# prstrive/SCGaussian

Hardware: AMD Instinct MI355X
Metric: train_iters_per_sec (higher is better)
Workload: dtype f32; 1 GPU; S2: 200000 Gaussians, 1008x756, SH degree 3, fwd+bwd per view (BASELINE configs[1] shape: LLFF-fern 3-view training, 200 k Gaussians @ 1008x756); gaussians=200000, width=1008, height=756, sh_degree=3, visible=174771, views=3, parallelism=single, ranks_seen=1, launched_by=single process, grad_bucket_bytes=0, grad_bucket_bytes_per_view=0

## Files before the change

scgaussian_amd/csrc/api.hip:

```cpp
#include <stdarg.h>
#include <stdio.h>
#include <string.h>

#include "scg_common.h"
#include "scg_debug.h"

#include <atomic>
#include <chrono>
#include <thread>

namespace scg {

static thread_local char g_err[512] = "";

int fail(int code, const char* fmt, ...) {
    va_list ap;
    va_start(ap, fmt);
    vsnprintf(g_err, sizeof(g_err), fmt, ap);
    va_end(ap);
    return code;
}

int check_hip(hipError_t e, const char* what) {
    if (e == hipSuccess) return 0;
    snprintf(g_err, sizeof(g_err), "%s: %s (hipError %d)", what, hipGetErrorString(e), (int)e);
    return (int)e;
}

int validate_frame(const ScgFrame* f, bool need_bg) {
    if (!f) return fail(SCG_E_NULL, "frame is NULL");
    if (f->P < 0) return fail(SCG_E_RANGE, "P = %d < 0", f->P);
    if (f->width <= 0 || f->height <= 0 || f->width > 65535 * SCG_TILE || f->height > 65535 * SCG_TILE)
        return fail(SCG_E_RANGE, "image size %d x %d out of range", f->width, f->height);
    if (f->sh_degree < 0 || f->sh_degree > 3) return fail(SCG_E_RANGE, "sh_degree %d not in 0..3", f->sh_degree);
    if (!(f->tanfovx > 0.f) || !(f->tanfovy > 0.f)) return fail(SCG_E_RANGE, "tanfov must be positive");
    if (!f->viewmatrix || !f->projmatrix || !f->campos) return fail(SCG_E_NULL, "viewmatrix/projmatrix/campos is NULL");
    if (need_bg && !f->bg) return fail(SCG_E_NULL, "bg is NULL");
    return 0;
}

static inline size_t align_up(size_t v, size_t a) { return (v + a - 1) / a * a; }
static inline bool aligned16(const void* p) { return (reinterpret_cast<uintptr_t>(p) & 15u) == 0; }
static inline bool aligned64(const void* p) { return (reinterpret_cast<uintptr_t>(p) & 63u) == 0; }
int validate_model(const ScgFrame* f, const ScgModel* m);

static int validate_inputs(const ScgFrame* f, const float* means3D, const float* opacities, const float* shs,
                           const float* colors_precomp, const float* scales, const float* rotations,
                           const float* cov3D_precomp) {
    if (f->P == 0) return 0;
    if (!means3D || !opacities) return fail(SCG_E_NULL, "means3D/opacities is NULL");
    if ((shs == nullptr) == (colors_precomp == nullptr))
        return fail(SCG_E_EXCLUSIVE, "Please provide exactly one of either SHs or precomputed colors!");
    const bool has_sr = scales != nullptr && rotations != nullptr;
    if ((scales != nullptr) != (rotations != nullptr) || has_sr == (cov3D_precomp != nullptr))
        return fail(SCG_E_EXCLUSIVE,
                    "Please provide exactly one of either scale/rotation pair or precomputed 3D covariance!");
    if (shs && f->sh_coeffs < (f->sh_degree + 1) * (f->sh_degree + 1))
        return fail(SCG_E_RANGE, "sh_coeffs %d < (sh_degree+1)^2 = %d", f->sh_coeffs,
                    (f->sh_degree + 1) * (f->sh_degree + 1));
    if (rotations && !aligned16(rotations)) return fail(SCG_E_ALIGN, "rotations must be 16-byte aligned");
    return 0;
}

static int validate_model_set(const ScgModelSet& m, bool ray, const char* name) {
    if (m.count < 0) return fail(SCG_E_RANGE, "%s.count = %d < 0", name, m.count);
    if (m.count == 0) return 0;
    if (ray ? (!m.zval || !m.rayo || !m.rayd) : !m.xyz)
        return fail(SCG_E_NULL, ray ? "%s: zval / rayo / rayd is NULL" : "%s: xyz is NULL", name);
    if (!m.features_dc || !m.features_rest || !m.opacity || !m.scaling || !m.rotation)
        return fail(SCG_E_NULL, "%s: features_dc / features_rest / opacity / scaling / rotation is NULL", name);
    if (!aligned16(m.rotation) || !aligned16(m.features_rest) || !aligned16(m.features_dc))
        return fail(SCG_E_ALIGN, "%s: rotation / features_rest / features_dc must be 16-byte aligned", name);
    return 0;
}

int validate_model(const ScgFrame* f, const ScgModel* m) {
    int rc = validate_model_set(m->ray, true, "model.ray");
    if (rc) return rc;
    if ((rc = validate_model_set(m->bg, false, "model.bg"))) return rc;
    if ((int64_t)m->ray.count + m->bg.count != f->P)
        return fail(SCG_E_RANGE, "model holds %d + %d Gaussians, frame.P = %d", m->ray.count, m->bg.count, f->P);
    if (f->P > 0 && f->sh_coeffs != 16)
        return fail(SCG_E_RANGE, "the model path reads (n,1,3) + (n,15,3) SH records: frame.sh_coeffs must be 16, not %d", f->sh_coeffs);
    return 0;
}

}

using namespace scg;

extern "C" {

const char* scg_last_error(void) { return g_err; }
int32_t scg_abi_version(void) { return SCG_ABI_VERSION; }

size_t scg_struct_bytes(int32_t which) {
    switch (which) {
        case 0: return sizeof(ScgFrame);
        case 1: return sizeof(ScgWorkspaceLayout);
        case 2: return sizeof(ScgStageEvents);
        case 3: return sizeof(ScgModel);
        case 4: return sizeof(ScgModelGrads);
        case 5: return sizeof(ScgAdamSegment);
        default: return 0;
    }
}

size_t scg_geometry_scratch_bytes(int32_t P) { return align_up(scan_scratch_bytes(P > 0 ? P : 1), 256); }

int scg_geometry_forward(const ScgFrame* frame, const float* means3D, const float* opacities, const float* shs,
                         const float* colors_precomp, const float* scales, const float* rotations,
                         const float* cov3D_precomp, float* splats, int32_t* radii, uint8_t* clamped,
                         uint32_t* rects, uint32_t* depth_keys, uint32_t* num_rendered_out, void* scratch,
                         size_t scratch_bytes, void* stream) {
    int rc = validate_frame(frame, false);
    if (rc) return rc;
    rc = validate_inputs(frame, means3D, opacities, shs, colors_precomp, scales, rotations, cov3D_precomp);
    if (rc) return rc;
    hipStream_t s = reinterpret_cast<hipStream_t>(stream);
    if (frame->P == 0)
        return num_rendered_out ? check_hip(hipMemsetAsync(num_rendered_out, 0, sizeof(uint32_t), s), "memset R") : 0;
    if (!splats || !radii || !clamped || !rects || !depth_keys || !scratch)
        return fail(SCG_E_NULL, "output/scratch pointer is NULL");
    if (!aligned16(splats)) return fail(SCG_E_ALIGN, "splats must be 16-byte aligned");
    if ((reinterpret_cast<uintptr_t>(rects) & 7u) != 0) return fail(SCG_E_ALIGN, "rects must be 8-byte aligned");
    if (scratch_bytes < scg_geometry_scratch_bytes(frame->P))
        return fail(SCG_E_SCRATCH, "geometry scratch: %zu < %zu bytes", scratch_bytes, scg_geometry_scratch_bytes(frame->P));
    const FrameDev f = make_frame_dev(frame);
    uint32_t* block_sums = reinterpret_cast<uint32_t*>(scratch);
    rc = launch_geometry_forward(f, means3D, opacities, shs, colors_precomp, scales, rotations, cov3D_precomp, splats,
                                 radii, clamped, rects, depth_keys, block_sums, s);
    if (rc || !num_rendered_out) return rc;
    return launch_total_from_block_sums(block_sums, (frame->P + kBlock - 1) / kBlock, num_rendered_out, s);
}

struct LegacyLayout { size_t keys0, keys1, vals0, offsets, scan, sortscr, total; };

static LegacyLayout legacy_layout(int P, int64_t R) {
    LegacyLayout L;
    size_t off = 0;
    auto take = [&](size_t bytes) { size_t o = off; off += align_up(bytes, 256); return o; };
    L.keys0 = take((size_t)R * sizeof(uint64_t));
    L.keys1 = take((size_t)R * sizeof(uint64_t));
    L.vals0 = take((size_t)R * sizeof(uint32_t));
    L.offsets = take((size_t)P * sizeof(uint32_t));
    L.scan = take(scan_scratch_bytes(P));
    L.sortscr = take(sort_scratch_bytes(R));
    L.total = off;
    return L;
}

static int key_bits(int n_tiles) {
    int bits = 0;
    while ((1ll << bits) < (long long)n_tiles) ++bits;
    return 32 + (bits > 0 ? bits : 1);
}

static int n_tiles_of(int32_t width, int32_t height) {
    return ((width + kTile - 1) / kTile) * ((height + kTile - 1) / kTile);
}

static bool use_tile_path(int n_tiles, int64_t R, int32_t algo) {
    if (algo == SCG_BINNING_GLOBAL_SORT) return false;
    return tile_binning_supported(n_tiles, R);
}

size_t scg_binning_scratch_bytes(int32_t P, int64_t num_rendered, int32_t width, int32_t height, int32_t algo) {
    const int64_t R = num_rendered > 0 ? num_rendered : 1;
    const int Pp = P > 0 ? P : 1;
    const int n_tiles = n_tiles_of(width, height);
    if (use_tile_path(n_tiles, R, algo)) return tile_binning_layout(Pp, R, n_tiles).total;
    return legacy_layout(Pp, R).total;
}

size_t scg_ranges_words(int32_t width, int32_t height) {
    const int n_tiles = ((width + kTile - 1) / kTile) * ((height + kTile - 1) / kTile);
    return (size_t)2 * n_tiles + (size_t)5 * tile_order_slots(n_tiles);
}

int32_t scg_forward_sorts_in_blend(int64_t capacity, int32_t width, int32_t height, int32_t options) {
    if (width <= 0 || height <= 0 || capacity <= 0 || (options & SCG_DEBUG_SEPARATE_SORT)) return 0;
    const int n_tiles = n_tiles_of(width, height);
    if (!use_tile_path(n_tiles, capacity, SCG_BINNING_AUTO)) return 0;
    return tile_binning_defers_sort(capacity, n_tiles) ? 1 : 0;
}

int32_t scg_binning_accepts_bound(int64_t num_rendered_bound, int32_t width, int32_t height, int32_t algo) {
    if (width <= 0 || height <= 0) return 0;
    return use_tile_path(n_tiles_of(width, height), num_rendered_bound > 0 ? num_rendered_bound : 1, algo) ? 1 : 0;
}

int scg_binning(const ScgFrame* frame, int64_t num_rendered, const uint32_t* rects, const uint32_t* depth_keys,
                uint32_t* point_list, uint32_t* ranges, uint64_t* keys_sorted, int32_t algo, void* scratch,
                size_t scratch_bytes, void* stream) {
    int rc = validate_frame(frame, false);
    if (rc) return rc;
    if (!ranges) return fail(SCG_E_NULL, "ranges is NULL");
    if (num_rendered < 0 || num_rendered > 0xFFFFFFFFll) return fail(SCG_E_RANGE, "num_rendered out of range");
    if (algo != SCG_BINNING_AUTO && algo != SCG_BINNING_GLOBAL_SORT) return fail(SCG_E_RANGE, "unknown binning algo %d", algo);
    hipStream_t s = reinterpret_cast<hipStream_t>(stream);
    const FrameDev f = make_frame_dev(frame);
    const int n_tiles = f.gx * f.gy;
    if (num_rendered == 0 || frame->P == 0) return launch_tile_ranges(nullptr, 0, ranges, n_tiles, s);
    if (!rects || !depth_keys || !point_list || !scratch) return fail(SCG_E_NULL, "binning pointer is NULL");
    const size_t need = scg_binning_scratch_bytes(frame->P, num_rendered, frame->width, frame->height, algo);
    if (scratch_bytes < need) return fail(SCG_E_SCRATCH, "binning scratch: %zu < %zu bytes", scratch_bytes, need);

    if (use_tile_path(n_tiles, num_rendered, algo))
        return launch_tile_binning(f, num_rendered, rects, depth_keys, point_list, ranges, keys_sorted, scratch, nullptr, false, false, false, false, s);

    const LegacyLayout L = legacy_layout(frame->P, num_rendered);
    char* base = reinterpret_cast<char*>(scratch);
    uint64_t* keys0 = reinterpret_cast<uint64_t*>(base + L.keys0);
    uint64_t* keys1 = reinterpret_cast<uint64_t*>(base + L.keys1);
    uint32_t* vals0 = reinterpret_cast<uint32_t*>(base + L.vals0);
    uint32_t* offsets = reinterpret_cast<uint32_t*>(base + L.offsets);
    rc = launch_rect_counts_scan(rects, frame->P, offsets, reinterpret_cast<uint32_t*>(base + L.scan), s);
    if (rc) return rc;
    const int end_bit = key_bits(n_tiles);
    const bool odd = (sort_num_passes(end_bit) & 1) != 0;
    uint64_t* ka = odd ? keys0 : keys1;
    uint32_t* va = odd ? vals0 : point_list;
    uint64_t* kb = odd ? keys1 : keys0;
    uint32_t* vb = odd ? point_list : vals0;
    rc = launch_duplicate_keys(f, rects, depth_keys, offsets, ka, va, s);
    if (rc) return rc;
    rc = launch_sort_pairs(ka, va, kb, vb, num_rendered, end_bit, base + L.sortscr, s, odd);
    if (rc) return rc;
    rc = launch_tile_ranges(keys1, num_rendered, ranges, n_tiles, s);
    if (rc) return rc;
    if (keys_sorted)
        return check_hip(hipMemcpyAsync(keys_sorted, keys1, (size_t)num_rendered * sizeof(uint64_t),
                                        hipMemcpyDeviceToDevice, s), "copy keys_sorted");
    return 0;
}

size_t scg_sort_scratch_bytes(int64_t n) { return align_up(sort_scratch_bytes(n > 0 ? n : 1), 256); }

int scg_sort_pairs(uint64_t* keys_in, uint32_t* vals_in, uint64_t* keys_out, uint32_t* vals_out, int64_t n,
                   int32_t end_bit, void* scratch, size_t scratch_bytes, void* stream) {
    if (n < 0 || n > 0xFFFFFFFFll) return fail(SCG_E_RANGE, "n out of range");
    if (end_bit < 1 || end_bit > 64) return fail(SCG_E_RANGE, "end_bit %d not in 1..64", end_bit);
    if (n == 0) return 0;
    if (!keys_in || !vals_in || !keys_out || !vals_out || !scratch) return fail(SCG_E_NULL, "sort pointer is NULL");
    if (scratch_bytes < scg_sort_scratch_bytes(n)) return fail(SCG_E_SCRATCH, "sort scratch too small");
    return launch_sort_pairs(keys_in, vals_in, keys_out, vals_out, n, end_bit, scratch,
                             reinterpret_cast<hipStream_t>(stream), true);
}

size_t scg_scan_scratch_bytes(int64_t n) { return align_up(scan_scratch_bytes(n > 0 ? n : 1), 256); }

int scg_inclusive_scan_u32(const uint32_t* in, uint32_t* out, int64_t n, uint32_t* total_out, void* scratch,
                           size_t scratch_bytes, void* stream) {
    if (n < 0 || n > 0x7FFFFFFFll * 256) return fail(SCG_E_RANGE, "n out of range");
    hipStream_t s = reinterpret_cast<hipStream_t>(stream);
    if (n == 0) return total_out ? check_hip(hipMemsetAsync(total_out, 0, sizeof(uint32_t), s), "memset total") : 0;
    if (!in || !out || !scratch) return fail(SCG_E_NULL, "scan pointer is NULL");
    if (scratch_bytes < scg_scan_scratch_bytes(n)) return fail(SCG_E_SCRATCH, "scan scratch too small");
    return launch_inclusive_scan(in, out, n, total_out, scratch, s);
}

int scg_blend_forward(const ScgFrame* frame, const uint32_t* ranges, const uint32_t* point_list,
                      const float* splats, float* out_color, float* out_depth, float* out_alpha, float* final_T,
                      uint32_t* n_contrib, float* dsplats_zero, void* stream) {
    int rc = validate_frame(frame, true);
    if (rc) return rc;
    if (!ranges || !out_color || !out_depth || !out_alpha || !final_T || !n_contrib)
        return fail(SCG_E_NULL, "blend_forward pointer is NULL");
    if (splats && !aligned16(splats)) return fail(SCG_E_ALIGN, "splats must be 16-byte aligned");
    if (dsplats_zero && !aligned64(dsplats_zero)) return fail(SCG_E_ALIGN, "dsplats_zero must be 64-byte aligned");
    const FrameDev f = make_frame_dev(frame);
    return launch_blend_forward(f, ranges, point_list, splats, out_color, out_depth, out_alpha, final_T, n_contrib,
                                dsplats_zero, reinterpret_cast<hipStream_t>(stream));
}

static int blend_backward_checked(const ScgFrame* frame, const uint32_t* ranges, const uint32_t* point_list,
                                  const float* splats, const float* final_T, const uint32_t* n_contrib,
                                  const float* dL_dcolor, const float* dL_ddepth, const float* dL_dalpha, float* dsplats,
                                  int32_t dsplats_prezeroed, void* stream, hipEvent_t started, hipEvent_t done) {
    int rc = validate_frame(frame, true);
    if (rc) return rc;
    if (frame->P == 0) return 0;
    if (!ranges || !final_T || !n_contrib || !dL_dcolor || !dsplats || !splats)
        return fail(SCG_E_NULL, "blend_backward pointer is NULL");
    if (!aligned16(splats)) return fail(SCG_E_ALIGN, "splats must be 16-byte aligned");
    if (!aligned64(dsplats)) return fail(SCG_E_ALIGN, "dsplats must be 64-byte aligned (one record = one line)");
    if (frame->P > 60000000) return fail(SCG_E_RANGE, "blend_backward addresses gradient records with 32-bit offsets: P <= 60e6");
    const FrameDev f = make_frame_dev(frame);
    return launch_blend_backward(f, ranges, point_list, splats, final_T, n_contrib, dL_dcolor, dL_ddepth, dL_dalpha,
                                 dsplats, dsplats_prezeroed != 0, reinterpret_cast<hipStream_t>(stream), started, done);
}

int scg_blend_backward(const ScgFrame* frame, const uint32_t* ranges, const uint32_t* point_list,
                       const float* splats, const float* final_T, const uint32_t* n_contrib, const float* dL_dcolor,
                       const float* dL_ddepth, const float* dL_dalpha, float* dsplats, int32_t dsplats_prezeroed,
                       void* stream) {
    return blend_backward_checked(frame, ranges, point_list, splats, final_T, n_contrib, dL_dcolor, dL_ddepth, dL_dalpha,
                                  dsplats, dsplats_prezeroed, stream, nullptr, nullptr);
}

int scg_geometry_backward(const ScgFrame* frame, const float* means3D, const float* opacities, const float* shs,
                          const float* colors_precomp, const float* scales, const float* rotations,
                          const float* cov3D_precomp, const int32_t* radii, const uint8_t* clamped,
                          const float* dsplats, float* dL_dmeans3D, float* dL_dmeans2D, float* dL_dopacities,
                          float* dL_dshs, float* dL_dcolors_precomp, float* dL_dscales, float* dL_drotations,
                          float* dL_dcov3D_precomp, int32_t accumulate, void* stream) {
    int rc = validate_frame(frame, false);
    if (rc) return rc;
    rc = validate_inputs(frame, means3D, opacities, shs, colors_precomp, scales, rotations, cov3D_precomp);
    if (rc) return rc;
    if (frame->P == 0) return 0;
    if (!radii || !clamped || !dsplats || !dL_dmeans3D || !dL_dmeans2D || !dL_dopacities)
        return fail(SCG_E_NULL, "geometry_backward pointer is NULL");
    if ((shs != nullptr) != (dL_dshs != nullptr) || (colors_precomp != nullptr) != (dL_dcolors_precomp != nullptr))
        return fail(SCG_E_EXCLUSIVE, "dL_dshs / dL_dcolors_precomp must match the colour input that was used");
    const bool has_sr = scales != nullptr;
    if (has_sr != (dL_dscales != nullptr) || has_sr != (dL_drotations != nullptr) ||
        (cov3D_precomp != nullptr) != (dL_dcov3D_precomp != nullptr))
        return fail(SCG_E_EXCLUSIVE, "dL_dscales/dL_drotations / dL_dcov3D_precomp must match the covariance input used");
    if (!aligned64(dsplats) || (dL_drotations && !aligned16(dL_drotations)))
        return fail(SCG_E_ALIGN, "dsplats must be 64-byte, dL_drotations 16-byte aligned");
    const FrameDev f = make_frame_dev(frame);
    return launch_geometry_backward(f, means3D, opacities, shs, colors_precomp, scales, rotations, cov3D_precomp, radii,
                                    clamped, dsplats, dL_dmeans3D, dL_dmeans2D, dL_dopacities, dL_dshs,
                                    dL_dcolors_precomp, dL_dscales, dL_drotations, dL_dcov3D_precomp,
                                    accumulate & (SCG_BACKWARD_ACCUMULATE | SCG_BACKWARD_SH_TAIL_ZERO),
                                    reinterpret_cast<hipStream_t>(stream));
}

static inline int mark(const ScgStageEvents* ev, int stage, bool end, hipStream_t s) {
    if (!ev) return 0;
    void* e = end ? ev->end[stage] : ev->begin[stage];
    return e ? check_hip(hipEventRecord(reinterpret_cast<hipEvent_t>(e), s), "stage event record") : 0;
}

int scg_workspace_layout(int32_t P, int64_t capacity, int32_t width, int32_t height, ScgWorkspaceLayout* out) {
    if (!out) return fail(SCG_E_NULL, "layout is NULL");
    if (P < 0 || capacity < 0 || capacity > 0xFFFFFFFFll || width <= 0 || height <= 0)
        return fail(SCG_E_RANGE, "workspace layout: P / capacity / image size out of range");
    const int64_t cap = capacity > 0 ? capacity : 1;
    const size_t Pp = (size_t)(P > 0 ? P : 1), hw = (size_t)width * height;
    size_t off = 0;
    auto take = [&](size_t bytes) { size_t o = off; off += align_up(bytes, 256); return (uint64_t)o; };
    out->splats = take(Pp * SCG_SPLAT_FLOATS * sizeof(float));
    out->rects = take(Pp * 2 * sizeof(uint32_t));
    out->depth_keys = take(Pp * sizeof(uint32_t));
    out->clamped = take(Pp);
    out->point_list = take((size_t)cap * sizeof(uint32_t));
    out->ranges = take(scg_ranges_words(width, height) * sizeof(uint32_t));
    out->final_T = take(hw * sizeof(float));
    out->n_contrib = take(hw * sizeof(uint32_t));
    out->bin_scratch = take(scg_binning_scratch_bytes(P, cap, width, height, SCG_BINNING_AUTO));
    out->total = (uint64_t)off;
    out->partial_words = (uint64_t)(scg_geometry_scratch_bytes(P) / sizeof(uint32_t));
    return 0;
}

static int forward_impl(const ScgFrame* frame, const ScgModel* model, const float* means3D, const float* opacities,
                        const float* shs, const float* colors_precomp, const float* scales, const float* rotations,
                        const float* cov3D_precomp, int64_t capacity, void* workspace, size_t workspace_bytes, int32_t* radii,
                        float* out_color, float* out_depth, float* out_alpha, uint32_t* partial_sums, void* event,
                        float* dsplats_zero, int32_t options, const ScgStageEvents* stage_events, void* stream) {
    int rc = validate_frame(frame, true);
    if (rc) return rc;
    rc = model ? validate_model(frame, model)
               : validate_inputs(frame, means3D, opacities, shs, colors_precomp, scales, rotations, cov3D_precomp);
    if (rc) return rc;
    if (!workspace || !out_color || !out_depth || !out_alpha || !partial_sums || (frame->P > 0 && !radii))
        return fail(SCG_E_NULL, "scg_forward: workspace / output / partial_sums pointer is NULL");
    if (!aligned16(workspace)) return fail(SCG_E_ALIGN, "workspace must be 16-byte aligned");
    if (dsplats_zero && !aligned64(dsplats_zero)) return fail(SCG_E_ALIGN, "dsplats_zero must be 64-byte aligned");
    ScgWorkspaceLayout L;
    rc = scg_workspace_layout(frame->P, capacity, frame->width, frame->height, &L);
    if (rc) return rc;
    if (workspace_bytes < L.total) return fail(SCG_E_SCRATCH, "workspace: %zu < %llu bytes", workspace_bytes, (unsigned long long)L.total);
    hipStream_t s = reinterpret_cast<hipStream_t>(stream);
    const FrameDev f = make_frame_dev(frame);
    const int n_tiles = f.gx * f.gy;
    char* base = reinterpret_cast<char*>(workspace);
    float* splats = reinterpret_cast<float*>(base + L.splats);
    uint32_t* rects = reinterpret_cast<uint32_t*>(base + L.rects);
    uint32_t* depth_keys = reinterpret_cast<uint32_t*>(base + L.depth_keys);
    uint8_t* clamped = reinterpret_cast<uint8_t*>(base + L.clamped);
    uint32_t* point_list = reinterpret_cast<uint32_t*>(base + L.point_list);
    uint32_t* ranges = reinterpret_cast<uint32_t*>(base + L.ranges);
    const bool keep_state = !(options & SCG_FORWARD_NO_BACKWARD_STATE);
    float* final_T = keep_state ? reinterpret_cast<float*>(base + L.final_T) : nullptr;
    uint32_t* n_contrib = keep_state ? reinterpret_cast<uint32_t*>(base + L.n_contrib) : nullptr;
    const bool empty = frame->P == 0 || capacity == 0;
    if (!empty && !use_tile_path(n_tiles, capacity, SCG_BINNING_AUTO))
        return fail(SCG_E_RANGE, "scg_forward needs the tile-first binning path (scg_binning_accepts_bound); use the staged calls");
    if (options & SCG_FORWARD_ARM_PARTIAL_SUMS) {
        const int nb = frame->P > 0 ? (frame->P + kBlock - 1) / kBlock : 1;
        volatile uint32_t* w = partial_sums;
        for (int i = 0; i < nb; ++i) w[i] = SCG_PARTIAL_SUM_ARMED;
        std::atomic_thread_fence(std::memory_order_release);
    }
    if ((rc = mark(stage_events, 0, false, s))) return rc;
    const bool hist_in_geometry = !empty && !(options & SCG_DEBUG_SEPARATE_HIST) && tile_binning_hist_in_geometry(f, capacity);
    if (frame->P == 0) {
        rc = check_hip(hipMemsetAsync(partial_sums, 0, sizeof(uint32_t), s), "memset partial sums");
    } else if (hist_in_geometry) {
        rc = model ? launch_geometry_hist_binned_model(f, capacity, *model, splats, radii, clamped, rects, depth_keys, partial_sums,
                                                       base + L.bin_scratch, s)
                   : launch_geometry_hist_binned(f, capacity, means3D, opacities, shs, colors_precomp, scales, rotations,
                                                 cov3D_precomp, splats, radii, clamped, rects, depth_keys, partial_sums,
                                                 base + L.bin_scratch, s);
    } else {
        rc = model ? launch_geometry_forward_model(f, *model, splats, radii, clamped, rects, depth_keys, partial_sums, s)
                   : launch_geometry_forward(f, means3D, opacities, shs, colors_precomp, scales, rotations, cov3D_precomp, splats,
                                             radii, clamped, rects, depth_keys, partial_sums, s);
    }
    if (rc) return rc;
    if ((rc = mark(stage_events, 0, true, s))) return rc;
    if (event) {
        rc = check_hip(hipEventRecord(reinterpret_cast<hipEvent_t>(event), s), "event record");
        if (rc) return rc;
    }
    if ((rc = mark(stage_events, 1, false, s))) return rc;
    bool fused_sort = !empty && !(options & SCG_DEBUG_SEPARATE_SORT);
    const bool skip_rare = (options & SCG_FORWARD_SKIP_RARE_SORT) != 0;
    if (empty && frame->num_rendered_out)
        if ((rc = check_hip(hipMemsetAsync(frame->num_rendered_out, 0, sizeof(uint32_t), s), "memset num_rendered_out"))) return rc;
    rc = empty ? launch_tile_ranges(nullptr, 0, ranges, n_tiles, s)
               : launch_tile_binning(f, capacity, rects, depth_keys, point_list, ranges, nullptr, base + L.bin_scratch,
                                     &fused_sort, hist_in_geometry, skip_rare, (options & SCG_FORWARD_RARE_8WAVE) != 0,
                                     (options & SCG_FORWARD_SPLIT_LONG_LISTS) != 0, s);
    if (rc) return rc;
    if ((rc = mark(stage_events, 1, true, s))) return rc;
    if ((rc = mark(stage_events, 2, false, s))) return rc;
    rc = fused_sort ? launch_tile_blend_forward(f, ranges, point_list, depth_keys, splats, out_color, out_depth, out_alpha,
                                                final_T, n_contrib, frame->P ? dsplats_zero : nullptr, base + L.bin_scratch,
                                                capacity, !skip_rare, s)
                    : launch_blend_forward(f, ranges, point_list, splats, out_color, out_depth, out_alpha, final_T, n_contrib,
                                           frame->P ? dsplats_zero : nullptr, s);
    if (rc) return rc;
    return mark(stage_events, 2, true, s);
}

int scg_forward(const ScgFrame* frame, const float* means3D, const float* opacities, const float* shs,
                const float* colors_precomp, const float* scales, const float* rotations, const float* cov3D_precomp,
                int64_t capacity, void* workspace, size_t workspace_bytes, int32_t* radii, float* out_color,
                float* out_depth, float* out_alpha, uint32_t* partial_sums, void* event, float* dsplats_zero,
                int32_t options, const ScgStageEvents* stage_events, void* stream) {
    return forward_impl(frame, nullptr, means3D, opacities, shs, colors_precomp, scales, rotations, cov3D_precomp, capacity,
                        workspace, workspace_bytes, radii, out_color, out_depth, out_alpha, partial_sums, event, dsplats_zero,
                        options, stage_events, stream);
}

int scg_forward_model(const ScgFrame* frame, const ScgModel* model, int64_t capacity, void* workspace, size_t workspace_bytes,
                      int32_t* radii, float* out_color, float* out_depth, float* out_alpha, uint32_t* partial_sums, void* event,
                      float* dsplats_zero, int32_t options, const ScgStageEvents* stage_events, void* stream) {
    if (!model) return fail(SCG_E_NULL, "model is NULL");
    return forward_impl(frame, model, nullptr, nullptr, nullptr, nullptr, nullptr, nullptr, nullptr, capacity, workspace,
                        workspace_bytes, radii, out_color, out_depth, out_alpha, partial_sums, event, dsplats_zero, options,
                        stage_events, stream);
}

int scg_model_activate(const ScgModel* model, float* means3D, float* opacities, float* scales, float* rotations, void* stream) {
    if (!model) return fail(SCG_E_NULL, "model is NULL");
    ScgFrame fr;
    memset(&fr, 0, sizeof(fr));
    fr.P = model->ray.count + model->bg.count;
    fr.sh_coeffs = 16;
    const int rc = validate_model(&fr, model);
    if (rc) return rc;
    if (rotations && !aligned16(rotations)) return fail(SCG_E_ALIGN, "rotations must be 16-byte aligned");
    return launch_model_activate(*model, means3D, opacities, scales, rotations, reinterpret_cast<hipStream_t>(stream));
}

int64_t scg_wait_num_rendered(void* event, const uint32_t* partial_sums_host, int32_t P) {
    if (!partial_sums_host) { fail(SCG_E_NULL, "partial_sums_host is NULL"); return SCG_E_NULL; }
    const int nb = P > 0 ? (P + kBlock - 1) / kBlock : 1;
    if (event) {
        const hipError_t e = hipEventSynchronize(reinterpret_cast<hipEvent_t>(event));
        if (e != hipSuccess) { check_hip(e, "event synchronize"); return -(int64_t)e - 1000; }
    } else {
        const volatile uint32_t* w = partial_sums_host;
        const auto t0 = std::chrono::steady_clock::now();
        for (int i = nb - 1; i >= 0; --i) {
            uint64_t spins = 0;
            while (w[i] == SCG_PARTIAL_SUM_ARMED) {
                if (spins < 100000u) __builtin_ia32_pause(); else std::this_thread::yield();
                if ((++spins & 0xFFFFu) == 0 &&
                    std::chrono::steady_clock::now() - t0 > std::chrono::seconds(120)) {
                    fail(SCG_E_RANGE, "scg_wait_num_rendered: the geometry stage's partial sums did not arrive within 120 s "
                                      "(kernel fault, or partial_sums is not host-coherent memory)");
                    return SCG_E_RANGE;
                }
            }
        }
        std::atomic_thread_fence(std::memory_order_acquire);
    }
    int64_t total = 0;
    for (int i = 0; i < nb; ++i) total += partial_sums_host[i];
    return total;
}

int scg_event_create(void** event_out, int32_t timing) {
    if (!event_out) return fail(SCG_E_NULL, "event_out is NULL");
    hipEvent_t ev;
    const int rc = check_hip(hipEventCreateWithFlags(&ev, timing ? hipEventDefault : hipEventDisableTiming), "event create");
    if (rc) return rc;
    *event_out = reinterpret_cast<void*>(ev);
    return 0;
}

int scg_event_destroy(void* event) {
    return event ? check_hip(hipEventDestroy(reinterpret_cast<hipEvent_t>(event)), "event destroy") : 0;
}

int scg_event_elapsed_ms(void* begin, void* end, float* ms_out) {
    if (!begin || !end || !ms_out) return fail(SCG_E_NULL, "event / ms_out is NULL");
    return check_hip(hipEventElapsedTime(ms_out, reinterpret_cast<hipEvent_t>(begin), reinterpret_cast<hipEvent_t>(end)),
                     "event elapsed time");
}

int scg_backward(const ScgFrame* frame, const float* means3D, const float* opacities, const float* shs,
                 const float* colors_precomp, const float* scales, const float* rotations, const float* cov3D_precomp,
                 const int32_t* radii, int64_t capacity, const void* workspace, const float* dL_dcolor,
                 const float* dL_ddepth, const float* dL_dalpha, float* dsplats, int32_t dsplats_prezeroed,
                 float* dL_dmeans3D, float* dL_dmeans2D, float* dL_dopacities, float* dL_dshs, float* dL_dcolors_precomp,
                 float* dL_dscales, float* dL_drotations, float* dL_dcov3D_precomp, int32_t accumulate,
                 const ScgStageEvents* stage_events, void* stream) {
    if (!frame) return fail(SCG_E_NULL, "frame is NULL");
    if (frame->P == 0) return 0;
    if (!workspace) return fail(SCG_E_NULL, "workspace is NULL");
    ScgWorkspaceLayout L;
    int rc = scg_workspace_layout(frame->P, capacity, frame->width, frame->height, &L);
    if (rc) return rc;
    hipStream_t s = reinterpret_cast<hipStream_t>(stream);
    const char* base = reinterpret_cast<const char*>(workspace);
    hipEvent_t bb_begin = stage_events ? reinterpret_cast<hipEvent_t>(stage_events->begin[0]) : nullptr;
    hipEvent_t bb_end = stage_events ? reinterpret_cast<hipEvent_t>(stage_events->end[0]) : nullptr;
    rc = blend_backward_checked(frame, reinterpret_cast<const uint32_t*>(base + L.ranges),
                                reinterpret_cast<const uint32_t*>(base + L.point_list),
                                reinterpret_cast<const float*>(base + L.splats),
                                reinterpret_cast<const float*>(base + L.final_T),
                                reinterpret_cast<const uint32_t*>(base + L.n_contrib), dL_dcolor, dL_ddepth, dL_dalpha,
                                dsplats, dsplats_prezeroed, stream, bb_begin, bb_end);
    if (rc) return rc;
    if ((rc = mark(stage_events, 1, false, s))) return rc;
    rc = scg_geometry_backward(frame, means3D, opacities, shs, colors_precomp, scales, rotations, cov3D_precomp, radii,
                               reinterpret_cast<const uint8_t*>(base + L.clamped), dsplats, dL_dmeans3D, dL_dmeans2D,
                               dL_dopacities, dL_dshs, dL_dcolors_precomp, dL_dscales, dL_drotations, dL_dcov3D_precomp,
                               accumulate, stream);
    if (rc) return rc;
    return mark(stage_events, 1, true, s);
}

int scg_backward_model(const ScgFrame* frame, const ScgModel* model, const int32_t* radii, int64_t capacity, const void* workspace,
                       const float* dL_dcolor, const float* dL_ddepth, const float* dL_dalpha, float* dsplats,
                       int32_t dsplats_prezeroed, const ScgModelGrads* grads, float* dL_dmeans2D, int32_t flags,
                       const ScgStageEvents* stage_events, void* stream) {
    if (!frame) return fail(SCG_E_NULL, "frame is NULL");
    if (!model || !grads) return fail(SCG_E_NULL, "model / grads is NULL");
    int rc = validate_frame(frame, false);
    if (rc) return rc;
    if ((rc = validate_model(frame, model))) return rc;
    if (frame->P == 0) return 0;
    if (!workspace || !radii || !dL_dmeans2D) return fail(SCG_E_NULL, "workspace / radii / dL_dmeans2D is NULL");
    for (int k = 0; k < 2; ++k) {
        const ScgModelSet& ms = k ? model->bg : model->ray;
        const ScgModelGradSet& gs = k ? grads->bg : grads->ray;
        if (ms.count == 0) continue;
        if ((k == 0 ? !gs.zval : !gs.xyz) || !gs.features_dc || !gs.features_rest || !gs.opacity || !gs.scaling || !gs.rotation)
            return fail(SCG_E_NULL, "grads.%s: a gradient buffer of a non-empty set is NULL", k ? "bg" : "ray");
        if (!aligned16(gs.rotation) || !aligned16(gs.features_rest) || !aligned16(gs.features_dc))
            return fail(SCG_E_ALIGN, "grads.%s: rotation / features_rest / features_dc must be 16-byte aligned", k ? "bg" : "ray");
    }
    ScgWorkspaceLayout L;
    rc = scg_workspace_layout(frame->P, capacity, frame->width, frame->height, &L);
    if (rc) return rc;
    hipStream_t s = reinterpret_cast<hipStream_t>(stream);
    const char* base = reinterpret_cast<const char*>(workspace);
    hipEvent_t bb_begin = stage_events ? reinterpret_cast<hipEvent_t>(stage_events->begin[0]) : nullptr;
    hipEvent_t bb_end = stage_events ? reinterpret_cast<hipEvent_t>(stage_events->end[0]) : nullptr;
    rc = blend_backward_checked(frame, reinterpret_cast<const uint32_t*>(base + L.ranges),
                                reinterpret_cast<const uint32_t*>(base + L.point_list),
                                reinterpret_cast<const float*>(base + L.splats),
                                reinterpret_cast<const float*>(base + L.final_T),
                                reinterpret_cast<const uint32_t*>(base + L.n_contrib), dL_dcolor, dL_ddepth, dL_dalpha,
                                dsplats, dsplats_prezeroed, stream, bb_begin, bb_end);
    if (rc) return rc;
    if ((rc = mark(stage_events, 1, false, s))) return rc;
    const FrameDev f = make_frame_dev(frame);
    rc = launch_geometry_backward_model(f, *model, *grads, radii, reinterpret_cast<const uint8_t*>(base + L.clamped), dsplats,
                                        dL_dmeans2D, flags & (SCG_BACKWARD_ACCUMULATE | SCG_BACKWARD_SH_TAIL_ZERO), s);
    if (rc) return rc;
    return mark(stage_events, 1, true, s);
}

}
```

scgaussian_amd/csrc/binning_tiles.hip:

```cpp
#include "scg_common.h"
#include "tile_sort.h"
#include "tile_walk.h"

#include <mutex>

namespace scg {

constexpr int kTileBlocksSmall = 128;
constexpr int kTileBlocksLarge = 256;
constexpr int64_t kLargeFrame = 1ll << 20;
constexpr int kLargeScene = 100000;
constexpr int kSortSmallMax = 2048;
constexpr int kSortDenseMax = 4096;
constexpr int kSortMidMax = 8192;
constexpr int kVeryLong = 16384;
constexpr int kSort8Max = 4096;
constexpr int kSortBigLdsMax = 16384;
constexpr int kMaxDynLds = 152 * 1024;

template <class F>
__device__ __forceinline__ void visit_instances(const uint2* __restrict__ rects, int grid_x, uint32_t ga, uint32_t gb,
                                                F&& f) {
    const int lane = lane_id();
    for (uint32_t g0 = ga; g0 < gb; g0 += kWave) {
        const uint32_t g = g0 + lane;
        uint2 r = make_uint2(0u, 0u);
        if (g < gb) r = rects[g];
        walk_rects(r, g, grid_x, f);
    }
}

__global__ __launch_bounds__(kBinThreads) void tile_hist_kernel(const uint2* __restrict__ rects, uint32_t P,
                                                                int grid_x, int n_tiles,
                                                                uint32_t* __restrict__ table,
                                                                uint32_t* __restrict__ class_counts,
                                                                uint32_t* __restrict__ len_hist) {
    extern __shared__ __attribute__((aligned(16))) unsigned char smem[];
    uint32_t* hist = reinterpret_cast<uint32_t*>(smem);
    if (blockIdx.x == 0) {
        if (threadIdx.x < 4) class_counts[threadIdx.x] = 0u;
        len_hist[threadIdx.x] = 0u;
    }
    for (int t = threadIdx.x; t < n_tiles; t += kBinThreads) hist[t] = 0;
    __syncthreads();
    uint32_t ga, gb;
    wave_slice(P, gridDim.x, blockIdx.x, wave_id(), ga, gb);
    visit_instances(rects, grid_x, ga, gb, [&](uint32_t tile, uint32_t) { atomicAdd(&hist[tile], 1u); });
    __syncthreads();
    uint32_t* row = table + (size_t)blockIdx.x * n_tiles;
    for (int t = threadIdx.x; t < n_tiles; t += kBinThreads) row[t] = hist[t];
}

constexpr int kColTiles = 64;
constexpr int kColGroups = kBinThreads / kColTiles;
constexpr int kColRowsMax = 16;

constexpr int kBands8 = 8;
constexpr int kLenClasses = 64;

__device__ __forceinline__ int len_class(uint32_t total, int shift) {
    return (int)min((uint32_t)(kLenClasses - 1), total >> shift);
}
__device__ __forceinline__ int order_class(const uint32_t* __restrict__ cost_in, int t, uint32_t total, int shift) {
    if (!cost_in) return len_class(total, shift);
    if (total == 0u) return 0;
    const int c = (int)(__float_as_uint((float)cost_in[t]) >> 19) - ((127 + 5) << 4);
    return max(0, min(kLenClasses - 1, c));
}

__global__ __launch_bounds__(kBinThreads) void table_colscan_kernel(uint32_t* __restrict__ table, int nblocks,
                                                                    int n_tiles, uint32_t* __restrict__ tile_total,
                                                                    uint32_t* __restrict__ len_hist, int len_shift,
                                                                    const uint32_t* __restrict__ cost_in,
                                                                    uint8_t* __restrict__ tile_class,
                                                                    uint32_t* __restrict__ tile_part) {
    __shared__ uint32_t s_part[kColGroups][kColTiles];
    const int c = threadIdx.x & (kColTiles - 1);
    const int q = threadIdx.x / kColTiles;
    const int t = blockIdx.x * kColTiles + c;
    const int b0 = (int)((int64_t)nblocks * q / kColGroups), b1 = (int)((int64_t)nblocks * (q + 1) / kColGroups);
    uint32_t v[kColRowsMax];
    uint32_t sum = 0;
#pragma unroll
    for (int k = 0; k < kColRowsMax; ++k) {
        v[k] = 0;
        if (t < n_tiles && b0 + k < b1) v[k] = table[(size_t)(b0 + k) * n_tiles + t];
    }
#pragma unroll
    for (int k = 0; k < kColRowsMax; ++k) sum += v[k];
    s_part[q][c] = sum;
    __syncthreads();
    uint32_t run = 0;
    for (int k = 0; k < q; ++k) run += s_part[k][c];
    __shared__ uint32_t s_len[kBands8 * kLenClasses];
    if (threadIdx.x < kBands8 * kLenClasses) s_len[threadIdx.x] = 0u;
    __syncthreads();
    if (t < n_tiles && q == kColGroups - 1) {
        tile_total[t] = run + sum;
        const int per = (n_tiles + 7) >> 3;
        const int cls = order_class(cost_in, t, run + sum, len_shift);
        tile_class[t] = (uint8_t)cls;
        atomicAdd(&s_len[(t / per) * kLenClasses + cls], 1u);
    }
    __syncthreads();
    if (threadIdx.x < kBands8 * kLenClasses && s_len[threadIdx.x]) atomicAdd(&len_hist[threadIdx.x], s_len[threadIdx.x]);
    if (q == kColGroups - 1) s_part[0][c] = (t < n_tiles) ? run + sum : 0u;
    __syncthreads();
    if (threadIdx.x < kColTiles) {
        uint32_t tot = s_part[0][threadIdx.x];
#pragma unroll
        for (int off = 32; off > 0; off >>= 1) tot += (uint32_t)__shfl_xor((int)tot, off, kWave);
        if (threadIdx.x == 0) tile_part[blockIdx.x] = tot;
    }
#pragma unroll
    for (int k = 0; k < kColRowsMax; ++k) {
        if (t < n_tiles && b0 + k < b1) table[(size_t)(b0 + k) * n_tiles + t] = run;
        run += v[k];
    }
}

constexpr int kBands = 8;
constexpr int kQueue = 2 * kWave;
constexpr int kScatterThreads = 256;
constexpr int kScatterWaves = kScatterThreads / kWave;

__device__ __forceinline__ uint32_t totals_before(const uint32_t* __restrict__ tile_total,
                                                  const uint32_t* __restrict__ tile_part, int t_first, uint32_t* s_red) {
    const int full = t_first / kColTiles;
    uint32_t v = 0;
    for (int k = threadIdx.x; k < full; k += kScatterThreads) v += tile_part[k];
    for (int k = full * kColTiles + (int)threadIdx.x; k < t_first; k += kScatterThreads) v += tile_total[k];
#pragma unroll
    for (int off = 32; off > 0; off >>= 1) v += (uint32_t)__shfl_xor((int)v, off, kWave);
    __syncthreads();
    if (lane_id() == 0) s_red[wave_id()] = v;
    __syncthreads();
    uint32_t sum = 0;
#pragma unroll
    for (int k = 0; k < kScatterWaves; ++k) sum += s_red[k];
    return sum;
}

__device__ __forceinline__ uint32_t block_exclusive_256(uint32_t v, uint32_t* s_red, uint32_t& total) {
    const int lane = lane_id(), w = wave_id();
    uint32_t inc = v;
#pragma unroll
    for (int off = 1; off < kWave; off <<= 1) {
        const uint32_t n = (uint32_t)__shfl_up((int)inc, off, kWave);
        if (lane >= off) inc += n;
    }
    __syncthreads();
    if (lane == kWave - 1) s_red[w] = inc;
    __syncthreads();
    uint32_t before = 0;
    total = 0;
#pragma unroll
    for (int k = 0; k < kScatterWaves; ++k) {
        const uint32_t sk = s_red[k];
        if (k < w) before += sk;
        total += sk;
    }
    return before + inc - v;
}

__device__ __forceinline__ void publish_tile_starts(int x, int n_tiles, const uint32_t* __restrict__ tile_total,
                                                    const uint32_t* __restrict__ tile_part,
                                                    uint32_t* __restrict__ tile_start, uint2* __restrict__ ranges,
                                                    uint32_t capacity, uint32_t* __restrict__ class_counts,
                                                    uint32_t* __restrict__ mid_tiles, uint32_t* __restrict__ big_tiles,
                                                    uint32_t small_max, const uint32_t* __restrict__ len_hist,
                                                    const uint8_t* __restrict__ tile_class,
                                                    uint32_t* __restrict__ cost_out, const uint32_t* __restrict__ bcost_in,
                                                    uint8_t* q_class ,
                                                    uint32_t* __restrict__ nr_out) {
    __shared__ uint32_t s_red[kScatterWaves];
    __shared__ uint32_t s_first[kLenClasses];
    __shared__ uint32_t s_cnt[kLenClasses];
    const int per = (n_tiles + 7) >> 3;
    const int t0 = x * per, t1 = min(t0 + per, n_tiles);
    const int lane = lane_id();
    if (threadIdx.x < kLenClasses) {
        uint32_t before = 0;
        for (int k = (int)threadIdx.x + 1; k < kLenClasses; ++k) before += len_hist[x * kLenClasses + k];
        s_first[threadIdx.x] = before;
        s_cnt[threadIdx.x] = 0u;
    }
    uint32_t carry = totals_before(tile_total, tile_part, min(t0, n_tiles), s_red);
    uint32_t* order = reinterpret_cast<uint32_t*>(ranges) + 2 * (size_t)n_tiles;
    for (int k0 = t0; k0 < t1; k0 += kScatterThreads) {
        const int t = k0 + (int)threadIdx.x;
        const bool in = t < t1;
        const uint32_t cnt = in ? tile_total[t] : 0u;
        uint32_t total;
        const uint32_t run = carry + block_exclusive_256(cnt, s_red, total);
        carry += total;
        uint32_t len = 0;
        if (in) {
            tile_start[t] = run;
            const uint32_t lo = min(run, capacity), hi = min(run + cnt, capacity);
            ranges[t] = (hi > lo) ? make_uint2(lo, hi) : make_uint2(0u, 0u);
            len = hi - lo;
            if (t == n_tiles - 1) {
                tile_start[n_tiles] = run + cnt;
                if (nr_out) *nr_out = run + cnt;
            }
            if (cost_out) cost_out[t] = 0u;
            const int c = (int)tile_class[t];
            order[t0 + s_first[c] + atomicAdd(&s_cnt[c], 1u)] = (uint32_t)t;
        }
        const bool is_big = len > (uint32_t)kSortMidMax, is_mid = !is_big && len > small_max;
        const uint64_t m_mid = __ballot(is_mid), m_big = __ballot(is_big);
        const uint64_t m_split = __ballot(len > (uint32_t)kVeryLong);
        if (lane == 0 && m_split) atomicAdd(&class_counts[3], (uint32_t)__popcll(m_split));
        uint32_t base_mid = 0, base_big = 0;
        if (lane == 0) {
            if (m_mid) base_mid = atomicAdd(&class_counts[0], (uint32_t)__popcll(m_mid));
            if (m_big) base_big = atomicAdd(&class_counts[1], (uint32_t)__popcll(m_big));
        }
        base_mid = (uint32_t)__shfl((int)base_mid, 0, kWave);
        base_big = (uint32_t)__shfl((int)base_big, 0, kWave);
        const uint64_t below = (lane == 0) ? 0ull : (~0ull >> (kWave - lane));
        if (is_mid) mid_tiles[base_mid + (uint32_t)__popcll(m_mid & below)] = (uint32_t)t;
        if (is_big) big_tiles[base_big + (uint32_t)__popcll(m_big & below)] = (uint32_t)t;
    }
    for (int k = max(t0, t1) + (int)threadIdx.x; k < t0 + per; k += kScatterThreads) order[k] = (uint32_t)n_tiles;

    uint32_t* order_q = order + (size_t)tile_order_slots(n_tiles);
    const int slots8 = tile_order_slots(n_tiles) >> 3;
    const int nq = 4 * max(t1 - t0, 0);
    __syncthreads();
    if (!bcost_in) {
        for (int e = threadIdx.x; e < 4 * slots8; e += kScatterThreads) {
            const uint32_t t = order[t0 + (e >> 2)];
            order_q[4 * (size_t)t0 + e] = (t < (uint32_t)n_tiles) ? 4u * t + (uint32_t)(e & 3) : 4u * (uint32_t)n_tiles;
        }
        return;
    }
    auto qclass = [&](int e) {
        const uint32_t c = bcost_in[4 * (size_t)t0 + e];
        const int k = (int)(__float_as_uint((float)c) >> 19) - ((127 + 4) << 4);
        return max(0, min(kLenClasses - 1, k));
    };
    if (threadIdx.x < kLenClasses) s_cnt[threadIdx.x] = 0u;
    __syncthreads();
    for (int e = threadIdx.x; e < nq; e += kScatterThreads) {
        const int c = qclass(e);
        q_class[e] = (uint8_t)c;
        atomicAdd(&s_cnt[c], 1u);
    }
    __syncthreads();
    if (threadIdx.x < kLenClasses) {
        uint32_t before = 0;
        for (int k = (int)threadIdx.x + 1; k < kLenClasses; ++k) before += s_cnt[k];
        s_first[threadIdx.x] = before;
    }
    __syncthreads();
    if (threadIdx.x < kLenClasses) s_cnt[threadIdx.x] = 0u;
    __syncthreads();
    for (int e = threadIdx.x; e < nq; e += kScatterThreads) {
        const int c = (int)q_class[e];
        order_q[4 * (size_t)t0 + s_first[c] + atomicAdd(&s_cnt[c], 1u)] = 4u * (uint32_t)t0 + (uint32_t)e;
    }
    for (int e = nq + (int)threadIdx.x; e < 4 * slots8; e += kScatterThreads) order_q[4 * (size_t)t0 + e] = 4u * (uint32_t)n_tiles;
}

__device__ __forceinline__ void band_rows(int gy, int band, int& r0, int& r1) {
    r0 = (int)((int64_t)gy * band / kBands);
    r1 = (int)((int64_t)gy * (band + 1) / kBands);
}

__global__ __launch_bounds__(kScatterThreads) void tile_scatter_kernel(const uint2* __restrict__ rects, uint32_t P,
                                                                   int grid_x, int grid_y, int n_slices,
                                                                   const uint32_t* __restrict__ table,
                                                                   const uint32_t* __restrict__ tile_total,
                                                                   const uint32_t* __restrict__ tile_part,
                                                                   uint32_t* __restrict__ point_list,
                                                                   uint32_t capacity,
                                                                   uint32_t* __restrict__ tile_start,
                                                                   uint2* __restrict__ ranges,
                                                                   uint32_t* __restrict__ class_counts,
                                                                   uint32_t* __restrict__ mid_tiles,
                                                                   uint32_t* __restrict__ big_tiles, uint32_t small_max,
                                                                   const uint32_t* __restrict__ len_hist,
                                                                   const uint8_t* __restrict__ tile_class,
                                                                   uint32_t* __restrict__ cost_out, int block_slices,
                                                                   const uint32_t* __restrict__ bcost_in,
                                                                   uint32_t* __restrict__ nr_out) {
    extern __shared__ __attribute__((aligned(16))) unsigned char smem[];
    uint32_t* cursor = reinterpret_cast<uint32_t*>(smem);
    __shared__ uint2 s_qrect[kScatterWaves][kQueue];
    __shared__ uint32_t s_qid[kScatterWaves][kQueue];
    __shared__ uint32_t s_red[2 * kScatterWaves];
    const int n_tiles = grid_x * grid_y;
    if (blockIdx.x < kBands) {
        publish_tile_starts((int)blockIdx.x, n_tiles, tile_total, tile_part, tile_start, ranges, capacity, class_counts,
                            mid_tiles, big_tiles, small_max, len_hist, tile_class, cost_out, bcost_in,
                            smem ,
                            nr_out);
        return;
    }
#ifdef SCG_PROBE_TIMELINE
    uint32_t* tl = cost_out ? cost_out + n_tiles + ((size_t)blockIdx.x * kScatterWaves + wave_id()) * 8 : nullptr;
    const uint32_t tl0 = (uint32_t)wall_clock64();
    uint32_t tl_walk = 0, tl_nwalk = 0, tl_most = 0;
#endif
    const int wg = (int)blockIdx.x - kBands;
    const int band = wg & (kBands - 1), slice = wg >> 3;
    int r0, r1;
    band_rows(grid_y, band, r0, r1);
    const int t_lo = r0 * grid_x, nt = (r1 - r0) * grid_x;
    if (nt == 0) return;
    const int w = wave_id(), lane = lane_id();
    uint32_t sa, sb, dummy;
    if (block_slices) {
        block_slice(P, (uint32_t)n_slices, (uint32_t)slice, sa, sb);
        sa = min(sa * (uint32_t)kBlock, P);
        sb = min(sb * (uint32_t)kBlock, P);
    } else {
        wave_slice(P, (uint32_t)n_slices, (uint32_t)slice, 0u, sa, dummy);
        wave_slice(P, (uint32_t)n_slices, (uint32_t)slice, (uint32_t)kBinWaves - 1u, dummy, sb);
    }
    const uint32_t ga = sa + (uint32_t)((uint64_t)(sb - sa) * w / kScatterWaves);
    const uint32_t gb = sa + (uint32_t)((uint64_t)(sb - sa) * (w + 1) / kScatterWaves);
    constexpr int kAhead = 2;
    auto fetch = [&](uint32_t g) { return (g < gb) ? rects[g] : make_uint2(0u, 0u); };
    uint2 r_q[kAhead];
#pragma unroll
    for (int a = 0; a < kAhead; ++a) r_q[a] = fetch(ga + (uint32_t)(a * kWave + lane));
    const uint32_t* row = table + (size_t)slice * n_tiles + t_lo;
    constexpr int kRowRegs = 8;
    uint32_t row_pre[kRowRegs];
#pragma unroll
    for (int j = 0; j < kRowRegs; ++j) {
        const int k = j * kScatterThreads + (int)threadIdx.x;
        row_pre[j] = (k < nt) ? row[k] : 0u;
    }
    {
        const int full = t_lo / kColTiles;
        uint32_t before = 0;
        const int tail_k = full * kColTiles + (int)threadIdx.x;
        const uint32_t part0 = tile_part[min((int)threadIdx.x, max(full - 1, 0))];
        const uint32_t tail0 = tile_total[min(tail_k, n_tiles - 1)];
        uint32_t tot_pre[kRowRegs];
#pragma unroll
        for (int j = 0; j < kRowRegs; ++j) tot_pre[j] = tile_total[t_lo + min(j * kScatterThreads + (int)threadIdx.x, nt - 1)];
#pragma unroll
        for (int j = 0; j < kRowRegs; ++j) {
            const int k = j * kScatterThreads + (int)threadIdx.x;
            if (k < nt) cursor[k] = tot_pre[j];
        }
        for (int k = kRowRegs * kScatterThreads + (int)threadIdx.x; k < nt; k += kScatterThreads) cursor[k] = tile_total[t_lo + k];
        if ((int)threadIdx.x < full) before += part0;
        if (tail_k < t_lo) before += tail0;
        for (int k = (int)threadIdx.x + kScatterThreads; k < full; k += kScatterThreads) before += tile_part[k];
#pragma unroll
        for (int off = 32; off > 0; off >>= 1) before += (uint32_t)__shfl_xor((int)before, off, kWave);
        __syncthreads();
        const int share = (nt + kScatterThreads - 1) / kScatterThreads;
        const int k_a = min((int)threadIdx.x * share, nt), k_b = min(k_a + share, nt);
        uint32_t mine = 0;
        for (int k = k_a; k < k_b; ++k) mine += cursor[k];
        uint32_t inc = mine;
#pragma unroll
        for (int off = 1; off < kWave; off <<= 1) {
            const uint32_t n = (uint32_t)__shfl_up((int)inc, off, kWave);
            if (lane >= off) inc += n;
        }
        if (lane == kWave - 1) { s_red[w] = inc; s_red[kScatterWaves + w] = before; }
        __syncthreads();
        uint32_t start = inc - mine;
#pragma unroll
        for (int k = 0; k < kScatterWaves; ++k) start += s_red[kScatterWaves + k] + (k < w ? s_red[k] : 0u);
        for (int k = k_a; k < k_b; ++k) {
            const uint32_t cnt = cursor[k];
            cursor[k] = start;
            start += cnt;
        }
        __syncthreads();
#pragma unroll
        for (int j = 0; j < kRowRegs; ++j) {
            const int k = j * kScatterThreads + (int)threadIdx.x;
            if (k < nt) cursor[k] += row_pre[j];
        }
        for (int k = kRowRegs * kScatterThreads + (int)threadIdx.x; k < nt; k += kScatterThreads) cursor[k] += row[k];
        if (threadIdx.x < kWave) cursor[nt + threadIdx.x] = 0u;
    }
    __syncthreads();

#ifdef SCG_PROBE_TIMELINE
    const uint32_t tl1 = (uint32_t)wall_clock64();
#endif
    uint2* qrect = s_qrect[w];
    uint32_t* qid = s_qid[w];
    auto drop = [&](uint32_t tile, uint32_t id) {
        const uint32_t pos = atomicAdd(&cursor[tile - (uint32_t)t_lo], 1u);
        if (pos < capacity) point_list[pos] = id;
    };
    auto scatter_rects = [&](uint2 r, uint32_t g) {
#ifdef SCG_PROBE_TIMELINE
        const uint32_t tw0 = (uint32_t)wall_clock64();
#endif
        const uint32_t wd = r.y & 0xFFFFu, ht = r.y >> 16;
        const uint32_t cnt = wd * ht;
        const uint32_t dump = (uint32_t)nt + (uint32_t)lane;
        uint32_t small = (cnt <= kCoopThreshold) ? cnt : 0u;
        uint32_t x = 0, row_tile = (r.x >> 16) * (uint32_t)grid_x + (r.x & 0xFFFFu) - (uint32_t)t_lo;
        uint32_t most = small;
#pragma unroll
        for (int off = 32; off > 0; off >>= 1) most = max(most, (uint32_t)__shfl_xor((int)most, off, kWave));
        for (uint32_t k = 0; k < most; k += 4) {
            uint32_t slot[4], pos[4];
#pragma unroll
            for (int u = 0; u < 4; ++u) {
                slot[u] = (k + u < small) ? row_tile + x : dump;
                if (++x == wd) { x = 0; row_tile += (uint32_t)grid_x; }
            }
#pragma unroll
            for (int u = 0; u < 4; ++u) pos[u] = atomicAdd(&cursor[slot[u]], 1u);
#pragma unroll
            for (int u = 0; u < 4; ++u)
                if (k + u < small && pos[u] < capacity) point_list[pos[u]] = g;
        }
        walk_rects(cnt > kCoopThreshold ? r : make_uint2(0u, 0u), g, grid_x, drop);
#ifdef SCG_PROBE_TIMELINE
        tl_walk += (uint32_t)wall_clock64() - tw0; tl_nwalk += 1; tl_most += most;
#endif
    };
    int qn = 0;
    for (uint32_t g0 = ga; g0 < gb; g0 += kWave) {
        const uint32_t g = g0 + lane;
        const uint2 r = r_q[0];
#pragma unroll
        for (int a = 0; a + 1 < kAhead; ++a) r_q[a] = r_q[a + 1];
        r_q[kAhead - 1] = fetch(g + kAhead * kWave);
        const int y0 = max((int)(r.x >> 16), r0), y1 = min((int)(r.x >> 16) + (int)(r.y >> 16), r1);
        const bool touches = (r.y & 0xFFFFu) != 0u && y1 > y0;
        const uint64_t m = __ballot(touches);
        if (touches) {
            const int at = qn + (int)__builtin_amdgcn_mbcnt_hi((uint32_t)(m >> 32), __builtin_amdgcn_mbcnt_lo((uint32_t)m, 0u));
            qrect[at] = make_uint2((r.x & 0xFFFFu) | ((uint32_t)y0 << 16), (r.y & 0xFFFFu) | ((uint32_t)(y1 - y0) << 16));
            qid[at] = g;
        }
        qn += __popcll(m);
        __builtin_amdgcn_fence(__ATOMIC_ACQ_REL, "wavefront");
        __builtin_amdgcn_wave_barrier();
        if (qn >= kWave) {
            const uint2 qr = qrect[lane];
            const uint32_t qg = qid[lane];
            const uint2 mr = qrect[kWave + lane];
            const uint32_t mg = qid[kWave + lane];
            __builtin_amdgcn_fence(__ATOMIC_ACQ_REL, "wavefront");
            __builtin_amdgcn_wave_barrier();
            qn -= kWave;
            if (lane < qn) { qrect[lane] = mr; qid[lane] = mg; }
            __builtin_amdgcn_fence(__ATOMIC_ACQ_REL, "wavefront");
            __builtin_amdgcn_wave_barrier();
            scatter_rects(qr, qg);
        }
    }
    if (qn > 0) {
        uint2 qr = make_uint2(0u, 0u);
        uint32_t qg = 0;
        if (lane < qn) { qr = qrect[lane]; qg = qid[lane]; }
        scatter_rects(qr, qg);
    }
#ifdef SCG_PROBE_TIMELINE
    if (tl && lane == 0) {
        tl[0] = tl0; tl[1] = tl1; tl[2] = (uint32_t)wall_clock64(); tl[3] = tl_walk; tl[4] = tl_nwalk; tl[5] = tl_most;
        tl[6] = gb - ga; tl[7] = 0xC0FFEEu;
    }
#endif
}

__device__ __forceinline__ void sort_tile_in_lds(uint64_t* s_keys, const uint32_t* __restrict__ depth_keys,
                                                 uint32_t* __restrict__ list, int n) {
    for (int i = threadIdx.x; i < n; i += (int)blockDim.x) {
        const uint32_t id = list[i];
        s_keys[i] = ((uint64_t)depth_keys[id] << 32) | (uint64_t)id;
    }
    __syncthreads();
    bitonic_sort_asc(s_keys, n, false);
    __syncthreads();
    for (int i = threadIdx.x; i < n; i += (int)blockDim.x) list[i] = (uint32_t)s_keys[i];
}

template <int NW, int MAX_N>
__global__ __launch_bounds__(NW * kWave) void tile_sort_kernel(const uint2* __restrict__ ranges,
                                                               const uint32_t* __restrict__ depth_keys,
                                                               uint32_t* __restrict__ point_list, int id_bits) {
    __shared__ TileSortLds<NW, MAX_N> L;
    const uint2 r = ranges[blockIdx.x];
    const int n = (int)(r.y - r.x);
    if (n < 2 || n > MAX_N) return;
    sort_one_tile<NW, MAX_N, MAX_N>(L, r, depth_keys, point_list, id_bits);
}

constexpr int kRareThreads = 16 * kWave;
constexpr int kLongBuckets = 8192;

__device__ __forceinline__ void sort_big_tile(unsigned char* smem, const uint2 r, const uint32_t* __restrict__ depth_keys,
                                              uint32_t* __restrict__ point_list, uint64_t* __restrict__ spill,
                                              uint64_t* __restrict__ spill2) {
    const int n = (int)(r.y - r.x);
    uint32_t* list = point_list + r.x;
    uint64_t* keys = spill + r.x;
    if (!sort_long_list<kRareThreads, kLongBuckets>(smem, depth_keys, list, n, keys, spill2 + r.x)) {
        __syncthreads();
        if (n <= kSortBigLdsMax) {
            sort_tile_in_lds(reinterpret_cast<uint64_t*>(smem), depth_keys, list, n);
        } else {
            for (int i = threadIdx.x; i < n; i += kRareThreads) {
                const uint32_t id = list[i];
                keys[i] = ((uint64_t)depth_keys[id] << 32) | (uint64_t)id;
            }
            __syncthreads();
            bitonic_sort_asc(keys, n, true);
            __syncthreads();
            for (int i = threadIdx.x; i < n; i += kRareThreads) list[i] = (uint32_t)keys[i];
        }
    }
}

constexpr int kSegTarget = 1024;
constexpr int kSplitBatch = 16;
constexpr int kSegMaxPerTile = 8192;
static_assert(kSegTarget + kLongBucketMax <= kSort8Max, "a segment must fit the 8-wave sort");
static_assert(kLongBucketMax <= kSegTarget, "consecutive bucket starts must be at most a segment apart: no segment index is skipped");

__device__ __forceinline__ bool split_long_list(unsigned char* smem, const uint2 r, const uint32_t* __restrict__ depth_keys,
                                                uint32_t* __restrict__ point_list, uint64_t* __restrict__ A,
                                                uint32_t* __restrict__ seg_count, uint2* __restrict__ segments) {
    constexpr int T = kRareThreads, NW = T / kWave, PER = kLongBuckets / T;
    uint32_t* cnt = reinterpret_cast<uint32_t*>(smem);
    uint32_t* cur = cnt + kLongBuckets + 4;
    uint32_t* red = cur + kLongBuckets;
    uint32_t* pm = red + 2 * NW + 4;
    const int n = (int)(r.y - r.x);
    uint32_t* list = point_list + r.x;
    const int t = threadIdx.x, w = wave_id(), lane = lane_id();
    const int n_seg = (n + kSegTarget - 1) / kSegTarget;
    if (n_seg > kSegMaxPerTile) return false;
    uint32_t kmin, kmax;
    {
        const uint32_t key = depth_keys[list[(int)(((int64_t)t * n) / T)]];
        kmin = key; kmax = key;
    }
    for (int b = t; b < kLongBuckets; b += T) cnt[b] = 0u;
    for (int m = t; m <= n_seg; m += T) pm[m] = (uint32_t)n;
#pragma unroll
    for (int off = 32; off > 0; off >>= 1) {
        kmin = min(kmin, (uint32_t)__shfl_xor((int)kmin, off, kWave));
        kmax = max(kmax, (uint32_t)__shfl_xor((int)kmax, off, kWave));
    }
    if (lane == 0) { red[2 * w] = kmin; red[2 * w + 1] = kmax; }
    __syncthreads();
#pragma unroll
    for (int k = 0; k < NW; ++k) { kmin = min(kmin, red[2 * k]); kmax = max(kmax, red[2 * k + 1]); }
    const int sh = __builtin_clz((kmax - kmin) | 1u);
    auto bucket_of = [&](uint64_t comp) {
        const uint32_t key = (uint32_t)(comp >> 32);
        return __umulhi((min(max(key, kmin), kmax) - kmin) << sh, (uint32_t)kLongBuckets);
    };
    for (int i0 = t; i0 < n; i0 += kSplitBatch * T) {
        uint32_t id[kSplitBatch], key[kSplitBatch];
#pragma unroll
        for (int u = 0; u < kSplitBatch; ++u) id[u] = list[min(i0 + u * T, n - 1)];
#pragma unroll
        for (int u = 0; u < kSplitBatch; ++u) key[u] = depth_keys[id[u]];
#pragma unroll
        for (int u = 0; u < kSplitBatch; ++u) {
            if (i0 + u * T < n) {
                const uint64_t comp = ((uint64_t)key[u] << 32) | (uint64_t)id[u];
                A[i0 + u * T] = comp;
                atomicAdd(&cnt[bucket_of(comp)], 1u);
            }
        }
    }
    __syncthreads();
    uint32_t c[PER], sum = 0, cmax = 0;
#pragma unroll
    for (int j = 0; j < PER; ++j) { c[j] = cnt[t * PER + j]; sum += c[j]; cmax = max(cmax, c[j]); }
    uint32_t incl = sum;
#pragma unroll
    for (int off = 1; off < kWave; off <<= 1) {
        const uint32_t up = (uint32_t)__shfl_up((int)incl, off, kWave);
        if (lane >= off) incl += up;
    }
#pragma unroll
    for (int off = 32; off > 0; off >>= 1) cmax = max(cmax, (uint32_t)__shfl_xor((int)cmax, off, kWave));
    __syncthreads();
    if (lane == kWave - 1) red[w] = incl;
    if (lane == 0) red[NW + w] = cmax;
    __syncthreads();
    uint32_t base = incl - sum;
    for (int k = 0; k < w; ++k) base += red[k];
#pragma unroll
    for (int k = 0; k < NW; ++k) cmax = max(cmax, red[NW + k]);
    if (cmax > (uint32_t)kLongBucketMax) return false;
#pragma unroll
    for (int j = 0; j < PER; ++j) { cnt[t * PER + j] = base; cur[t * PER + j] = base; base += c[j]; }
    if (t == T - 1) cnt[kLongBuckets] = base;
    __syncthreads();
#pragma unroll
    for (int j = 0; j < PER; ++j) {
        const int b = t * PER + j;
        const uint32_t s_b = cnt[b];
        if (b == 0) {
            pm[0] = 0u;
        } else if (s_b < (uint32_t)n) {
            const uint32_t m = s_b / (uint32_t)kSegTarget;
            if (m * (uint32_t)kSegTarget > cnt[b - 1]) pm[m] = s_b;
        }
    }
    __syncthreads();
    for (int i0 = t; i0 < n; i0 += kSplitBatch * T) {
        uint64_t comp[kSplitBatch];
#pragma unroll
        for (int u = 0; u < kSplitBatch; ++u) comp[u] = A[min(i0 + u * T, n - 1)];
#pragma unroll
        for (int u = 0; u < kSplitBatch; ++u)
            if (i0 + u * T < n) list[atomicAdd(&cur[bucket_of(comp[u])], 1u)] = (uint32_t)comp[u];
    }
    int n_valid = 0;
    for (int m0 = 0; m0 < n_seg; m0 += T) n_valid += __syncthreads_count((m0 + t < n_seg) && pm[m0 + t] < (uint32_t)n);
    if (t == 0) red[2 * NW] = atomicAdd(seg_count, (uint32_t)n_valid);
    __syncthreads();
    const uint32_t out = red[2 * NW];
    for (int m = t; m < n_valid; m += T)
        segments[out + m] = make_uint2(r.x + pm[m], r.x + ((m + 1 < n_valid) ? pm[m + 1] : (uint32_t)n));
    return true;
}

__global__ __launch_bounds__(kRareThreads) void tile_split_long_kernel(const uint2* __restrict__ ranges,
                                                                       const uint32_t* __restrict__ depth_keys,
                                                                       uint32_t* __restrict__ point_list,
                                                                       uint64_t* __restrict__ spill,
                                                                       uint64_t* __restrict__ spill2,
                                                                       uint32_t* __restrict__ class_counts,
                                                                       const uint32_t* __restrict__ mid_tiles,
                                                                       const uint32_t* __restrict__ big_tiles,
                                                                       uint2* __restrict__ segments) {
    extern __shared__ __attribute__((aligned(16))) unsigned char smem[];
    const uint32_t n_mid = class_counts[0], n_big = class_counts[1];
    for (uint32_t i = blockIdx.x; i < n_big + n_mid; i += gridDim.x) {
        const uint2 r = ranges[i < n_big ? big_tiles[i] : mid_tiles[i - n_big]];
        if (r.y - r.x <= (uint32_t)kSort8Max) continue;
        if (!split_long_list(smem, r, depth_keys, point_list, spill + r.x, class_counts + 2, segments)) {
            __syncthreads();
            sort_big_tile(smem, r, depth_keys, point_list, spill, spill2);
            __syncthreads();
            if (threadIdx.x == 0) {
                const uint32_t at = atomicAdd(class_counts + 2, 1u);
                segments[at] = make_uint2(r.x, r.x);
            }
        }
        __syncthreads();
    }
}

constexpr int kList8Threads = 8 * kWave;
constexpr int kList8LongBuckets = 4096;

__device__ __noinline__ void sort_unsplit_list8(unsigned char* smem, const uint2 r, const uint32_t* __restrict__ depth_keys,
                                                uint32_t* __restrict__ point_list, uint64_t* __restrict__ spill,
                                                uint64_t* __restrict__ spill2) {
    const int n = (int)(r.y - r.x);
    uint32_t* list = point_list + r.x;
    uint64_t* keys = spill + r.x;
    if (!sort_long_list<kList8Threads, kList8LongBuckets, 2>(smem, depth_keys, list, n, keys, spill2 + r.x)) {
        __syncthreads();
        for (int k = threadIdx.x; k < n; k += kList8Threads) {
            const uint32_t id = list[k];
            keys[k] = ((uint64_t)depth_keys[id] << 32) | (uint64_t)id;
        }
        __syncthreads();
        bitonic_sort_asc(keys, n, true);
        __syncthreads();
        for (int k = threadIdx.x; k < n; k += kList8Threads) list[k] = (uint32_t)keys[k];
    }
}

__global__ __launch_bounds__(kList8Threads) __attribute__((amdgpu_waves_per_eu(6, 6))) void tile_sort_list8_kernel(const uint2* __restrict__ ranges,
                                                                        const uint32_t* __restrict__ depth_keys,
                                                                        uint32_t* __restrict__ point_list, int id_bits,
                                                                        uint64_t* __restrict__ spill,
                                                                        uint64_t* __restrict__ spill2,
                                                                        const uint32_t* __restrict__ class_counts,
                                                                        const uint32_t* __restrict__ mid_tiles,
                                                                        const uint32_t* __restrict__ big_tiles,
                                                                        const uint2* __restrict__ segments, int presplit) {
    __shared__ TileSortLds<8, kSort8Max> L;
    static_assert(sizeof(L) >= (2 * kList8LongBuckets + 4 + 2 * 8 + 8) * sizeof(uint32_t), "the unsplit fallback's counters must fit");
    const uint32_t n_mid = class_counts[0], n_big = class_counts[1];
    const uint32_t n_seg = presplit ? class_counts[2] : 0u;
    for (uint32_t i = blockIdx.x; i < n_seg + n_mid + n_big; i += gridDim.x) {
        uint2 r;
        if (i < n_seg) r = segments[i];
        else if (i < n_seg + n_mid) r = ranges[mid_tiles[i - n_seg]];
        else r = ranges[big_tiles[i - n_seg - n_mid]];
        const int n = (int)(r.y - r.x);
        if (n >= 2 && n <= kSort8Max) {
            sort_one_tile<8, kSort8Max, kSort8Max>(L, r, depth_keys, point_list, id_bits);
        } else if (n > kSort8Max && !presplit) {
            sort_unsplit_list8(reinterpret_cast<unsigned char*>(&L), r, depth_keys, point_list, spill, spill2);
        }
        __syncthreads();
    }
}

constexpr size_t kRareLds = (size_t)kSortBigLdsMax * sizeof(uint64_t) > sizeof(TileSortLds<16, kSortMidMax>)
                                ? (size_t)kSortBigLdsMax * sizeof(uint64_t) : sizeof(TileSortLds<16, kSortMidMax>);
static_assert(kRareLds >= (2 * kLongBuckets + 4 + 2 * 16 + 8 + kSegMaxPerTile + 1) * sizeof(uint32_t), "split_long_list's LDS");

__global__ __launch_bounds__(kRareThreads) void tile_sort_rare_kernel(const uint2* __restrict__ ranges,
                                                                      const uint32_t* __restrict__ depth_keys,
                                                                      uint32_t* __restrict__ point_list, int id_bits,
                                                                      uint64_t* __restrict__ spill,
                                                                      uint64_t* __restrict__ spill2,
                                                                      const uint32_t* __restrict__ class_counts,
                                                                      const uint32_t* __restrict__ mid_tiles,
                                                                      const uint32_t* __restrict__ big_tiles) {
    extern __shared__ __attribute__((aligned(16))) unsigned char smem[];
    TileSortLds<16, kSortMidMax>& L = *reinterpret_cast<TileSortLds<16, kSortMidMax>*>(smem);
    const uint32_t n_mid = class_counts[0], n_big = class_counts[1];
    for (uint32_t i = blockIdx.x; i < n_mid; i += gridDim.x) {
        sort_one_tile<16, kSortMidMax, kSortMidMax>(L, ranges[mid_tiles[i]], depth_keys, point_list, id_bits);
        __syncthreads();
    }
    for (uint32_t t = gridDim.x - 1 - blockIdx.x; t < n_big; t += gridDim.x) {
        sort_big_tile(smem, ranges[big_tiles[t]], depth_keys, point_list, spill, spill2);
        __syncthreads();
    }
}

__global__ __launch_bounds__(kBlock) void rebuild_keys_kernel(const uint32_t* __restrict__ tile_start, int n_tiles,
                                                              const uint32_t* __restrict__ point_list,
                                                              const uint32_t* __restrict__ depth_keys, int64_t R,
                                                              uint64_t* __restrict__ keys_sorted) {
    const int64_t s = (int64_t)blockIdx.x * kBlock + threadIdx.x;
    if (s >= R) return;
    int lo = 0, hi = n_tiles;
    while (hi - lo > 1) {
        const int mid = (lo + hi) >> 1;
        if (tile_start[mid] <= (uint32_t)s) lo = mid; else hi = mid;
    }
    keys_sorted[s] = ((uint64_t)(uint32_t)lo << 32) | (uint64_t)depth_keys[point_list[s]];
}

static inline size_t align_up(size_t v, size_t a) { return (v + a - 1) / a * a; }

struct DeviceSetup {
    std::once_flag once;
    bool ok = false;
    int n_cus = 256;
};
constexpr int kMaxDevices = 64;
static DeviceSetup g_device_setup[kMaxDevices];

static const DeviceSetup* device_setup() {
    int dev = 0;
    if (hipGetDevice(&dev) != hipSuccess || dev < 0 || dev >= kMaxDevices) return nullptr;
    DeviceSetup& d = g_device_setup[dev];
    std::call_once(d.once, [&] {
        int v = 0;
        const hipError_t e0 = hipFuncSetAttribute(reinterpret_cast<const void*>(tile_hist_kernel),
                                                  hipFuncAttributeMaxDynamicSharedMemorySize, kMaxDynLds);
        hipError_t e1 = hipFuncSetAttribute(reinterpret_cast<const void*>(tile_sort_rare_kernel),
                                            hipFuncAttributeMaxDynamicSharedMemorySize, (int)kRareLds);
        if (e1 == hipSuccess)
            e1 = hipFuncSetAttribute(reinterpret_cast<const void*>(tile_split_long_kernel),
                                     hipFuncAttributeMaxDynamicSharedMemorySize, (int)kRareLds);
        const hipError_t e2 = hipDeviceGetAttribute(&v, hipDeviceAttributeMultiprocessorCount, dev);
        hipError_t e3 = geometry_hist_set_max_lds(kMaxDynLds);
        if (e3 == hipSuccess) e3 = geometry_hist_model_set_max_lds(kMaxDynLds);
        d.n_cus = (e2 == hipSuccess && v > 0) ? v : 256;
        d.ok = (e0 == hipSuccess && e1 == hipSuccess && e3 == hipSuccess);
    });
    return d.ok ? &d : nullptr;
}

int tile_binning_blocks(int P, int64_t R) {
    return (R >= kLargeFrame || P >= kLargeScene) ? kTileBlocksLarge : kTileBlocksSmall;
}

bool tile_binning_supported(int n_tiles, int64_t R) {
    return (size_t)n_tiles * 4 <= (size_t)kMaxDynLds - 2048 && (size_t)kTileBlocksLarge * n_tiles * 4 <= (1ull << 30);
}

TileBinningLayout tile_binning_layout(int P, int64_t R, int n_tiles) {
    TileBinningLayout L;
    size_t off = 0;
    const int nb = tile_binning_blocks(P, R);
    auto take = [&](size_t bytes) { size_t o = off; off += align_up(bytes, 256); return o; };
    L.table = take((size_t)nb * n_tiles * 4);
    L.tile_total = take((size_t)n_tiles * 4);
    L.tile_start = take((size_t)(n_tiles + 1) * 4);
    L.class_counts = take(16);
    L.mid_tiles = take((size_t)n_tiles * 4);
    L.big_tiles = take((size_t)n_tiles * 4);
    L.len_hist = take((size_t)2 * kBands8 * kLenClasses * 4);
    L.tile_part = take((size_t)((n_tiles + kColTiles - 1) / kColTiles) * 4);
    L.tile_class = take((size_t)n_tiles);
    L.spill = take((size_t)R * 16);
    L.segments = take(((size_t)R / 1024 + 2 * (size_t)n_tiles + 8) * sizeof(uint2));
    L.total = off;
    L.nblocks = nb;
    return L;
}

bool tile_binning_defers_sort(int64_t R, int n_tiles) { return true; }

bool tile_binning_hist_in_geometry(const FrameDev& f, int64_t R) {
    const int n_tiles = f.gx * f.gy;
    return f.P > 0 && tile_binning_supported(n_tiles, R) &&
           (size_t)(n_tiles + (f.P + kBlock - 1) / kBlock / tile_binning_blocks(f.P, R) + 2) * 4 + 16 +
                   (size_t)kBinThreads * 64
               <= (size_t)kMaxDynLds - 2048;
}

int launch_geometry_hist_binned(const FrameDev& f, int64_t R, const float* means3D, const float* opacities, const float* shs,
                                const float* colors_precomp, const float* scales, const float* rotations,
                                const float* cov3D_precomp, float* splats, int32_t* radii, uint8_t* clamped, uint32_t* rects,
                                uint32_t* depth_keys, uint32_t* block_sums, void* bin_scratch, hipStream_t stream) {
    const TileBinningLayout L = tile_binning_layout(f.P, R, f.gx * f.gy);
    char* base = reinterpret_cast<char*>(bin_scratch);
    if (!device_setup()) return fail(SCG_E_RANGE, "tile binning: device setup failed (hipFuncSetAttribute / device query)");
    return launch_geometry_hist(f, means3D, opacities, shs, colors_precomp, scales, rotations, cov3D_precomp, splats, radii,
                                clamped, rects, depth_keys, block_sums, L.nblocks,
                                reinterpret_cast<uint32_t*>(base + L.table), reinterpret_cast<uint32_t*>(base + L.class_counts),
                                reinterpret_cast<uint32_t*>(base + L.len_hist), stream);
}

int launch_geometry_hist_binned_model(const FrameDev& f, int64_t R, const ScgModel& m, float* splats, int32_t* radii,
                                      uint8_t* clamped, uint32_t* rects, uint32_t* depth_keys, uint32_t* block_sums,
                                      void* bin_scratch, hipStream_t stream) {
    const TileBinningLayout L = tile_binning_layout(f.P, R, f.gx * f.gy);
    char* base = reinterpret_cast<char*>(bin_scratch);
    if (!device_setup()) return fail(SCG_E_RANGE, "tile binning: device setup failed (hipFuncSetAttribute / device query)");
    return launch_geometry_hist_model(f, m, splats, radii, clamped, rects, depth_keys, block_sums, L.nblocks,
                                      reinterpret_cast<uint32_t*>(base + L.table), reinterpret_cast<uint32_t*>(base + L.class_counts),
                                      reinterpret_cast<uint32_t*>(base + L.len_hist), stream);
}

int launch_tile_binning(const FrameDev& f, int64_t R, const uint32_t* rects, const uint32_t* depth_keys,
                        uint32_t* point_list, uint32_t* ranges, uint64_t* keys_sorted, void* scratch,
                        bool* defer_sort, bool hist_done, bool skip_rare, bool rare8, bool split_long, hipStream_t stream) {
    const int P = f.P;
    const int n_tiles = f.gx * f.gy;
    const TileBinningLayout L = tile_binning_layout(P, R, n_tiles);
    char* base = reinterpret_cast<char*>(scratch);
    uint32_t* table = reinterpret_cast<uint32_t*>(base + L.table);
    uint32_t* tile_total = reinterpret_cast<uint32_t*>(base + L.tile_total);
    uint32_t* tile_start = reinterpret_cast<uint32_t*>(base + L.tile_start);
    uint64_t* spill = reinterpret_cast<uint64_t*>(base + L.spill);
    uint32_t* class_counts = reinterpret_cast<uint32_t*>(base + L.class_counts);
    uint32_t* mid_tiles = reinterpret_cast<uint32_t*>(base + L.mid_tiles);
    uint32_t* big_tiles = reinterpret_cast<uint32_t*>(base + L.big_tiles);
    uint2* segments = reinterpret_cast<uint2*>(base + L.segments);
    uint32_t* len_hist = reinterpret_cast<uint32_t*>(base + L.len_hist);
    uint8_t* tile_class = reinterpret_cast<uint8_t*>(base + L.tile_class);
    uint32_t* tile_part = reinterpret_cast<uint32_t*>(base + L.tile_part);
    const uint2* rects2 = reinterpret_cast<const uint2*>(rects);
    uint2* ranges2 = reinterpret_cast<uint2*>(ranges);

    const DeviceSetup* ds = device_setup();
    if (!ds) return fail(SCG_E_RANGE, "tile binning: device setup failed (hipFuncSetAttribute / device query)");
    const int nb = L.nblocks;
    const bool dense = R / n_tiles >= kDenseMeanList;
    const bool deferred = defer_sort && *defer_sort && tile_binning_defers_sort(R, n_tiles) && !keys_sorted;
    if (defer_sort) *defer_sort = deferred;
    const size_t lds_tiles = (size_t)n_tiles * sizeof(uint32_t);
    if (!hist_done)
        hipLaunchKernelGGL(tile_hist_kernel, dim3(nb), dim3(kBinThreads), lds_tiles, stream, rects2, (uint32_t)P, f.gx,
                           n_tiles, table, class_counts, len_hist);
    int len_shift = 0;
    while (((R / n_tiles) >> len_shift) >= 32) ++len_shift;
    hipLaunchKernelGGL(table_colscan_kernel, dim3((n_tiles + kColTiles - 1) / kColTiles), dim3(kBinThreads), 0, stream,
                       table, nb, n_tiles, tile_total, len_hist, len_shift, f.cost_in, tile_class, tile_part);
    const size_t lds_band = ((size_t)((f.gy + kBands - 1) / kBands + 1) * f.gx + kWave) * sizeof(uint32_t);
    hipLaunchKernelGGL(tile_scatter_kernel, dim3(kBands + nb * kBands), dim3(kScatterThreads), lds_band, stream, rects2,
                       (uint32_t)P, f.gx, f.gy, nb, table, tile_total, tile_part, point_list, (uint32_t)R, tile_start, ranges2,
                       class_counts, mid_tiles, big_tiles,
                       (uint32_t)(deferred ? fused_max_list(R, n_tiles) : dense ? kSortDenseMax : kSortSmallMax), len_hist, tile_class,
                       f.cost_out, hist_done ? 1 : 0, f.bcost_in, f.nr_out);
    int id_bits = 8;
    while (id_bits < 32 && (1ll << id_bits) < (long long)P) id_bits += 8;
    if (deferred) {
    } else if (dense)
        hipLaunchKernelGGL((tile_sort_kernel<8, kSortDenseMax>), dim3(n_tiles), dim3(8 * kWave), 0, stream, ranges2,
                           depth_keys, point_list, id_bits);
    else
        hipLaunchKernelGGL((tile_sort_kernel<4, kSortSmallMax>), dim3(n_tiles), dim3(4 * kWave), 0, stream, ranges2,
                           depth_keys, point_list, id_bits);
    const int n_cus = ds->n_cus;
    if (!(deferred && skip_rare)) {
        if (rare8) {
            if (split_long)
                hipLaunchKernelGGL(tile_split_long_kernel, dim3(n_tiles < n_cus ? n_tiles : n_cus), dim3(kRareThreads), kRareLds,
                                   stream, ranges2, depth_keys, point_list, spill, spill + R, class_counts, mid_tiles, big_tiles,
                                   segments);
            hipLaunchKernelGGL(tile_sort_list8_kernel, dim3(3 * n_cus), dim3(kList8Threads), 0, stream, ranges2, depth_keys,
                               point_list, id_bits, spill, spill + R, class_counts, mid_tiles, big_tiles, segments,
                               split_long ? 1 : 0);
        } else {
            hipLaunchKernelGGL(tile_sort_rare_kernel, dim3(n_tiles < n_cus ? n_tiles : n_cus), dim3(kRareThreads), kRareLds,
                               stream, ranges2, depth_keys, point_list, id_bits, spill, spill + R, class_counts, mid_tiles,
                               big_tiles);
        }
    }
    if (keys_sorted) {
        const int kb = (int)((R + kBlock - 1) / kBlock);
        hipLaunchKernelGGL(rebuild_keys_kernel, dim3(kb), dim3(kBlock), 0, stream, tile_start, n_tiles, point_list,
                           depth_keys, R, keys_sorted);
    }
    return check_hip(hipGetLastError(), "tile binning");
}

}
```

scgaussian_amd/csrc/geometry.hip:

```cpp
#include "scg_common.h"
#include "tile_walk.h"

#include <type_traits>

#pragma clang fp contract(off)

namespace scg {

__constant__ const float kC0 = 0.28209479177387814f;
__constant__ const float kC1 = 0.4886025119029199f;
__constant__ const float kC2[5] = {1.0925484305920792f, -1.0925484305920792f, 0.31539156525252005f,
                                   -1.0925484305920792f, 0.5462742152960396f};
__constant__ const float kC3[7] = {-0.5900435899266435f, 2.890611442640554f, -0.4570457994644658f,
                                   0.3731763325901154f, -0.4570457994644658f, 1.445305721320277f,
                                   -0.5900435899266435f};

struct Mat16 { float m[16]; };

__device__ __forceinline__ Mat16 load16(const float* __restrict__ p) {
    Mat16 r;
#pragma unroll
    for (int i = 0; i < 16; ++i) r.m[i] = p[i];
    return r;
}

struct Proj {
    float tx, ty, tz;
    float hx, hy, m_w;
    float t_x, t_y;
    bool cl_x, cl_y;
    float cov[6];
    float T00, T01, T02, T10, T11, T12;
    float u0, u1, u2, v0, v1, v2;
    float A, B, C, det, det_inv;
    float L[9];
    float R[9];
};

struct GeoIn {
    float x, y, z, opacity;
    float a[7];
    float rgb[3];
};

template <bool WITH_RGB>
__device__ __forceinline__ GeoIn load_geo_in(int i, const float* __restrict__ means3D, const float* __restrict__ opacities,
                                             const float* __restrict__ colors_precomp, const float* __restrict__ scales,
                                             const float* __restrict__ rotations, const float* __restrict__ cov3D_precomp) {
    GeoIn g;
    g.x = means3D[3 * (size_t)i + 0];
    g.y = means3D[3 * (size_t)i + 1];
    g.z = means3D[3 * (size_t)i + 2];
    g.opacity = opacities[i];
    if (cov3D_precomp) {
#pragma unroll
        for (int k = 0; k < 6; ++k) g.a[k] = cov3D_precomp[6 * (size_t)i + k];
        g.a[6] = 0.f;
    } else {
        const float4 q = *reinterpret_cast<const float4*>(rotations + 4 * (size_t)i);
        g.a[0] = q.x; g.a[1] = q.y; g.a[2] = q.z; g.a[3] = q.w;
        g.a[4] = scales[3 * (size_t)i + 0];
        g.a[5] = scales[3 * (size_t)i + 1];
        g.a[6] = scales[3 * (size_t)i + 2];
    }
    if (WITH_RGB) {
        g.rgb[0] = colors_precomp[3 * (size_t)i + 0];
        g.rgb[1] = colors_precomp[3 * (size_t)i + 1];
        g.rgb[2] = colors_precomp[3 * (size_t)i + 2];
    } else {
        g.rgb[0] = g.rgb[1] = g.rgb[2] = 0.f;
    }
    return g;
}

__device__ __forceinline__ void cov3d_from_scale_rot(const GeoIn& g, float mod, Proj& p) {
    const float r = g.a[0], x = g.a[1], y = g.a[2], z = g.a[3];
    p.R[0] = 1.0f - 2.0f * (y * y + z * z);
    p.R[1] = 2.0f * (x * y - r * z);
    p.R[2] = 2.0f * (x * z + r * y);
    p.R[3] = 2.0f * (x * y + r * z);
    p.R[4] = 1.0f - 2.0f * (x * x + z * z);
    p.R[5] = 2.0f * (y * z - r * x);
    p.R[6] = 2.0f * (x * z - r * y);
    p.R[7] = 2.0f * (y * z + r * x);
    p.R[8] = 1.0f - 2.0f * (x * x + y * y);
    const float s0 = mod * g.a[4];
    const float s1 = mod * g.a[5];
    const float s2 = mod * g.a[6];
    float* L = p.L;
    L[0] = p.R[0] * s0; L[1] = p.R[1] * s1; L[2] = p.R[2] * s2;
    L[3] = p.R[3] * s0; L[4] = p.R[4] * s1; L[5] = p.R[5] * s2;
    L[6] = p.R[6] * s0; L[7] = p.R[7] * s1; L[8] = p.R[8] * s2;
    p.cov[0] = L[0] * L[0] + L[1] * L[1] + L[2] * L[2];
    p.cov[1] = L[0] * L[3] + L[1] * L[4] + L[2] * L[5];
    p.cov[2] = L[0] * L[6] + L[1] * L[7] + L[2] * L[8];
    p.cov[3] = L[3] * L[3] + L[4] * L[4] + L[5] * L[5];
    p.cov[4] = L[3] * L[6] + L[4] * L[7] + L[5] * L[8];
    p.cov[5] = L[6] * L[6] + L[7] * L[7] + L[8] * L[8];
}

__device__ __forceinline__ bool project(const FrameDev& f, const Mat16& V, const Mat16& PM, float x, float y,
                                        float z, Proj& p) {
    p.tx = V.m[0] * x + V.m[4] * y + V.m[8] * z + V.m[12];
    p.ty = V.m[1] * x + V.m[5] * y + V.m[9] * z + V.m[13];
    p.tz = V.m[2] * x + V.m[6] * y + V.m[10] * z + V.m[14];
    if (!(p.tz > kNearZ)) return false;
    p.hx = PM.m[0] * x + PM.m[4] * y + PM.m[8] * z + PM.m[12];
    p.hy = PM.m[1] * x + PM.m[5] * y + PM.m[9] * z + PM.m[13];
    const float hw = PM.m[3] * x + PM.m[7] * y + PM.m[11] * z + PM.m[15];
    p.m_w = 1.0f / (hw + 1e-7f);
    return true;
}

__device__ __forceinline__ void cov2d(const FrameDev& f, const Mat16& V, Proj& p) {
    const float txtz = p.tx / p.tz;
    const float tytz = p.ty / p.tz;
    p.cl_x = (txtz < -f.limx) || (txtz > f.limx);
    p.cl_y = (tytz < -f.limy) || (tytz > f.limy);
    p.t_x = fminf(fmaxf(txtz, -f.limx), f.limx) * p.tz;
    p.t_y = fminf(fmaxf(tytz, -f.limy), f.limy) * p.tz;
    const float tz2 = p.tz * p.tz;
    const float J00 = f.focal_x / p.tz;
    const float J02 = -(f.focal_x * p.t_x) / tz2;
    const float J11 = f.focal_y / p.tz;
    const float J12 = -(f.focal_y * p.t_y) / tz2;
    p.T00 = J00 * V.m[0] + J02 * V.m[2];
    p.T01 = J00 * V.m[4] + J02 * V.m[6];
    p.T02 = J00 * V.m[8] + J02 * V.m[10];
    p.T10 = J11 * V.m[1] + J12 * V.m[2];
    p.T11 = J11 * V.m[5] + J12 * V.m[6];
    p.T12 = J11 * V.m[9] + J12 * V.m[10];
    const float* c = p.cov;
    p.u0 = c[0] * p.T00 + c[1] * p.T01 + c[2] * p.T02;
    p.u1 = c[1] * p.T00 + c[3] * p.T01 + c[4] * p.T02;
    p.u2 = c[2] * p.T00 + c[4] * p.T01 + c[5] * p.T02;
    p.v0 = c[0] * p.T10 + c[1] * p.T11 + c[2] * p.T12;
    p.v1 = c[1] * p.T10 + c[3] * p.T11 + c[4] * p.T12;
    p.v2 = c[2] * p.T10 + c[4] * p.T11 + c[5] * p.T12;
    p.A = p.T00 * p.u0 + p.T01 * p.u1 + p.T02 * p.u2 + kLowpass;
    p.B = p.T00 * p.v0 + p.T01 * p.v1 + p.T02 * p.v2;
    p.C = p.T10 * p.v0 + p.T11 * p.v1 + p.T12 * p.v2 + kLowpass;
    p.det = p.A * p.C - p.B * p.B;
    p.det_inv = 1.0f / p.det;
}

template <int K>
__device__ __forceinline__ void load_sh(const float* __restrict__ rec, bool vec16, float* sh) {
    constexpr int n = 3 * K;
    if (vec16) {
        constexpr int nv = (n + 3) / 4;
        const float4* r4 = reinterpret_cast<const float4*>(rec);
#pragma unroll
        for (int i = 0; i < nv; ++i) {
            const float4 v = r4[i];
            sh[4 * i + 0] = v.x; sh[4 * i + 1] = v.y; sh[4 * i + 2] = v.z; sh[4 * i + 3] = v.w;
        }
    } else {
#pragma unroll
        for (int i = 0; i < n; ++i) sh[i] = rec[i];
#pragma unroll
        for (int i = n; i < (n + 3) / 4 * 4; ++i) sh[i] = 0.f;
    }
}

struct TensorSource {
    const float* means3D; const float* opacities; const float* shs; const float* colors_precomp;
    const float* scales; const float* rotations; const float* cov3D_precomp;
    int M, sh_vec16;
    __device__ __forceinline__ bool has_cov() const { return cov3D_precomp != nullptr; }
    template <bool WITH_RGB>
    __device__ __forceinline__ GeoIn load(int i) const {
        return load_geo_in<WITH_RGB>(i, means3D, opacities, colors_precomp, scales, rotations, cov3D_precomp);
    }
    template <int K>
    __device__ __forceinline__ void load_sh(int i, float* sh) const { scg::load_sh<K>(shs + (size_t)i * M * 3, sh_vec16 != 0, sh); }
};

constexpr float kNormalizeEps = 1e-12f;
__device__ __forceinline__ float act_opacity(float logit) { return 1.0f / (1.0f + expf(-logit)); }
__device__ __forceinline__ float act_scale(float log_s) { return expf(log_s); }
__device__ __forceinline__ float quat_denominator(float r, float x, float y, float z) {
    return fmaxf(sqrtf(r * r + x * x + y * y + z * z), kNormalizeEps);
}

constexpr int kRestCoeffs = 15;

struct ModelSource {
    ScgModel m;
    __device__ __forceinline__ bool has_cov() const { return false; }
    __device__ __forceinline__ bool locate(int i, int& j) const {
        const bool ray = i < m.ray.count;
        j = ray ? i : i - m.ray.count;
        return ray;
    }
    struct Raw { float o[3], d[3], zv, logit, ls[3]; float4 q; bool ray; };
    __device__ __forceinline__ Raw load_raw(int i) const {
        int j;
        Raw r;
        r.ray = locate(i, j);
        r.zv = 0.f; r.o[0] = r.o[1] = r.o[2] = 0.f;
        if (r.ray) {
            r.zv = m.ray.zval[j];
#pragma unroll
            for (int c = 0; c < 3; ++c) { r.o[c] = m.ray.rayo[3 * (size_t)j + c]; r.d[c] = m.ray.rayd[3 * (size_t)j + c]; }
        } else {
#pragma unroll
            for (int c = 0; c < 3; ++c) r.d[c] = m.bg.xyz[3 * (size_t)j + c];
        }
        const float* op = r.ray ? m.ray.opacity : m.bg.opacity;
        const float* sc = r.ray ? m.ray.scaling : m.bg.scaling;
        const float* ro = r.ray ? m.ray.rotation : m.bg.rotation;
        r.logit = op[j];
        r.q = *reinterpret_cast<const float4*>(ro + 4 * (size_t)j);
#pragma unroll
        for (int c = 0; c < 3; ++c) r.ls[c] = sc[3 * (size_t)j + c];
        return r;
    }
    static __device__ __forceinline__ GeoIn activate(const Raw& r, float* den_out = nullptr, float* rayd_out = nullptr) {
        GeoIn g;
        g.x = r.ray ? r.o[0] + r.d[0] * r.zv : r.d[0];
        g.y = r.ray ? r.o[1] + r.d[1] * r.zv : r.d[1];
        g.z = r.ray ? r.o[2] + r.d[2] * r.zv : r.d[2];
        g.opacity = act_opacity(r.logit);
        const float den = quat_denominator(r.q.x, r.q.y, r.q.z, r.q.w);
        g.a[0] = r.q.x / den; g.a[1] = r.q.y / den; g.a[2] = r.q.z / den; g.a[3] = r.q.w / den;
        g.a[4] = act_scale(r.ls[0]); g.a[5] = act_scale(r.ls[1]); g.a[6] = act_scale(r.ls[2]);
        g.rgb[0] = g.rgb[1] = g.rgb[2] = 0.f;
        if (den_out) *den_out = den;
        if (rayd_out) { rayd_out[0] = r.ray ? r.d[0] : 0.f; rayd_out[1] = r.ray ? r.d[1] : 0.f; rayd_out[2] = r.ray ? r.d[2] : 0.f; }
        return g;
    }
    template <bool WITH_RGB>
    __device__ __forceinline__ GeoIn load(int i) const { return activate(load_raw(i)); }
    template <int K>
    __device__ __forceinline__ void load_sh(int i, float* sh) const {
        int j;
        const bool ray = locate(i, j);
        const float* dc = (ray ? m.ray.features_dc : m.bg.features_dc) + 3 * (size_t)j;
        sh[0] = dc[0]; sh[1] = dc[1]; sh[2] = dc[2];
        if (K > 1) {
            const float* rest = (ray ? m.ray.features_rest : m.bg.features_rest) + 3 * kRestCoeffs * (size_t)j;
#pragma unroll
            for (int k = 0; k < 3 * (K - 1); ++k) sh[3 + k] = rest[k];
        }
#pragma unroll
        for (int k = 3 * K; k < (3 * K + 3) / 4 * 4; ++k) sh[k] = 0.f;
    }
};

template <int DEG>
__device__ __forceinline__ void eval_sh(const float* sh, float x, float y, float z, float* rgb) {
#pragma unroll
    for (int c = 0; c < 3; ++c) {
        float res = kC0 * sh[c];
        if (DEG > 0) {
            res = res - (kC1 * y) * sh[3 + c] + (kC1 * z) * sh[6 + c] - (kC1 * x) * sh[9 + c];
            if (DEG > 1) {
                const float xx = x * x, yy = y * y, zz = z * z;
                const float xy = x * y, yz = y * z, xz = x * z;
                res = res + (kC2[0] * xy) * sh[12 + c] + (kC2[1] * yz) * sh[15 + c] +
                      (kC2[2] * (2.0f * zz - xx - yy)) * sh[18 + c] + (kC2[3] * xz) * sh[21 + c] +
                      (kC2[4] * (xx - yy)) * sh[24 + c];
                if (DEG > 2) {
                    res = res + ((kC3[0] * y) * (3.0f * xx - yy)) * sh[27 + c] +
                          ((kC3[1] * xy) * z) * sh[30 + c] +
                          ((kC3[2] * y) * (4.0f * zz - xx - yy)) * sh[33 + c] +
                          ((kC3[3] * z) * (2.0f * zz - 3.0f * xx - 3.0f * yy)) * sh[36 + c] +
                          ((kC3[4] * x) * (4.0f * zz - xx - yy)) * sh[39 + c] +
                          ((kC3[5] * z) * (xx - yy)) * sh[42 + c] +
                          ((kC3[6] * x) * (xx - 3.0f * yy)) * sh[45 + c];
                }
            }
        }
        rgb[c] = res;
    }
}

constexpr int kStageVec = 4 * kWave;

__device__ __forceinline__ void flush_stage(const float4* stage, int first, int P, float4* __restrict__ splats,
                                            int32_t* __restrict__ radii, uint8_t* __restrict__ clamped,
                                            uint2* __restrict__ rects, uint32_t* __restrict__ depth_keys) {
    const int lane = lane_id();
    __builtin_amdgcn_fence(__ATOMIC_RELEASE, "wavefront");
    __builtin_amdgcn_wave_barrier();
    __builtin_amdgcn_fence(__ATOMIC_ACQUIRE, "wavefront");
    const int n = min(kWave, P - first);
    float4* dst = splats + 3 * (size_t)first;
#pragma unroll
    for (int k = 0; k < 3; ++k) {
        const int idx = k * kWave + lane;
        if (idx < 3 * n) dst[idx] = stage[idx];
    }
    if (lane < n) {
        const uint4 u = reinterpret_cast<const uint4*>(stage + 3 * kWave)[lane];
        const float tz = stage[3 * lane + 2].w;
        const int i = first + lane;
        radii[i] = (int32_t)u.x;
        clamped[i] = (uint8_t)u.y;
        rects[i] = make_uint2(u.z, u.w);
        depth_keys[i] = u.x ? __float_as_uint(tz) : 0xFFFFFFFFu;
    }
    __builtin_amdgcn_fence(__ATOMIC_RELEASE, "wavefront");
    __builtin_amdgcn_wave_barrier();
}

template <int DEG, class Src, class Between>
__device__ __forceinline__ uint32_t geometry_forward_one(
    const FrameDev& f, const Mat16& V, const Mat16& PM, int i, bool valid, const GeoIn& in,
    const Src& src, float4* stage , Between&& between
#ifdef SCG_PROBE_TIMELINE
    , uint32_t* g_tp
#endif
    ) {
    uint32_t my_tiles = 0;
    float4 sa = make_float4(0.f, 0.f, 0.f, 0.f), sb = sa, sc = sa;
    int radius_i = 0;
    uint8_t clamp_bits = 0;
    uint2 rect = make_uint2(0u, 0u);
    float px = 0.f, py = 0.f, con_a = 0.f, con_b = 0.f, con_c = 0.f, tz = 0.f;

    Proj p;
    bool ok = valid && project(f, V, PM, in.x, in.y, in.z, p);
    if (ok) {
        if (src.has_cov()) {
#pragma unroll
            for (int k = 0; k < 6; ++k) p.cov[k] = in.a[k];
        } else {
            cov3d_from_scale_rot(in, f.mod, p);
        }
        cov2d(f, V, p);
        ok = (p.det != 0.0f);
    }
    if (ok) {
        con_a = p.C * p.det_inv;
        con_b = -p.B * p.det_inv;
        con_c = p.A * p.det_inv;
        const float mid = 0.5f * (p.A + p.C);
        const float lam1 = mid + sqrtf(fmaxf(mid * mid - p.det, 0.1f));
        const float radius_f = ceilf(3.0f * sqrtf(lam1));
        const float ndc_x = p.hx * p.m_w;
        const float ndc_y = p.hy * p.m_w;
        px = ((ndc_x + 1.0f) * (float)f.W - 1.0f) * 0.5f;
        py = ((ndc_y + 1.0f) * (float)f.H - 1.0f) * 0.5f;
        int minx, miny, maxx, maxy;
        tile_rect(px, py, radius_f, f.gx, f.gy, minx, miny, maxx, maxy);
        const int tiles = (maxx - minx) * (maxy - miny);
        ok = tiles > 0;
        if (ok) {
            my_tiles = (uint32_t)tiles;
            radius_i = (int)fminf(fmaxf(radius_f, 0.0f), 2.0e9f);
            rect = make_uint2((uint32_t)minx | ((uint32_t)miny << 16),
                              (uint32_t)(maxx - minx) | ((uint32_t)(maxy - miny) << 16));
            tz = p.tz;
        }
    }
    constexpr bool has_colors = DEG < 0;
    constexpr int K = has_colors ? 1 : (DEG + 1) * (DEG + 1);
    float sh[(3 * K + 3) / 4 * 4];
#ifdef SCG_PROBE_TIMELINE
    { float pin = con_a; asm volatile("" : "+v"(pin)); }
    const uint32_t tp_math = (uint32_t)wall_clock64();
#endif
    if (!has_colors) src.template load_sh<K>(ok ? i : 0, sh);
    between(rect);
#ifdef SCG_PROBE_TIMELINE
    const uint32_t tp_between = (uint32_t)wall_clock64();
    asm volatile("" : "+v"(sh[0]), "+v"(sh[(3 * K + 3) / 4 * 4 - 1]));
    const uint32_t tp_sh = (uint32_t)wall_clock64();
    g_tp[0] += tp_math - g_tp[4]; g_tp[1] += tp_between - tp_math; g_tp[2] += tp_sh - tp_between; g_tp[4] = tp_sh;
#endif
    if (ok) {
        float rgb[3];
        if (has_colors) {
            rgb[0] = in.rgb[0]; rgb[1] = in.rgb[1]; rgb[2] = in.rgb[2];
        } else {
            float dx = in.x - f.campos[0], dy = in.y - f.campos[1], dz = in.z - f.campos[2];
            const float len = sqrtf(dx * dx + dy * dy + dz * dz);
            dx = dx / len; dy = dy / len; dz = dz / len;
            eval_sh<(DEG < 0 ? 0 : DEG)>(sh, dx, dy, dz, rgb);
#pragma unroll
            for (int c = 0; c < 3; ++c) {
                rgb[c] = rgb[c] + 0.5f;
                if (rgb[c] < 0.0f) { clamp_bits |= (uint8_t)(1u << c); rgb[c] = 0.0f; }
            }
        }
        sa = make_float4(px, py, con_a, con_b);
        const float opa = in.opacity;
        sb = make_float4(con_c, opa, 2.0f * logf(255.0f * opa) * 1.001f + 0.01f, -con_b / con_c);
        sc = make_float4(rgb[0], rgb[1], rgb[2], tz);
    }
    const int lane = lane_id();
    stage[3 * lane + 0] = sa;
    stage[3 * lane + 1] = sb;
    stage[3 * lane + 2] = sc;
    reinterpret_cast<uint4*>(stage + 3 * kWave)[lane] = make_uint4((uint32_t)radius_i, (uint32_t)clamp_bits, rect.x, rect.y);
    return my_tiles;
}

template <int DEG, class Src>
__device__ __forceinline__ void geometry_forward_body(
    const FrameDev& f, const Src& src, float4* __restrict__ splats,
    int32_t* __restrict__ radii, uint8_t* __restrict__ clamped, uint2* __restrict__ rects,
    uint32_t* __restrict__ depth_keys, uint32_t* __restrict__ block_sums) {
    __shared__ uint32_t s_wave_sum[kBlock / kWave];
    __shared__ float4 s_stage[(kBlock / kWave) * kStageVec];
    const int i = blockIdx.x * kBlock + threadIdx.x;
    const bool valid = i < f.P;
    const GeoIn in = src.template load<(DEG < 0)>(valid ? i : f.P - 1);
    const Mat16 V = load16(f.view);
    const Mat16 PM = load16(f.proj);
    float4* stage = s_stage + kStageVec * wave_id();
#ifdef SCG_PROBE_TIMELINE
    uint32_t tp_dummy[5] = {0u, 0u, 0u, 0u, 0u};
#endif
    const uint32_t my_tiles = geometry_forward_one<DEG>(f, V, PM, i, valid, in, src, stage,
                                                        [](uint2) {}
#ifdef SCG_PROBE_TIMELINE
                                                        , tp_dummy
#endif
                                                        );
    flush_stage(stage, i - lane_id(), f.P, splats, radii, clamped, rects, depth_keys);

    uint32_t s = my_tiles;
#pragma unroll
    for (int off = 32; off > 0; off >>= 1) s += __shfl_down(s, off, kWave);
    if (lane_id() == 0) s_wave_sum[wave_id()] = s;
    __syncthreads();
    if (threadIdx.x == 0) block_sums[blockIdx.x] = s_wave_sum[0] + s_wave_sum[1] + s_wave_sum[2] + s_wave_sum[3];
}

template <int DEG>
__global__ __launch_bounds__(kBlock) void geometry_forward_kernel(
    FrameDev f, const float* __restrict__ means3D, const float* __restrict__ opacities,
    const float* __restrict__ shs, const float* __restrict__ colors_precomp, const float* __restrict__ scales,
    const float* __restrict__ rotations, const float* __restrict__ cov3D_precomp, float4* __restrict__ splats,
    int32_t* __restrict__ radii, uint8_t* __restrict__ clamped, uint2* __restrict__ rects,
    uint32_t* __restrict__ depth_keys, uint32_t* __restrict__ block_sums, int sh_vec16) {
    const TensorSource src{means3D, opacities, shs, colors_precomp, scales, rotations, cov3D_precomp, f.M, sh_vec16};
    geometry_forward_body<DEG>(f, src, splats, radii, clamped, rects, depth_keys, block_sums);
}

template <int DEG>
__global__ __launch_bounds__(kBlock) void geometry_forward_model_kernel(
    FrameDev f, ScgModel model, float4* __restrict__ splats, int32_t* __restrict__ radii, uint8_t* __restrict__ clamped,
    uint2* __restrict__ rects, uint32_t* __restrict__ depth_keys, uint32_t* __restrict__ block_sums) {
    const ModelSource src{model};
    geometry_forward_body<DEG>(f, src, splats, radii, clamped, rects, depth_keys, block_sums);
}

__host__ __device__ __forceinline__ size_t geometry_hist_stage_offset(int n_tiles, int max_blocks) {
    return ((size_t)(n_tiles + max_blocks) * sizeof(uint32_t) + 15) & ~(size_t)15;
}
__host__ __device__ __forceinline__ size_t geometry_hist_lds_bytes(int n_tiles, int max_blocks) {
    return geometry_hist_stage_offset(n_tiles, max_blocks) + (size_t)(kBinThreads / kWave) * kStageVec * sizeof(float4);
}

template <int DEG, class Src>
__device__ __forceinline__ void geometry_hist_body(
    const FrameDev& f, const Src& src, float4* __restrict__ splats,
    int32_t* __restrict__ radii, uint8_t* __restrict__ clamped, uint2* __restrict__ rects,
    uint32_t* __restrict__ depth_keys, uint32_t* __restrict__ block_sums,
    uint32_t* __restrict__ table, uint32_t* __restrict__ class_counts, uint32_t* __restrict__ len_hist, int max_blocks) {
    extern __shared__ __attribute__((aligned(16))) unsigned char smem[];
    uint32_t* hist = reinterpret_cast<uint32_t*>(smem);
    const int n_tiles = f.gx * f.gy;
    uint32_t* s_blk = hist + n_tiles;
    float4* stage = reinterpret_cast<float4*>(smem + geometry_hist_stage_offset(n_tiles, max_blocks)) + kStageVec * wave_id();
    uint32_t blk_a, blk_b;
    block_slice((uint32_t)f.P, gridDim.x, blockIdx.x, blk_a, blk_b);
    const int lane = lane_id();
    uint32_t chunk = 4u * blk_a + (uint32_t)wave_id();
    auto fetch = [&](uint32_t c) {
        const int g = (int)(c * kWave) + lane;
        return src.template load<(DEG < 0)>(min(g, f.P - 1));
    };
    const Mat16 V = load16(f.view);
    const Mat16 PM = load16(f.proj);
    if (blockIdx.x == 0) {
        if (threadIdx.x < 4) class_counts[threadIdx.x] = 0u;
        len_hist[threadIdx.x] = 0u;
    }
    for (int t = threadIdx.x; t < n_tiles + max_blocks; t += kBinThreads) hist[t] = 0;
    uint32_t* next_chunk = s_blk + (max_blocks - 1);
    __syncthreads();
    if (threadIdx.x == 0) *next_chunk = 4u * blk_a + (uint32_t)kBinWaves;
    __syncthreads();
    int pending = -1;
#ifdef SCG_PROBE_TIMELINE
    uint32_t g_tp[5] = {0u, 0u, 0u, 0u, (uint32_t)wall_clock64()};
    const uint32_t tp_begin = g_tp[4];
    uint32_t tp_iters = 0;
#endif
    while (chunk < 4u * blk_b) {
        const int i = (int)(chunk * kWave) + lane;
        const GeoIn in = fetch(chunk);
        uint32_t grabbed = 0;
        if (lane == 0) grabbed = atomicAdd(next_chunk, 1u);
        const uint32_t my_tiles = geometry_forward_one<DEG>(
            f, V, PM, i, i < f.P, in, src, stage, [&](uint2 rect) {
                if (pending >= 0) flush_stage(stage, pending, f.P, splats, radii, clamped, rects, depth_keys);
                walk_rects(rect, (uint32_t)i, f.gx, [&](uint32_t tile, uint32_t) { atomicAdd(&hist[tile], 1u); });
            }
#ifdef SCG_PROBE_TIMELINE
            , g_tp
#endif
            );
#ifdef SCG_PROBE_TIMELINE
        { const uint32_t t = (uint32_t)wall_clock64(); g_tp[3] += t - g_tp[4]; g_tp[4] = t; ++tp_iters; }
#endif
        pending = i - lane;
        uint32_t s = my_tiles;
#pragma unroll
        for (int off = 32; off > 0; off >>= 1) s += __shfl_down(s, off, kWave);
        if (lane == 0 && s) atomicAdd(&s_blk[(chunk >> 2) - blk_a], s);
        chunk = (uint32_t)__builtin_amdgcn_readfirstlane((int)grabbed);
    }
    if (pending >= 0) flush_stage(stage, pending, f.P, splats, radii, clamped, rects, depth_keys);
#ifdef SCG_PROBE_TIMELINE
    const uint32_t tp_loop_end = (uint32_t)wall_clock64();
#endif
    __syncthreads();
#ifdef SCG_PROBE_TIMELINE
    if (f.cost_out && lane == 0) {
        uint32_t* tl = f.cost_out + n_tiles + 65792 + ((size_t)blockIdx.x * kBinWaves + wave_id()) * 8;
        tl[0] = tp_begin; tl[1] = g_tp[0]; tl[2] = g_tp[1]; tl[3] = g_tp[2]; tl[4] = g_tp[3]; tl[5] = tp_loop_end;
        tl[6] = (uint32_t)wall_clock64(); tl[7] = 0xC0FFEE00u | tp_iters;
    }
#endif
    uint32_t* row = table + (size_t)blockIdx.x * n_tiles;
    for (int t = threadIdx.x; t < n_tiles; t += kBinThreads) row[t] = hist[t];
    for (uint32_t k = threadIdx.x; k < blk_b - blk_a; k += kBinThreads) block_sums[blk_a + k] = s_blk[k];
}

template <int DEG>
__global__ __launch_bounds__(kBinThreads) void geometry_hist_kernel(
    FrameDev f, const float* __restrict__ means3D, const float* __restrict__ opacities,
    const float* __restrict__ shs, const float* __restrict__ colors_precomp, const float* __restrict__ scales,
    const float* __restrict__ rotations, const float* __restrict__ cov3D_precomp, float4* __restrict__ splats,
    int32_t* __restrict__ radii, uint8_t* __restrict__ clamped, uint2* __restrict__ rects,
    uint32_t* __restrict__ depth_keys, uint32_t* __restrict__ block_sums, int sh_vec16,
    uint32_t* __restrict__ table, uint32_t* __restrict__ class_counts, uint32_t* __restrict__ len_hist, int max_blocks) {
    const TensorSource src{means3D, opacities, shs, colors_precomp, scales, rotations, cov3D_precomp, f.M, sh_vec16};
    geometry_hist_body<DEG>(f, src, splats, radii, clamped, rects, depth_keys, block_sums, table, class_counts, len_hist, max_blocks);
}

template <int DEG>
__global__ __launch_bounds__(kBinThreads) void geometry_hist_model_kernel(
    FrameDev f, ScgModel model, float4* __restrict__ splats, int32_t* __restrict__ radii, uint8_t* __restrict__ clamped,
    uint2* __restrict__ rects, uint32_t* __restrict__ depth_keys, uint32_t* __restrict__ block_sums,
    uint32_t* __restrict__ table, uint32_t* __restrict__ class_counts, uint32_t* __restrict__ len_hist, int max_blocks) {
    const ModelSource src{model};
    geometry_hist_body<DEG>(f, src, splats, radii, clamped, rects, depth_keys, block_sums, table, class_counts, len_hist, max_blocks);
}

template <int DEG>
__device__ __forceinline__ void sh_basis_grads(float x, float y, float z, float* basis, float* bx, float* by, float* bz) {
    basis[0] = kC0; bx[0] = by[0] = bz[0] = 0.f;
    if (DEG > 0) {
        basis[1] = -kC1 * y; bx[1] = 0.f; by[1] = -kC1; bz[1] = 0.f;
        basis[2] = kC1 * z;  bx[2] = 0.f; by[2] = 0.f; bz[2] = kC1;
        basis[3] = -kC1 * x; bx[3] = -kC1; by[3] = 0.f; bz[3] = 0.f;
    }
    if (DEG > 1) {
        const float xx = x * x, yy = y * y, zz = z * z, xy = x * y, yz = y * z, xz = x * z;
        basis[4] = kC2[0] * xy;                    bx[4] = kC2[0] * y; by[4] = kC2[0] * x; bz[4] = 0.f;
        basis[5] = kC2[1] * yz;                    bx[5] = 0.f; by[5] = kC2[1] * z; bz[5] = kC2[1] * y;
        basis[6] = kC2[2] * (2.0f * zz - xx - yy); bx[6] = kC2[2] * -2.0f * x; by[6] = kC2[2] * -2.0f * y; bz[6] = kC2[2] * 4.0f * z;
        basis[7] = kC2[3] * xz;                    bx[7] = kC2[3] * z; by[7] = 0.f; bz[7] = kC2[3] * x;
        basis[8] = kC2[4] * (xx - yy);             bx[8] = kC2[4] * 2.0f * x; by[8] = kC2[4] * -2.0f * y; bz[8] = 0.f;
        if (DEG > 2) {
            basis[9] = kC3[0] * y * (3.0f * xx - yy);
            bx[9] = kC3[0] * 6.0f * xy; by[9] = kC3[0] * (3.0f * xx - 3.0f * yy); bz[9] = 0.f;
            basis[10] = kC3[1] * xy * z;
            bx[10] = kC3[1] * yz; by[10] = kC3[1] * xz; bz[10] = kC3[1] * xy;
            basis[11] = kC3[2] * y * (4.0f * zz - xx - yy);
            bx[11] = kC3[2] * -2.0f * xy; by[11] = kC3[2] * (4.0f * zz - xx - 3.0f * yy); bz[11] = kC3[2] * 8.0f * yz;
            basis[12] = kC3[3] * z * (2.0f * zz - 3.0f * xx - 3.0f * yy);
            bx[12] = kC3[3] * -6.0f * xz; by[12] = kC3[3] * -6.0f * yz; bz[12] = kC3[3] * (6.0f * zz - 3.0f * xx - 3.0f * yy);
            basis[13] = kC3[4] * x * (4.0f * zz - xx - yy);
            bx[13] = kC3[4] * (4.0f * zz - 3.0f * xx - yy); by[13] = kC3[4] * -2.0f * xy; bz[13] = kC3[4] * 8.0f * xz;
            basis[14] = kC3[5] * z * (xx - yy);
            bx[14] = kC3[5] * 2.0f * xz; by[14] = kC3[5] * -2.0f * yz; bz[14] = kC3[5] * (xx - yy);
            basis[15] = kC3[6] * x * (xx - 3.0f * yy);
            bx[15] = kC3[6] * (3.0f * xx - 3.0f * yy); by[15] = kC3[6] * -6.0f * xy; bz[15] = 0.f;
        }
    }
}

template <int DEG, bool STREAM = false>
__device__ __forceinline__ void sh_backward(const float* rec, bool vec16, float x, float y, float z,
                                            const float* dRGB, float* dsh_rec, int M,
                                            float& ddx, float& ddy, float& ddz, bool acc,
                                            int sw = -1) {
    auto at = [&](int j) { return sw < 0 ? j : ((((j >> 2) ^ sw) << 2) | (j & 3)); };
    constexpr int K = (DEG + 1) * (DEG + 1);
    float sh[STREAM ? 3 : (3 * K + 3) / 4 * 4];
    if (!STREAM) load_sh<K>(rec, vec16, sh);
    float basis[K];
    float bx[K], by[K], bz[K];
    sh_basis_grads<DEG>(x, y, z, basis, bx, by, bz);
    ddx = ddy = ddz = 0.f;
#pragma unroll
    for (int k = 0; k < K; ++k) {
        float s0, s1, s2;
        if (STREAM) { s0 = rec[at(3 * k)]; s1 = rec[at(3 * k + 1)]; s2 = rec[at(3 * k + 2)]; }
        else { s0 = sh[3 * k]; s1 = sh[3 * k + 1]; s2 = sh[3 * k + 2]; }
        const float g = s0 * dRGB[0] + s1 * dRGB[1] + s2 * dRGB[2];
        ddx += g * bx[k]; ddy += g * by[k]; ddz += g * bz[k];
        if (acc) {
            dsh_rec[at(3 * k + 0)] += basis[k] * dRGB[0];
            dsh_rec[at(3 * k + 1)] += basis[k] * dRGB[1];
            dsh_rec[at(3 * k + 2)] += basis[k] * dRGB[2];
        } else {
            dsh_rec[at(3 * k + 0)] = basis[k] * dRGB[0];
            dsh_rec[at(3 * k + 1)] = basis[k] * dRGB[1];
            dsh_rec[at(3 * k + 2)] = basis[k] * dRGB[2];
        }
    }
    if (!acc)
        for (int k = 3 * K; k < 3 * M; ++k) dsh_rec[at(k)] = 0.f;
}

__device__ __forceinline__ void geometry_backward_one(const FrameDev& f, const Mat16& V, const Mat16& PM, const GeoIn& in,
                                                      bool has_cov, float4& ga, float4& gb, float* dm, float* dm2, float& d_op,
                                                      float* ds, float* dq, float* dcov) {
    const float x = in.x, y = in.y, z = in.z;
    const float opac = in.opacity;
    d_op = (opac > 0.0f) ? ga.w / opac : 0.0f;

    Proj p;
    project(f, V, PM, x, y, z, p);
    if (has_cov) {
#pragma unroll
        for (int k = 0; k < 6; ++k) p.cov[k] = in.a[k];
    } else {
        cov3d_from_scale_rot(in, f.mod, p);
    }
    cov2d(f, V, p);
    {
        const float con_a = p.C * p.det_inv, con_b = -p.B * p.det_inv, con_c = p.A * p.det_inv;
        const float sx = ga.x, sy = ga.y;
        ga.x = -(con_a * sx + con_b * sy);
        ga.y = -(con_b * sx + con_c * sy);
        gb.x *= -0.5f; gb.y = -gb.y; gb.z *= -0.5f;
    }

    const float di2 = p.det_inv * p.det_inv;
    const float dA = di2 * (-p.C * p.C * gb.x + p.B * p.C * gb.y - p.B * p.B * gb.z);
    const float dC = di2 * (-p.B * p.B * gb.x + p.A * p.B * gb.y - p.A * p.A * gb.z);
    const float dB = di2 * (2.0f * p.B * p.C * gb.x - (p.A * p.C + p.B * p.B) * gb.y + 2.0f * p.A * p.B * gb.z);

    const float T0[3] = {p.T00, p.T01, p.T02};
    const float T1[3] = {p.T10, p.T11, p.T12};
    float Ms[9];
#pragma unroll
    for (int j = 0; j < 3; ++j)
#pragma unroll
        for (int k = 0; k < 3; ++k)
            Ms[3 * j + k] = dA * T0[j] * T0[k] + 0.5f * dB * (T0[j] * T1[k] + T1[j] * T0[k]) + dC * T1[j] * T1[k];
    const float u[3] = {p.u0, p.u1, p.u2};
    const float v[3] = {p.v0, p.v1, p.v2};
    float dT0[3], dT1[3];
#pragma unroll
    for (int k = 0; k < 3; ++k) {
        dT0[k] = 2.0f * dA * u[k] + dB * v[k];
        dT1[k] = dB * u[k] + 2.0f * dC * v[k];
    }
    const float dJ00 = dT0[0] * V.m[0] + dT0[1] * V.m[4] + dT0[2] * V.m[8];
    const float dJ02 = dT0[0] * V.m[2] + dT0[1] * V.m[6] + dT0[2] * V.m[10];
    const float dJ11 = dT1[0] * V.m[1] + dT1[1] * V.m[5] + dT1[2] * V.m[9];
    const float dJ12 = dT1[0] * V.m[2] + dT1[1] * V.m[6] + dT1[2] * V.m[10];
    const float itz = 1.0f / p.tz;
    const float itz2 = itz * itz;
    const float itz3 = itz2 * itz;
    const float dtx = p.cl_x ? 0.f : -f.focal_x * itz2 * dJ02;
    const float dty = p.cl_y ? 0.f : -f.focal_y * itz2 * dJ12;
    float dtz = -f.focal_x * itz2 * dJ00 - f.focal_y * itz2 * dJ11 +
                2.0f * f.focal_x * p.t_x * itz3 * dJ02 + 2.0f * f.focal_y * p.t_y * itz3 * dJ12;
    dtz += ga.z;
#pragma unroll
    for (int j = 0; j < 3; ++j)
        dm[j] = V.m[4 * j] * dtx + V.m[4 * j + 1] * dty + V.m[4 * j + 2] * dtz;

    const float dndc_x = ga.x * 0.5f * (float)f.W;
    const float dndc_y = ga.y * 0.5f * (float)f.H;
    dm2[0] = dndc_x; dm2[1] = dndc_y;
    const float mw2 = p.m_w * p.m_w;
#pragma unroll
    for (int j = 0; j < 3; ++j) {
        dm[j] += (PM.m[4 * j] * p.m_w - PM.m[4 * j + 3] * p.hx * mw2) * dndc_x +
                 (PM.m[4 * j + 1] * p.m_w - PM.m[4 * j + 3] * p.hy * mw2) * dndc_y;
    }

    if (has_cov) {
        dcov[0] = Ms[0]; dcov[1] = 2.0f * Ms[1]; dcov[2] = 2.0f * Ms[2];
        dcov[3] = Ms[4]; dcov[4] = 2.0f * Ms[5]; dcov[5] = Ms[8];
    } else {
        const float* L = p.L;
        const float* R = p.R;
        const float S[3] = {f.mod * in.a[4], f.mod * in.a[5], f.mod * in.a[6]};
        float dL[9];
#pragma unroll
        for (int a = 0; a < 3; ++a)
#pragma unroll
            for (int b = 0; b < 3; ++b)
                dL[3 * a + b] = 2.0f * (Ms[3 * a + 0] * L[0 + b] + Ms[3 * a + 1] * L[3 + b] + Ms[3 * a + 2] * L[6 + b]);
        float dR[9];
#pragma unroll
        for (int b = 0; b < 3; ++b) {
            ds[b] = f.mod * (dL[b] * R[b] + dL[3 + b] * R[3 + b] + dL[6 + b] * R[6 + b]);
            dR[b] = dL[b] * S[b]; dR[3 + b] = dL[3 + b] * S[b]; dR[6 + b] = dL[6 + b] * S[b];
        }
        const float r = in.a[0], qx = in.a[1], qy = in.a[2], qz = in.a[3];
        dq[0] = 2.0f * (-qz * dR[1] + qy * dR[2] + qz * dR[3] - qx * dR[5] - qy * dR[6] + qx * dR[7]);
        dq[1] = 2.0f * (qy * dR[1] + qz * dR[2] + qy * dR[3] - 2.0f * qx * dR[4] - r * dR[5] + qz * dR[6] + r * dR[7] - 2.0f * qx * dR[8]);
        dq[2] = 2.0f * (-2.0f * qy * dR[0] + qx * dR[1] + r * dR[2] + qx * dR[3] + qz * dR[5] - r * dR[6] + qz * dR[7] - 2.0f * qy * dR[8]);
        dq[3] = 2.0f * (-2.0f * qz * dR[0] - r * dR[1] + qx * dR[2] + r * dR[3] - 2.0f * qz * dR[4] + qy * dR[5] + qx * dR[6] + qy * dR[7]);
    }
}

constexpr int kShVec = 12;
constexpr int kShSlot = 13;

template <bool STAGED, int BLOCK, bool STAGE_IN = STAGED>
__global__ __launch_bounds__(BLOCK) void geometry_backward_kernel(
    FrameDev f, const float* __restrict__ means3D, const float* __restrict__ opacities,
    const float* __restrict__ shs, const float* __restrict__ colors_precomp, const float* __restrict__ scales,
    const float* __restrict__ rotations, const float* __restrict__ cov3D_precomp,
    const int32_t* __restrict__ radii, const uint8_t* __restrict__ clamped, const float4* __restrict__ dsplats,
    float* __restrict__ dmeans3D, float* __restrict__ dmeans2D, float* __restrict__ dopac,
    float* __restrict__ dshs, float* __restrict__ dcolors, float* __restrict__ dscales, float* __restrict__ drots,
    float* __restrict__ dcov3D, int sh_vec16, int flags) {
    const int accumulate = flags & SCG_BACKWARD_ACCUMULATE;
    const int live_pieces = (flags & SCG_BACKWARD_SH_TAIL_ZERO) ? (3 * (f.D + 1) * (f.D + 1) + 3) / 4 : kShVec;
    constexpr int kSlot = (BLOCK == kWave) ? kShVec : kShSlot;
    constexpr int RECS = (BLOCK == kWave) ? 60 : BLOCK;
    __shared__ float4 s_sh[STAGED ? RECS * kSlot : 1];
    constexpr bool kSwizzle = (BLOCK == kWave);
    auto slot_piece = [&](int idx) {
        const int r = idx / kShVec, pc = idx % kShVec;
        return r * kSlot + (kSwizzle ? (pc ^ ((r >> 2) & 3)) : pc);
    };
    const int sw = kSwizzle ? (((int)threadIdx.x >> 2) & 3) : -1;
    const int block_first = blockIdx.x * RECS;
    const bool owner = (int)threadIdx.x < RECS;
    const int i = owner ? block_first + (int)threadIdx.x : f.P;
    const int n_vec = min(RECS, f.P - block_first) * kShVec;
    if (!STAGED && i >= f.P) return;
    constexpr bool stage_sh = STAGED && STAGE_IN;
    float4 stage[stage_sh ? kShVec : 1];
    if (stage_sh) {
        const float4* src = reinterpret_cast<const float4*>(shs) + (size_t)block_first * kShVec;
#pragma unroll
        for (int k = 0; k < kShVec; ++k) stage[k] = src[min(k * BLOCK + (int)threadIdx.x, n_vec - 1)];
    }
    const int ic = min(i, f.P - 1);
    int radius = radii[ic];
    GeoIn in = load_geo_in<false>(ic, means3D, opacities, nullptr, scales, rotations, cov3D_precomp);
    constexpr int kRec = SCG_DSPLAT_FLOATS / 4;
    float4 ga = dsplats[kRec * (size_t)ic + 0];
    float4 gb = dsplats[kRec * (size_t)ic + 1];
    float4 gc = dsplats[kRec * (size_t)ic + 2];
    uint8_t cb = clamped[ic];
    const Mat16 V = load16(f.view);
    const Mat16 PM = load16(f.proj);
    float cam_x = f.campos[0], cam_y = f.campos[1], cam_z = f.campos[2];
    __builtin_amdgcn_sched_barrier(0);
    if (STAGED) {
        if (stage_sh) {
#pragma unroll
            for (int k = 0; k < kShVec; ++k)
                s_sh[slot_piece(min(k * BLOCK + (int)threadIdx.x, n_vec - 1))] = stage[k];
        }
    }
    {
        int rr = radius, cc = cb;
        asm volatile("" : "+v"(rr), "+v"(cc), "+v"(ga.x), "+v"(ga.y), "+v"(ga.z), "+v"(ga.w), "+v"(gb.x), "+v"(gb.y), "+v"(gb.z));
        radius = rr; cb = (uint8_t)cc;
        asm volatile("" : "+v"(gc.x), "+v"(gc.y), "+v"(gc.z), "+v"(in.x), "+v"(in.y), "+v"(in.z), "+v"(in.opacity));
        asm volatile("" : "+v"(in.a[0]), "+v"(in.a[1]), "+v"(in.a[2]), "+v"(in.a[3]), "+v"(in.a[4]), "+v"(in.a[5]), "+v"(in.a[6]));
        asm volatile("" : "+v"(cam_x), "+v"(cam_y), "+v"(cam_z));
    }
    if (STAGED) __syncthreads();
    float* my_slot = reinterpret_cast<float*>(&s_sh[STAGED ? min((int)threadIdx.x, RECS - 1) * kSlot : 0]);

    float dm[3] = {0.f, 0.f, 0.f};
    float dm2[2] = {0.f, 0.f};
    float d_op = 0.f;
    float ds[3] = {0.f, 0.f, 0.f};
    float dq[4] = {0.f, 0.f, 0.f, 0.f};
    float dcov[6] = {0.f, 0.f, 0.f, 0.f, 0.f, 0.f};
    float dcol[3] = {0.f, 0.f, 0.f};
    bool sh_written = false;

    if (i < f.P && radius > 0) {
        const float x = in.x, y = in.y, z = in.z;
        geometry_backward_one(f, V, PM, in, cov3D_precomp != nullptr, ga, gb, dm, dm2, d_op, ds, dq, dcov);

        if (colors_precomp) {
            dcol[0] = gc.x; dcol[1] = gc.y; dcol[2] = gc.z;
        } else {
            const float dRGB[3] = {(cb & 1) ? 0.f : gc.x, (cb & 2) ? 0.f : gc.y, (cb & 4) ? 0.f : gc.z};
            float dx = x - cam_x, dy = y - cam_y, dz = z - cam_z;
            const float len = sqrtf(dx * dx + dy * dy + dz * dz);
            const float ilen = 1.0f / len;
            dx *= ilen; dy *= ilen; dz *= ilen;
            float gx_ = 0.f, gy_ = 0.f, gz_ = 0.f;
            const float* rec = stage_sh ? my_slot : shs + (size_t)i * f.M * 3;
            float* drec = STAGED ? my_slot : dshs + (size_t)i * f.M * 3;
            switch (f.D) {
                case 0: sh_backward<0>(rec, sh_vec16, dx, dy, dz, dRGB, drec, f.M, gx_, gy_, gz_, !STAGED && accumulate,
                                        STAGED ? sw : -1); break;
                case 1: sh_backward<1>(rec, sh_vec16, dx, dy, dz, dRGB, drec, f.M, gx_, gy_, gz_, !STAGED && accumulate,
                                        STAGED ? sw : -1); break;
                case 2: sh_backward<2>(rec, sh_vec16, dx, dy, dz, dRGB, drec, f.M, gx_, gy_, gz_, !STAGED && accumulate,
                                        STAGED ? sw : -1); break;
                default: sh_backward<3, stage_sh>(rec, sh_vec16, dx, dy, dz, dRGB, drec, f.M, gx_, gy_, gz_, !STAGED && accumulate,
                                                STAGED ? sw : -1); break;
            }
            sh_written = true;
            const float dot = dx * gx_ + dy * gy_ + dz * gz_;
            dm[0] += (gx_ - dx * dot) * ilen;
            dm[1] += (gy_ - dy * dot) * ilen;
            dm[2] += (gz_ - dz * dot) * ilen;
        }
    }

    if (STAGED) {
        if (!sh_written && owner) {
#pragma unroll
            for (int k = 0; k < kShVec; ++k) s_sh[threadIdx.x * kSlot + k] = make_float4(0.f, 0.f, 0.f, 0.f);
        }
        __syncthreads();
        float4* dst = reinterpret_cast<float4*>(dshs) + (size_t)block_first * kShVec;
#pragma unroll
        for (int k = 0; k < kShVec; ++k) {
            const int idx = k * BLOCK + (int)threadIdx.x;
            if (idx < n_vec && idx % kShVec < live_pieces) {
                float4 v = s_sh[slot_piece(idx)];
                if (accumulate) {
                    const float4 o = dst[idx];
                    v.x += o.x; v.y += o.y; v.z += o.z; v.w += o.w;
                }
                dst[idx] = v;
            }
        }
        __syncthreads();
        float* sm = reinterpret_cast<float*>(s_sh);
        constexpr int kArr = 3 * RECS;
        if (owner) {
#pragma unroll
            for (int c = 0; c < 3; ++c) {
                sm[3 * threadIdx.x + c] = dm[c];
                sm[kArr + 3 * threadIdx.x + c] = c < 2 ? dm2[c] : 0.f;
                sm[2 * kArr + 3 * threadIdx.x + c] = ds[c];
            }
        }
        __syncthreads();
        const int n3 = 3 * min(RECS, f.P - block_first);
        float* o_m3 = dmeans3D + 3 * (size_t)block_first;
        float* o_m2 = dmeans2D + 3 * (size_t)block_first;
        float* o_sc = dscales ? dscales + 3 * (size_t)block_first : nullptr;
#pragma unroll
        for (int k = 0; k < (kArr + BLOCK - 1) / BLOCK; ++k) {
            const int idx = k * BLOCK + (int)threadIdx.x;
            if (idx < n3) {
                float v = sm[idx], w = sm[2 * kArr + idx];
                if (accumulate) {
                    v += o_m3[idx];
                    if (o_sc) w += o_sc[idx];
                }
                o_m3[idx] = v;
                o_m2[idx] = sm[kArr + idx];
                if (o_sc) o_sc[idx] = w;
            }
        }
        if (i >= f.P) return;
    } else if (dshs && !sh_written && !accumulate) {
        float* drec = dshs + (size_t)i * f.M * 3;
        for (int k = 0; k < 3 * f.M; ++k) drec[k] = 0.f;
    }
    if (!STAGED) {
        dmeans2D[3 * (size_t)i + 0] = dm2[0];
        dmeans2D[3 * (size_t)i + 1] = dm2[1];
        dmeans2D[3 * (size_t)i + 2] = 0.f;
    }
    if (accumulate) {
        if (radius <= 0) return;
        if (!STAGED) {
            dm[0] += dmeans3D[3 * (size_t)i + 0]; dm[1] += dmeans3D[3 * (size_t)i + 1]; dm[2] += dmeans3D[3 * (size_t)i + 2];
        }
        d_op += dopac[i];
        if (dcolors) {
            dcol[0] += dcolors[3 * (size_t)i + 0]; dcol[1] += dcolors[3 * (size_t)i + 1]; dcol[2] += dcolors[3 * (size_t)i + 2];
        }
        if (dscales) {
            if (!STAGED) {
                ds[0] += dscales[3 * (size_t)i + 0]; ds[1] += dscales[3 * (size_t)i + 1]; ds[2] += dscales[3 * (size_t)i + 2];
            }
            const float4 o = *reinterpret_cast<const float4*>(drots + 4 * (size_t)i);
            dq[0] += o.x; dq[1] += o.y; dq[2] += o.z; dq[3] += o.w;
        }
        if (dcov3D) {
#pragma unroll
            for (int k = 0; k < 6; ++k) dcov[k] += dcov3D[6 * (size_t)i + k];
        }
    }
    if (!STAGED) {
        dmeans3D[3 * (size_t)i + 0] = dm[0];
        dmeans3D[3 * (size_t)i + 1] = dm[1];
        dmeans3D[3 * (size_t)i + 2] = dm[2];
    }
    dopac[i] = d_op;
    if (dcolors) {
        dcolors[3 * (size_t)i + 0] = dcol[0]; dcolors[3 * (size_t)i + 1] = dcol[1]; dcolors[3 * (size_t)i + 2] = dcol[2];
    }
    if (dscales) {
        if (!STAGED) {
            dscales[3 * (size_t)i + 0] = ds[0]; dscales[3 * (size_t)i + 1] = ds[1]; dscales[3 * (size_t)i + 2] = ds[2];
        }
        *reinterpret_cast<float4*>(drots + 4 * (size_t)i) = make_float4(dq[0], dq[1], dq[2], dq[3]);
    }
    if (dcov3D) {
#pragma unroll
        for (int k = 0; k < 6; ++k) dcov3D[6 * (size_t)i + k] = dcov[k];
    }
}

constexpr int kModelRecs = 60;
constexpr int kRestFloats = 3 * kRestCoeffs;
constexpr int kRestVecs = kModelRecs * kRestFloats / 4;
constexpr int kRestRounds = (kRestVecs + kWave - 1) / kWave;
constexpr int kDcVecs = kModelRecs * 3 / 4;

template <int DEG, bool STREAM>
__device__ __forceinline__ void sh_backward_model(const float* sh, float* dc_t, float* rest_t, float x, float y, float z,
                                                  const float* dRGB, float& ddx, float& ddy, float& ddz) {
    constexpr int K = (DEG + 1) * (DEG + 1);
    float basis[K], bx[K], by[K], bz[K];
    sh_basis_grads<DEG>(x, y, z, basis, bx, by, bz);
    ddx = ddy = ddz = 0.f;
#pragma unroll
    for (int k = 0; k < K; ++k) {
        float* slot = (k == 0) ? dc_t : rest_t + 3 * (k - 1);
        float s0, s1, s2;
        if (STREAM) { s0 = slot[0]; s1 = slot[1]; s2 = slot[2]; }
        else { s0 = sh[3 * k]; s1 = sh[3 * k + 1]; s2 = sh[3 * k + 2]; }
        const float g = s0 * dRGB[0] + s1 * dRGB[1] + s2 * dRGB[2];
        ddx += g * bx[k]; ddy += g * by[k]; ddz += g * bz[k];
        slot[0] = basis[k] * dRGB[0];
        slot[1] = basis[k] * dRGB[1];
        slot[2] = basis[k] * dRGB[2];
    }
    if (DEG > 0)
        for (int w = 3 * (K - 1); w < kRestFloats; ++w) rest_t[w] = 0.f;
}

template <bool STAGE_IN>
__global__ __launch_bounds__(kWave) __attribute__((amdgpu_waves_per_eu(4, 4))) void geometry_backward_model_kernel(
    FrameDev f, ScgModel m, ScgModelGrads g, const int32_t* __restrict__ radii, const uint8_t* __restrict__ clamped,
    const float4* __restrict__ dsplats, float* __restrict__ dmeans2D, int flags, int blocks_ray) {
    __shared__ float4 s_rest4[kRestVecs];
    __shared__ float4 s_dc4[kDcVecs];
    float* s_rest = reinterpret_cast<float*>(s_rest4);
    float* s_dc = reinterpret_cast<float*>(s_dc4);
    const bool accumulate = (flags & SCG_BACKWARD_ACCUMULATE) != 0;
    const bool skip_tail = (flags & (SCG_BACKWARD_ACCUMULATE | SCG_BACKWARD_SH_TAIL_ZERO)) != 0;
    const bool ray = (int)blockIdx.x < blocks_ray;
    const ScgModelSet set = ray ? m.ray : m.bg;
    const ScgModelGradSet gs = ray ? g.ray : g.bg;
    const int first = ((int)blockIdx.x - (ray ? 0 : blocks_ray)) * kModelRecs;
    const int n = min(kModelRecs, set.count - first);
    const int t = (int)threadIdx.x;
    const bool owner = t < n;
    const int j = first + min(t, n - 1);
    const int i = (ray ? 0 : m.ray.count) + j;
    const int n_rest = n * kRestFloats, nv = n_rest >> 2;
    const int n_dc = n * 3, nvd = n_dc >> 2;
    const int K = (f.D + 1) * (f.D + 1);
    const int active = 3 * (K - 1);
    const ModelSource src{m};

    const bool full = n == kModelRecs;
    if constexpr (STAGE_IN) {
        typedef const __attribute__((address_space(1))) void* gptr_t;
        typedef __attribute__((address_space(3))) void* lptr_t;
        if (full) {
            const float4* src4 = reinterpret_cast<const float4*>(set.features_rest + (size_t)first * kRestFloats);
#pragma unroll
            for (int k = 0; k < kRestRounds - 1; ++k)
                __builtin_amdgcn_global_load_lds((gptr_t)(src4 + k * kWave + t), (lptr_t)(s_rest4 + k * kWave), 16, 0, 0);
            if ((kRestRounds - 1) * kWave + t < kRestVecs)
                __builtin_amdgcn_global_load_lds((gptr_t)(src4 + (kRestRounds - 1) * kWave + t),
                                                 (lptr_t)(s_rest4 + (kRestRounds - 1) * kWave), 16, 0, 0);
            if (t < kDcVecs)
                __builtin_amdgcn_global_load_lds((gptr_t)(reinterpret_cast<const float4*>(set.features_dc + (size_t)first * 3) + t),
                                                 (lptr_t)s_dc4, 16, 0, 0);
        } else {
            for (int w = t; w < n_rest; w += kWave) s_rest[w] = set.features_rest[(size_t)first * kRestFloats + w];
            for (int w = t; w < n_dc; w += kWave) s_dc[w] = set.features_dc[(size_t)first * 3 + w];
        }
    }
    int radius = radii[i];
    ModelSource::Raw raw = src.load_raw(i);
    constexpr int kRec = SCG_DSPLAT_FLOATS / 4;
    float4 ga = dsplats[kRec * (size_t)i + 0];
    float4 gb = dsplats[kRec * (size_t)i + 1];
    float4 gc = dsplats[kRec * (size_t)i + 2];
    uint8_t cb = clamped[i];
    const Mat16 V = load16(f.view);
    const Mat16 PM = load16(f.proj);
    float cam_x = f.campos[0], cam_y = f.campos[1], cam_z = f.campos[2];
    __builtin_amdgcn_sched_barrier(0);
    {
        int rr = radius, cc = cb;
        asm volatile("" : "+v"(rr), "+v"(cc), "+v"(ga.x), "+v"(ga.y), "+v"(ga.z), "+v"(ga.w), "+v"(gb.x), "+v"(gb.y), "+v"(gb.z));
        radius = rr; cb = (uint8_t)cc;
        asm volatile("" : "+v"(gc.x), "+v"(gc.y), "+v"(gc.z), "+v"(raw.zv), "+v"(raw.logit), "+v"(raw.q.x), "+v"(raw.q.y), "+v"(raw.q.z), "+v"(raw.q.w));
        asm volatile("" : "+v"(raw.o[0]), "+v"(raw.o[1]), "+v"(raw.o[2]), "+v"(raw.d[0]), "+v"(raw.d[1]), "+v"(raw.d[2]));
        asm volatile("" : "+v"(raw.ls[0]), "+v"(raw.ls[1]), "+v"(raw.ls[2]), "+v"(cam_x), "+v"(cam_y), "+v"(cam_z));
    }
    __syncthreads();
    float den;
    const GeoIn in = ModelSource::activate(raw, &den);
    float* dc_t = s_dc + 3 * min(t, kModelRecs - 1);
    float* rest_t = s_rest + kRestFloats * min(t, kModelRecs - 1);

    float dm[3] = {0.f, 0.f, 0.f};
    float dm2[2] = {0.f, 0.f};
    float d_op = 0.f;
    float ds[3] = {0.f, 0.f, 0.f};
    float dq[4] = {0.f, 0.f, 0.f, 0.f};
    float dcov[6];
    bool sh_written = false;
    const bool visible = owner && radius > 0;
    if (visible) {
        geometry_backward_one(f, V, PM, in, false, ga, gb, dm, dm2, d_op, ds, dq, dcov);
        d_op = d_op * in.opacity * (1.0f - in.opacity);
        ds[0] *= in.a[4]; ds[1] *= in.a[5]; ds[2] *= in.a[6];
        {
            const bool clamped_norm = !(den > kNormalizeEps);
            const float dotq = clamped_norm ? 0.f : in.a[0] * dq[0] + in.a[1] * dq[1] + in.a[2] * dq[2] + in.a[3] * dq[3];
#pragma unroll
            for (int k = 0; k < 4; ++k) dq[k] = (dq[k] - in.a[k] * dotq) / den;
        }
        const float dRGB[3] = {(cb & 1) ? 0.f : gc.x, (cb & 2) ? 0.f : gc.y, (cb & 4) ? 0.f : gc.z};
        float dx = in.x - cam_x, dy = in.y - cam_y, dz = in.z - cam_z;
        const float len = sqrtf(dx * dx + dy * dy + dz * dz);
        const float ilen = 1.0f / len;
        dx *= ilen; dy *= ilen; dz *= ilen;
        float gx_ = 0.f, gy_ = 0.f, gz_ = 0.f;
        if constexpr (STAGE_IN) {
            sh_backward_model<3, true>(nullptr, dc_t, rest_t, dx, dy, dz, dRGB, gx_, gy_, gz_);
        } else {
            switch (f.D) {
                case 0: { float sh[4]; src.load_sh<1>(i, sh); sh_backward_model<0, false>(sh, dc_t, rest_t, dx, dy, dz, dRGB, gx_, gy_, gz_); break; }
                case 1: { float sh[12]; src.load_sh<4>(i, sh); sh_backward_model<1, false>(sh, dc_t, rest_t, dx, dy, dz, dRGB, gx_, gy_, gz_); break; }
                default: { float sh[28]; src.load_sh<9>(i, sh); sh_backward_model<2, false>(sh, dc_t, rest_t, dx, dy, dz, dRGB, gx_, gy_, gz_); break; }
            }
        }
        sh_written = true;
        const float dot = dx * gx_ + dy * gy_ + dz * gz_;
        dm[0] += (gx_ - dx * dot) * ilen;
        dm[1] += (gy_ - dy * dot) * ilen;
        dm[2] += (gz_ - dz * dot) * ilen;
    }
    if (owner && !sh_written) {
        dc_t[0] = dc_t[1] = dc_t[2] = 0.f;
        if (f.D > 0)
            for (int w = 0; w < kRestFloats; ++w) rest_t[w] = 0.f;
    }
    float d_zval = 0.f;
    if (ray)
        d_zval = set.rayd[3 * (size_t)j + 0] * dm[0] + set.rayd[3 * (size_t)j + 1] * dm[1] + set.rayd[3 * (size_t)j + 2] * dm[2];
    const float d_logit = d_op;
    const float* d_ls = ds;
    const float* d_q = dq;

    __syncthreads();
    {
        float4* dst = reinterpret_cast<float4*>(gs.features_dc + (size_t)first * 3);
        if (t < nvd) {
            float4 v = s_dc4[t];
            if (accumulate) { const float4 o = dst[t]; v.x += o.x; v.y += o.y; v.z += o.z; v.w += o.w; }
            dst[t] = v;
        }
        if (4 * nvd + t < n_dc) {
            float* d1 = gs.features_dc + (size_t)first * 3 + 4 * nvd + t;
            *d1 = s_dc[4 * nvd + t] + (accumulate ? *d1 : 0.f);
        }
    }
    if (f.D > 0 || !skip_tail) {
        float4* dst = reinterpret_cast<float4*>(gs.features_rest + (size_t)first * kRestFloats);
        const bool zeros = f.D == 0;
#pragma unroll
        for (int k = 0; k < kRestRounds; ++k) {
            const int idx = k * kWave + t;
            const int w0 = (4 * idx) % kRestFloats;
            const bool live = !skip_tail || w0 < active || w0 + 3 >= kRestFloats;
            if (idx < nv && live) {
                float4 v = zeros ? make_float4(0.f, 0.f, 0.f, 0.f) : s_rest4[idx];
                if (accumulate) { const float4 o = dst[idx]; v.x += o.x; v.y += o.y; v.z += o.z; v.w += o.w; }
                dst[idx] = v;
            }
        }
        if (4 * nv + t < n_rest) {
            float* d1 = gs.features_rest + (size_t)first * kRestFloats + 4 * nv + t;
            *d1 = (zeros ? 0.f : s_rest[4 * nv + t]) + (accumulate ? *d1 : 0.f);
        }
    }
    __syncthreads();
    constexpr int kArr = 3 * kModelRecs;
    if (owner) {
#pragma unroll
        for (int c = 0; c < 3; ++c) {
            s_rest[3 * t + c] = dm[c];
            s_rest[kArr + 3 * t + c] = c < 2 ? dm2[c] : 0.f;
            s_rest[2 * kArr + 3 * t + c] = d_ls[c];
        }
    }
    __syncthreads();
    {
        float* o_xyz = ray ? nullptr : gs.xyz + 3 * (size_t)first;
        float* o_m2 = dmeans2D + 3 * ((size_t)(ray ? 0 : m.ray.count) + first);
        float* o_sc = gs.scaling + 3 * (size_t)first;
#pragma unroll
        for (int k = 0; k < (kArr + kWave - 1) / kWave; ++k) {
            const int idx = k * kWave + t;
            if (idx < n_dc) {
                float v = s_rest[idx], w = s_rest[2 * kArr + idx];
                if (accumulate) {
                    if (o_xyz) v += o_xyz[idx];
                    w += o_sc[idx];
                }
                if (o_xyz) o_xyz[idx] = v;
                o_m2[idx] = s_rest[kArr + idx];
                o_sc[idx] = w;
            }
        }
    }
    if (!owner) return;
    if (accumulate) {
        if (ray) gs.zval[j] += d_zval;
        gs.opacity[j] += d_logit;
        float4* dr = reinterpret_cast<float4*>(gs.rotation + 4 * (size_t)j);
        const float4 o = *dr;
        *dr = make_float4(o.x + d_q[0], o.y + d_q[1], o.z + d_q[2], o.w + d_q[3]);
    } else {
        if (ray) gs.zval[j] = d_zval;
        gs.opacity[j] = d_logit;
        *reinterpret_cast<float4*>(gs.rotation + 4 * (size_t)j) = make_float4(d_q[0], d_q[1], d_q[2], d_q[3]);
    }
}

__global__ __launch_bounds__(kBlock) void model_activate_kernel(ScgModel m, int P, float* __restrict__ means3D,
                                                                float* __restrict__ opacities, float* __restrict__ scales,
                                                                float* __restrict__ rotations) {
    const int i = blockIdx.x * kBlock + threadIdx.x;
    if (i >= P) return;
    const ModelSource src{m};
    const GeoIn in = src.load<false>(i);
    if (means3D) { means3D[3 * (size_t)i] = in.x; means3D[3 * (size_t)i + 1] = in.y; means3D[3 * (size_t)i + 2] = in.z; }
    if (opacities) opacities[i] = in.opacity;
    if (scales) { scales[3 * (size_t)i] = in.a[4]; scales[3 * (size_t)i + 1] = in.a[5]; scales[3 * (size_t)i + 2] = in.a[6]; }
    if (rotations) *reinterpret_cast<float4*>(rotations + 4 * (size_t)i) = make_float4(in.a[0], in.a[1], in.a[2], in.a[3]);
}

static inline bool aligned16(const void* p) { return (reinterpret_cast<uintptr_t>(p) & 15u) == 0; }

template <class F>
static inline void by_degree(int deg, F&& f) {
    switch (deg) {
        case -1: f(std::integral_constant<int, -1>()); break;
        case 0: f(std::integral_constant<int, 0>()); break;
        case 1: f(std::integral_constant<int, 1>()); break;
        case 2: f(std::integral_constant<int, 2>()); break;
        default: f(std::integral_constant<int, 3>()); break;
    }
}

int launch_geometry_forward(const FrameDev& f, const float* means3D, const float* opacities, const float* shs,
                            const float* colors_precomp, const float* scales, const float* rotations,
                            const float* cov3D_precomp, float* splats, int32_t* radii, uint8_t* clamped,
                            uint32_t* rects, uint32_t* depth_keys, uint32_t* block_sums, hipStream_t stream) {
    const int blocks = (f.P + kBlock - 1) / kBlock;
    const int vec16 = (shs && aligned16(shs) && ((f.M * 3 * 4) % 16 == 0)) ? 1 : 0;
    by_degree(colors_precomp ? -1 : f.D, [&](auto deg) {
        hipLaunchKernelGGL(geometry_forward_kernel<decltype(deg)::value>, dim3(blocks), dim3(kBlock), 0, stream, f, means3D,
                           opacities, shs, colors_precomp, scales, rotations, cov3D_precomp, reinterpret_cast<float4*>(splats),
                           radii, clamped, reinterpret_cast<uint2*>(rects), depth_keys, block_sums, vec16);
    });
    return check_hip(hipGetLastError(), "geometry_forward_kernel");
}

hipError_t geometry_hist_set_max_lds(int bytes) {
    hipError_t rc = hipSuccess;
    for (int deg = -1; deg <= 3; ++deg)
        by_degree(deg, [&](auto d) {
            const hipError_t e = hipFuncSetAttribute(reinterpret_cast<const void*>(geometry_hist_kernel<decltype(d)::value>),
                                                     hipFuncAttributeMaxDynamicSharedMemorySize, bytes);
            if (e != hipSuccess) rc = e;
        });
    return rc;
}

int launch_geometry_hist(const FrameDev& f, const float* means3D, const float* opacities, const float* shs,
                         const float* colors_precomp, const float* scales, const float* rotations,
                         const float* cov3D_precomp, float* splats, int32_t* radii, uint8_t* clamped, uint32_t* rects,
                         uint32_t* depth_keys, uint32_t* block_sums, int nblocks, uint32_t* table, uint32_t* class_counts,
                         uint32_t* len_hist, hipStream_t stream) {
    const int vec16 = (shs && aligned16(shs) && ((f.M * 3 * 4) % 16 == 0)) ? 1 : 0;
    const int n_tiles = f.gx * f.gy;
    const int nb256 = (f.P + kBlock - 1) / kBlock;
    const int max_blocks = nb256 / nblocks + 2;
    const size_t lds = geometry_hist_lds_bytes(n_tiles, max_blocks);
    by_degree(colors_precomp ? -1 : f.D, [&](auto deg) {
        hipLaunchKernelGGL(geometry_hist_kernel<decltype(deg)::value>, dim3(nblocks), dim3(kBinThreads), lds, stream, f, means3D,
                           opacities, shs, colors_precomp, scales, rotations, cov3D_precomp, reinterpret_cast<float4*>(splats),
                           radii, clamped, reinterpret_cast<uint2*>(rects), depth_keys, block_sums, vec16, table, class_counts,
                           len_hist, max_blocks);
    });
    return check_hip(hipGetLastError(), "geometry_hist_kernel");
}

int launch_geometry_backward(const FrameDev& f, const float* means3D, const float* opacities, const float* shs,
                             const float* colors_precomp, const float* scales, const float* rotations,
                             const float* cov3D_precomp, const int32_t* radii, const uint8_t* clamped,
                             const float* dsplats, float* dmeans3D, float* dmeans2D, float* dopac, float* dshs,
                             float* dcolors, float* dscales, float* drots, float* dcov3D, int flags,
                             hipStream_t stream) {
    const int vec16 = (shs && aligned16(shs) && ((f.M * 3 * 4) % 16 == 0)) ? 1 : 0;
    const bool staged = vec16 && dshs && aligned16(dshs) && f.M == 16;
    const int block = staged ? kWave : kBlock;
    const int recs = staged ? 60 : kBlock;
    const int blocks = (f.P + recs - 1) / recs;
    auto kernel = !staged ? geometry_backward_kernel<false, kBlock>
                          : (f.D >= 3 ? geometry_backward_kernel<true, kWave, true> : geometry_backward_kernel<true, kWave, false>);
    hipLaunchKernelGGL(kernel, dim3(blocks), dim3(block), 0, stream, f, means3D, opacities, shs, colors_precomp, scales, rotations,
                       cov3D_precomp, radii, clamped, reinterpret_cast<const float4*>(dsplats), dmeans3D, dmeans2D, dopac,
                       dshs, dcolors, dscales, drots, dcov3D, vec16, flags);
    return check_hip(hipGetLastError(), "geometry_backward_kernel");
}

int launch_geometry_forward_model(const FrameDev& f, const ScgModel& m, float* splats, int32_t* radii, uint8_t* clamped,
                                  uint32_t* rects, uint32_t* depth_keys, uint32_t* block_sums, hipStream_t stream) {
    const int blocks = (f.P + kBlock - 1) / kBlock;
    by_degree(f.D, [&](auto deg) {
        hipLaunchKernelGGL(geometry_forward_model_kernel<decltype(deg)::value>, dim3(blocks), dim3(kBlock), 0, stream, f, m,
                           reinterpret_cast<float4*>(splats), radii, clamped, reinterpret_cast<uint2*>(rects), depth_keys,
                           block_sums);
    });
    return check_hip(hipGetLastError(), "geometry_forward_model_kernel");
}

hipError_t geometry_hist_model_set_max_lds(int bytes) {
    hipError_t rc = hipSuccess;
    for (int deg = 0; deg <= 3; ++deg)
        by_degree(deg, [&](auto d) {
            const hipError_t e = hipFuncSetAttribute(reinterpret_cast<const void*>(geometry_hist_model_kernel<decltype(d)::value>),
                                                     hipFuncAttributeMaxDynamicSharedMemorySize, bytes);
            if (e != hipSuccess) rc = e;
        });
    return rc;
}

int launch_geometry_hist_model(const FrameDev& f, const ScgModel& m, float* splats, int32_t* radii, uint8_t* clamped,
                               uint32_t* rects, uint32_t* depth_keys, uint32_t* block_sums, int nblocks, uint32_t* table,
                               uint32_t* class_counts, uint32_t* len_hist, hipStream_t stream) {
    const int n_tiles = f.gx * f.gy;
    const int nb256 = (f.P + kBlock - 1) / kBlock;
    const int max_blocks = nb256 / nblocks + 2;
    const size_t lds = geometry_hist_lds_bytes(n_tiles, max_blocks);
    by_degree(f.D, [&](auto deg) {
        hipLaunchKernelGGL(geometry_hist_model_kernel<decltype(deg)::value>, dim3(nblocks), dim3(kBinThreads), lds, stream, f, m,
                           reinterpret_cast<float4*>(splats), radii, clamped, reinterpret_cast<uint2*>(rects), depth_keys,
                           block_sums, table, class_counts, len_hist, max_blocks);
    });
    return check_hip(hipGetLastError(), "geometry_hist_model_kernel");
}

int launch_geometry_backward_model(const FrameDev& f, const ScgModel& m, const ScgModelGrads& g, const int32_t* radii,
                                   const uint8_t* clamped, const float* dsplats, float* dmeans2D, int flags, hipStream_t stream) {
    const int blocks_ray = (m.ray.count + kModelRecs - 1) / kModelRecs;
    const int blocks_bg = (m.bg.count + kModelRecs - 1) / kModelRecs;
    if (blocks_ray + blocks_bg == 0) return 0;
    auto kernel = f.D >= 3 ? geometry_backward_model_kernel<true> : geometry_backward_model_kernel<false>;
    hipLaunchKernelGGL(kernel, dim3(blocks_ray + blocks_bg), dim3(kWave), 0, stream, f, m, g, radii, clamped,
                       reinterpret_cast<const float4*>(dsplats), dmeans2D, flags, blocks_ray);
    return check_hip(hipGetLastError(), "geometry_backward_model_kernel");
}

int launch_model_activate(const ScgModel& m, float* means3D, float* opacities, float* scales, float* rotations,
                          hipStream_t stream) {
    const int P = m.ray.count + m.bg.count;
    if (P == 0) return 0;
    hipLaunchKernelGGL(model_activate_kernel, dim3((P + kBlock - 1) / kBlock), dim3(kBlock), 0, stream, m, P, means3D, opacities,
                       scales, rotations);
    return check_hip(hipGetLastError(), "model_activate_kernel");
}

}
```

scgaussian_amd/csrc/scg_common.h:

```cpp
#pragma once

#include <hip/hip_runtime.h>
#include <hip/hip_ext.h>
#include <stdint.h>

#include "../../include/scg_raster.h"

namespace scg {

constexpr int kWave = 64;
constexpr int kTile = SCG_TILE;
constexpr int kTilePix = kTile * kTile;
constexpr int kBlock = 256;

constexpr float kNearZ = 0.2f;
constexpr float kLowpass = 0.3f;
constexpr float kAlphaMin = 1.0f / 255.0f;
constexpr float kAlphaMax = 0.99f;
constexpr float kTEps = 1e-4f;

struct FrameDev {
    int P, D, M, W, H;
    int gx, gy;
    float tanfovx, tanfovy, focal_x, focal_y, limx, limy, mod;
    const float* view;
    const float* proj;
    const float* campos;
    const float* bg;
    const uint32_t* cost_in;
    uint32_t* cost_out;
    uint32_t* long_out;
    const uint32_t* bcost_in;
    uint32_t* bcost_out;
    uint32_t* nr_out;
};

inline FrameDev make_frame_dev(const ScgFrame* f) {
    FrameDev d;
    d.P = f->P; d.D = f->sh_degree; d.M = f->sh_coeffs; d.W = f->width; d.H = f->height;
    d.gx = (f->width + kTile - 1) / kTile;
    d.gy = (f->height + kTile - 1) / kTile;
    d.tanfovx = f->tanfovx; d.tanfovy = f->tanfovy;
    d.focal_x = (float)f->width / (2.0f * f->tanfovx);
    d.focal_y = (float)f->height / (2.0f * f->tanfovy);
    d.limx = 1.3f * f->tanfovx;
    d.limy = 1.3f * f->tanfovy;
    d.mod = f->scale_modifier;
    d.view = f->viewmatrix; d.proj = f->projmatrix; d.campos = f->campos; d.bg = f->bg;
    d.cost_in = f->tile_cost_in; d.cost_out = f->tile_cost_out; d.long_out = f->long_lists_out;
    d.bcost_in = f->bwd_cost_in; d.bcost_out = f->bwd_cost_out;
    d.nr_out = f->num_rendered_out;
    return d;
}

int fail(int code, const char* fmt, ...);
int check_hip(hipError_t e, const char* what);
int validate_frame(const ScgFrame* f, bool need_bg);

int launch_geometry_forward(const FrameDev& f, const float* means3D, const float* opacities, const float* shs,
                            const float* colors_precomp, const float* scales, const float* rotations,
                            const float* cov3D_precomp, float* splats, int32_t* radii, uint8_t* clamped,
                            uint32_t* rects, uint32_t* depth_keys, uint32_t* block_sums, hipStream_t stream);
int launch_geometry_backward(const FrameDev& f, const float* means3D, const float* opacities, const float* shs,
                             const float* colors_precomp, const float* scales, const float* rotations,
                             const float* cov3D_precomp, const int32_t* radii, const uint8_t* clamped,
                             const float* dsplats, float* dmeans3D, float* dmeans2D, float* dopac, float* dshs,
                             float* dcolors, float* dscales, float* drots, float* dcov3D, int flags ,
                             hipStream_t stream);
int launch_geometry_forward_model(const FrameDev& f, const ScgModel& m, float* splats, int32_t* radii, uint8_t* clamped,
                                  uint32_t* rects, uint32_t* depth_keys, uint32_t* block_sums, hipStream_t stream);
int launch_geometry_hist_model(const FrameDev& f, const ScgModel& m, float* splats, int32_t* radii, uint8_t* clamped,
                               uint32_t* rects, uint32_t* depth_keys, uint32_t* block_sums, int nblocks, uint32_t* table,
                               uint32_t* class_counts, uint32_t* len_hist, hipStream_t stream);
int launch_geometry_hist_binned_model(const FrameDev& f, int64_t R, const ScgModel& m, float* splats, int32_t* radii,
                                      uint8_t* clamped, uint32_t* rects, uint32_t* depth_keys, uint32_t* block_sums,
                                      void* bin_scratch, hipStream_t stream);
hipError_t geometry_hist_model_set_max_lds(int bytes);
int launch_geometry_backward_model(const FrameDev& f, const ScgModel& m, const ScgModelGrads& g, const int32_t* radii,
                                   const uint8_t* clamped, const float* dsplats, float* dmeans2D, int flags, hipStream_t stream);
int launch_model_activate(const ScgModel& m, float* means3D, float* opacities, float* scales, float* rotations,
                          hipStream_t stream);

size_t scan_scratch_bytes(int64_t n);
int launch_inclusive_scan(const uint32_t* in, uint32_t* out, int64_t n, uint32_t* total_out, void* scratch,
                          hipStream_t stream);

size_t sort_scratch_bytes(int64_t n);
int launch_sort_pairs(uint64_t* keys_a, uint32_t* vals_a, uint64_t* keys_b, uint32_t* vals_b, int64_t n,
                      int end_bit, void* scratch, hipStream_t stream, bool result_in_b);
int sort_num_passes(int end_bit);

int launch_duplicate_keys(const FrameDev& f, const uint32_t* rects, const uint32_t* depth_keys,
                          const uint32_t* point_offsets, uint64_t* keys, uint32_t* vals, hipStream_t stream);
int launch_rect_counts_scan(const uint32_t* rects, int P, uint32_t* offsets_out, uint32_t* block_sums,
                            hipStream_t stream);
int launch_total_from_block_sums(uint32_t* block_sums, int nb, uint32_t* total_out, hipStream_t stream);

struct TileBinningLayout {
    size_t table, tile_total, tile_start, class_counts, mid_tiles, big_tiles, len_hist, tile_class, tile_part, spill, segments, total;
    int nblocks;
};
int tile_binning_blocks(int P, int64_t R);
bool tile_binning_supported(int n_tiles, int64_t R);
TileBinningLayout tile_binning_layout(int P, int64_t R, int n_tiles);
constexpr int kFusedMaxN = SCG_FUSED_MAX_LIST;
constexpr int kFusedLongBuckets = 1024;
constexpr int kFusedCounters = 1024;
constexpr int kFusedDenseMaxN = 3584;
constexpr int kFusedDenseCounters = 2048;
constexpr int kFusedDenseWaves = 8, kFusedDenseWpe = 8;
constexpr int kDenseMeanList = 1100;
__host__ __device__ inline int fused_max_list(int64_t R, int n_tiles) {
    return (R / (n_tiles > 0 ? n_tiles : 1) >= kDenseMeanList) ? kFusedDenseMaxN : kFusedMaxN;
}
int launch_tile_binning(const FrameDev& f, int64_t R, const uint32_t* rects, const uint32_t* depth_keys,
                        uint32_t* point_list, uint32_t* ranges, uint64_t* keys_sorted, void* scratch,
                        bool* defer_sort, bool hist_done, bool skip_rare, bool rare8, bool split_long, hipStream_t stream);
bool tile_binning_hist_in_geometry(const FrameDev& f, int64_t R);
int launch_geometry_hist_binned(const FrameDev& f, int64_t R, const float* means3D, const float* opacities, const float* shs,
                                const float* colors_precomp, const float* scales, const float* rotations,
                                const float* cov3D_precomp, float* splats, int32_t* radii, uint8_t* clamped, uint32_t* rects,
                                uint32_t* depth_keys, uint32_t* block_sums, void* bin_scratch, hipStream_t stream);
int launch_geometry_hist(const FrameDev& f, const float* means3D, const float* opacities, const float* shs,
                         const float* colors_precomp, const float* scales, const float* rotations,
                         const float* cov3D_precomp, float* splats, int32_t* radii, uint8_t* clamped, uint32_t* rects,
                         uint32_t* depth_keys, uint32_t* block_sums, int nblocks, uint32_t* table, uint32_t* class_counts,
                         uint32_t* len_hist, hipStream_t stream);
hipError_t geometry_hist_set_max_lds(int bytes);
bool tile_binning_defers_sort(int64_t R, int n_tiles);
int launch_tile_blend_forward(const FrameDev& f, const uint32_t* ranges, uint32_t* point_list, const uint32_t* depth_keys,
                              const float* splats, float* out_color, float* out_depth, float* out_alpha,
                              float* final_T, uint32_t* n_contrib, float* dsplats_zero, void* bin_scratch, int64_t R,
                              bool long_presorted, hipStream_t stream);
int launch_tile_ranges(const uint64_t* keys_sorted, int64_t n, uint32_t* ranges, int n_tiles, hipStream_t stream);

int launch_blend_forward(const FrameDev& f, const uint32_t* ranges, const uint32_t* point_list,
                         const float* splats, float* out_color, float* out_depth, float* out_alpha,
                         float* final_T, uint32_t* n_contrib, float* dsplats_zero, hipStream_t stream);
int launch_blend_backward(const FrameDev& f, const uint32_t* ranges, const uint32_t* point_list,
                          const float* splats, const float* final_T, const uint32_t* n_contrib,
                          const float* dL_dcolor, const float* dL_ddepth, const float* dL_dalpha,
                          float* dsplats, bool dsplats_prezeroed, hipStream_t stream, hipEvent_t started = nullptr,
                          hipEvent_t done = nullptr);

#if defined(__HIPCC__)
__device__ __forceinline__ int lane_id() { return threadIdx.x & (kWave - 1); }
__device__ __forceinline__ int wave_id() { return threadIdx.x >> 6; }

__device__ __forceinline__ void tile_rect(float px, float py, float radius, int gx, int gy, int& minx,
                                          int& miny, int& maxx, int& maxy) {
    minx = (int)fminf(fmaxf(truncf((px - radius) * 0.0625f), 0.0f), (float)gx);
    maxx = (int)fminf(fmaxf(truncf((px + radius + 15.0f) * 0.0625f), 0.0f), (float)gx);
    miny = (int)fminf(fmaxf(truncf((py - radius) * 0.0625f), 0.0f), (float)gy);
    maxy = (int)fminf(fmaxf(truncf((py + radius + 15.0f) * 0.0625f), 0.0f), (float)gy);
}

__host__ __device__ __forceinline__ int tile_order_slots(int n_tiles) { return ((n_tiles + 7) >> 3) << 3; }

__device__ __forceinline__ int xcd_tile_remap(int b, int n_tiles) {
    const int xcd = b & 7;
    const int slot = b >> 3;
    const int per = (n_tiles + 7) >> 3;
    const int t = xcd * per + slot;
    return t;
}
#endif

}
```

Measured before the change: 4316 iters/s.

## Precompute SH colour-direction Jacobian in forward and reuse it in backward

During the forward geometry pass, each visible Gaussian's 3x3 Jacobian of SH colour with respect to view direction is computed and stored in extra workspace, staged through LDS when it fits. The backward geometry kernel then forms the mean gradient as a Jacobian-vector product instead of reloading the SH coefficients and re-evaluating basis gradients. This removes SH loads and arithmetic from the backward pass. In exchange the forward does more work, writes 48 bytes per Gaussian, and needs more LDS or workspace.

```diff
diff --git a/scgaussian_amd/csrc/api.hip b/scgaussian_amd/csrc/api.hip
--- a/scgaussian_amd/csrc/api.hip
+++ b/scgaussian_amd/csrc/api.hip
@@ -299,12 +299,12 @@
                                   dsplats, dsplats_prezeroed, stream, nullptr, nullptr);
 }
 
-int scg_geometry_backward(const ScgFrame* frame, const float* means3D, const float* opacities, const float* shs,
-                          const float* colors_precomp, const float* scales, const float* rotations,
-                          const float* cov3D_precomp, const int32_t* radii, const uint8_t* clamped,
-                          const float* dsplats, float* dL_dmeans3D, float* dL_dmeans2D, float* dL_dopacities,
-                          float* dL_dshs, float* dL_dcolors_precomp, float* dL_dscales, float* dL_drotations,
-                          float* dL_dcov3D_precomp, int32_t accumulate, void* stream) {
+static int geometry_backward_checked(const ScgFrame* frame, const float* means3D, const float* opacities, const float* shs,
+                                     const float* colors_precomp, const float* scales, const float* rotations,
+                                     const float* cov3D_precomp, const int32_t* radii, const uint8_t* clamped,
+                                     const float* dsplats, float* dL_dmeans3D, float* dL_dmeans2D, float* dL_dopacities,
+                                     float* dL_dshs, float* dL_dcolors_precomp, float* dL_dscales, float* dL_drotations,
+                                     float* dL_dcov3D_precomp, int32_t accumulate, const float4* jac, void* stream) {
     int rc = validate_frame(frame, false);
     if (rc) return rc;
     rc = validate_inputs(frame, means3D, opacities, shs, colors_precomp, scales, rotations, cov3D_precomp);
@@ -320,7 +320,8 @@
         return fail(SCG_E_EXCLUSIVE, "dL_dscales/dL_drotations / dL_dcov3D_precomp must match the covariance input used");
     if (!aligned64(dsplats) || (dL_drotations && !aligned16(dL_drotations)))
         return fail(SCG_E_ALIGN, "dsplats must be 64-byte, dL_drotations 16-byte aligned");
-    const FrameDev f = make_frame_dev(frame);
+    FrameDev f = make_frame_dev(frame);
+    f.jac = const_cast<float4*>(jac);
     return launch_geometry_backward(f, means3D, opacities, shs, colors_precomp, scales, rotations, cov3D_precomp, radii,
                                     clamped, dsplats, dL_dmeans3D, dL_dmeans2D, dL_dopacities, dL_dshs,
                                     dL_dcolors_precomp, dL_dscales, dL_drotations, dL_dcov3D_precomp,
@@ -328,11 +329,25 @@
                                     reinterpret_cast<hipStream_t>(stream));
 }
 
+int scg_geometry_backward(const ScgFrame* frame, const float* means3D, const float* opacities, const float* shs,
+                          const float* colors_precomp, const float* scales, const float* rotations,
+                          const float* cov3D_precomp, const int32_t* radii, const uint8_t* clamped,
+                          const float* dsplats, float* dL_dmeans3D, float* dL_dmeans2D, float* dL_dopacities,
+                          float* dL_dshs, float* dL_dcolors_precomp, float* dL_dscales, float* dL_drotations,
+                          float* dL_dcov3D_precomp, int32_t accumulate, void* stream) {
+    return geometry_backward_checked(frame, means3D, opacities, shs, colors_precomp, scales, rotations, cov3D_precomp, radii,
+                                     clamped, dsplats, dL_dmeans3D, dL_dmeans2D, dL_dopacities, dL_dshs, dL_dcolors_precomp,
+                                     dL_dscales, dL_drotations, dL_dcov3D_precomp, accumulate, nullptr, stream);
+}
+
 static inline int mark(const ScgStageEvents* ev, int stage, bool end, hipStream_t s) {
     if (!ev) return 0;
     void* e = end ? ev->end[stage] : ev->begin[stage];
     return e ? check_hip(hipEventRecord(reinterpret_cast<hipEvent_t>(e), s), "stage event record") : 0;
 }
+
+static inline size_t jacobian_bytes(int32_t P) { return align_up((size_t)(P > 0 ? P : 1) * 3 * sizeof(float4), 256); }
+static inline size_t jacobian_offset(const ScgWorkspaceLayout& L, int32_t P) { return (size_t)L.total - jacobian_bytes(P); }
 
 int scg_workspace_layout(int32_t P, int64_t capacity, int32_t width, int32_t height, ScgWorkspaceLayout* out) {
     if (!out) return fail(SCG_E_NULL, "layout is NULL");
@@ -351,6 +366,7 @@
     out->final_T = take(hw * sizeof(float));
     out->n_contrib = take(hw * sizeof(uint32_t));
     out->bin_scratch = take(scg_binning_scratch_bytes(P, cap, width, height, SCG_BINNING_AUTO));
+    take(jacobian_bytes(P));
     out->total = (uint64_t)off;
     out->partial_words = (uint64_t)(scg_geometry_scratch_bytes(P) / sizeof(uint32_t));
     return 0;
@@ -375,9 +391,11 @@
     if (rc) return rc;
     if (workspace_bytes < L.total) return fail(SCG_E_SCRATCH, "workspace: %zu < %llu bytes", workspace_bytes, (unsigned long long)L.total);
     hipStream_t s = reinterpret_cast<hipStream_t>(stream);
-    const FrameDev f = make_frame_dev(frame);
+    FrameDev f = make_frame_dev(frame);
     const int n_tiles = f.gx * f.gy;
     char* base = reinterpret_cast<char*>(workspace);
+    if (!(options & SCG_FORWARD_NO_BACKWARD_STATE) && (model || shs))
+        f.jac = reinterpret_cast<float4*>(base + jacobian_offset(L, frame->P));
     float* splats = reinterpret_cast<float*>(base + L.splats);
     uint32_t* rects = reinterpret_cast<uint32_t*>(base + L.rects);
     uint32_t* depth_keys = reinterpret_cast<uint32_t*>(base + L.depth_keys);
@@ -541,10 +559,10 @@
                                 dsplats, dsplats_prezeroed, stream, bb_begin, bb_end);
     if (rc) return rc;
     if ((rc = mark(stage_events, 1, false, s))) return rc;
-    rc = scg_geometry_backward(frame, means3D, opacities, shs, colors_precomp, scales, rotations, cov3D_precomp, radii,
-                               reinterpret_cast<const uint8_t*>(base + L.clamped), dsplats, dL_dmeans3D, dL_dmeans2D,
-                               dL_dopacities, dL_dshs, dL_dcolors_precomp, dL_dscales, dL_drotations, dL_dcov3D_precomp,
-                               accumulate, stream);
+    rc = geometry_backward_checked(frame, means3D, opacities, shs, colors_precomp, scales, rotations, cov3D_precomp, radii,
+                                   reinterpret_cast<const uint8_t*>(base + L.clamped), dsplats, dL_dmeans3D, dL_dmeans2D,
+                                   dL_dopacities, dL_dshs, dL_dcolors_precomp, dL_dscales, dL_drotations, dL_dcov3D_precomp,
+                                   accumulate, reinterpret_cast<const float4*>(base + jacobian_offset(L, frame->P)), stream);
     if (rc) return rc;
     return mark(stage_events, 1, true, s);
 }
@@ -584,7 +602,8 @@
                                 dsplats, dsplats_prezeroed, stream, bb_begin, bb_end);
     if (rc) return rc;
     if ((rc = mark(stage_events, 1, false, s))) return rc;
-    const FrameDev f = make_frame_dev(frame);
+    FrameDev f = make_frame_dev(frame);
+    f.jac = const_cast<float4*>(reinterpret_cast<const float4*>(base + jacobian_offset(L, frame->P)));
     rc = launch_geometry_backward_model(f, *model, *grads, radii, reinterpret_cast<const uint8_t*>(base + L.clamped), dsplats,
                                         dL_dmeans2D, flags & (SCG_BACKWARD_ACCUMULATE | SCG_BACKWARD_SH_TAIL_ZERO), s);
     if (rc) return rc;
diff --git a/scgaussian_amd/csrc/binning_tiles.hip b/scgaussian_amd/csrc/binning_tiles.hip
--- a/scgaussian_amd/csrc/binning_tiles.hip
+++ b/scgaussian_amd/csrc/binning_tiles.hip
@@ -828,7 +828,7 @@
     return launch_geometry_hist(f, means3D, opacities, shs, colors_precomp, scales, rotations, cov3D_precomp, splats, radii,
                                 clamped, rects, depth_keys, block_sums, L.nblocks,
                                 reinterpret_cast<uint32_t*>(base + L.table), reinterpret_cast<uint32_t*>(base + L.class_counts),
-                                reinterpret_cast<uint32_t*>(base + L.len_hist), stream);
+                                reinterpret_cast<uint32_t*>(base + L.len_hist), (size_t)kMaxDynLds - 2048, stream);
 }
 
 int launch_geometry_hist_binned_model(const FrameDev& f, int64_t R, const ScgModel& m, float* splats, int32_t* radii,
@@ -839,7 +839,7 @@
     if (!device_setup()) return fail(SCG_E_RANGE, "tile binning: device setup failed (hipFuncSetAttribute / device query)");
     return launch_geometry_hist_model(f, m, splats, radii, clamped, rects, depth_keys, block_sums, L.nblocks,
                                       reinterpret_cast<uint32_t*>(base + L.table), reinterpret_cast<uint32_t*>(base + L.class_counts),
-                                      reinterpret_cast<uint32_t*>(base + L.len_hist), stream);
+                                      reinterpret_cast<uint32_t*>(base + L.len_hist), (size_t)kMaxDynLds - 2048, stream);
 }
 
 int launch_tile_binning(const FrameDev& f, int64_t R, const uint32_t* rects, const uint32_t* depth_keys,
diff --git a/scgaussian_amd/csrc/geometry.hip b/scgaussian_amd/csrc/geometry.hip
--- a/scgaussian_amd/csrc/geometry.hip
+++ b/scgaussian_amd/csrc/geometry.hip
@@ -276,11 +276,41 @@
     }
 }
 
+template <int DEG>
+__device__ __forceinline__ void sh_basis_grads(float x, float y, float z, float* basis, float* bx, float* by, float* bz);
+
+template <int DEG, int L>
+__device__ __forceinline__ void sh_colour_jacobian_band(const float* sh, float& x, float& y, float& z, float (*J)[3]) {
+    constexpr int K = (DEG + 1) * (DEG + 1);
+#pragma unroll
+    for (int k = L * L; k < (L + 1) * (L + 1); ++k) {
+        if (L < 3 ? k == L * L : (k & 1)) asm volatile("" : "+v"(x), "+v"(y), "+v"(z));
+        float basis[K], bx[K], by[K], bz[K];
+        sh_basis_grads<DEG>(x, y, z, basis, bx, by, bz);
+#pragma unroll
+        for (int c = 0; c < 3; ++c) {
+            J[c][0] += sh[3 * k + c] * bx[k]; J[c][1] += sh[3 * k + c] * by[k]; J[c][2] += sh[3 * k + c] * bz[k];
+        }
+    }
+}
+
+template <int DEG>
+__device__ __forceinline__ void sh_colour_jacobian(const float* sh, float x, float y, float z, float4* j) {
+    float J[3][3] = {{0.f, 0.f, 0.f}, {0.f, 0.f, 0.f}, {0.f, 0.f, 0.f}};
+    sh_colour_jacobian_band<DEG, 1>(sh, x, y, z, J);
+    if constexpr (DEG > 1) sh_colour_jacobian_band<DEG, 2>(sh, x, y, z, J);
+    if constexpr (DEG > 2) sh_colour_jacobian_band<DEG, 3>(sh, x, y, z, J);
+#pragma unroll
+    for (int c = 0; c < 3; ++c) j[c] = make_float4(J[c][0], J[c][1], J[c][2], 0.f);
+}
+
 constexpr int kStageVec = 4 * kWave;
+constexpr int kStageVecJ = 7 * kWave;
 
 __device__ __forceinline__ void flush_stage(const float4* stage, int first, int P, float4* __restrict__ splats,
                                             int32_t* __restrict__ radii, uint8_t* __restrict__ clamped,
-                                            uint2* __restrict__ rects, uint32_t* __restrict__ depth_keys) {
+                                            uint2* __restrict__ rects, uint32_t* __restrict__ depth_keys,
+                                            float4* __restrict__ jac_staged = nullptr ) {
     const int lane = lane_id();
     __builtin_amdgcn_fence(__ATOMIC_RELEASE, "wavefront");
     __builtin_amdgcn_wave_barrier();
@@ -291,6 +321,15 @@
     for (int k = 0; k < 3; ++k) {
         const int idx = k * kWave + lane;
         if (idx < 3 * n) dst[idx] = stage[idx];
+    }
+    if (jac_staged) {
+        __builtin_amdgcn_sched_barrier(0);
+        float4* dstj = jac_staged + 3 * (size_t)first;
+#pragma unroll
+        for (int k = 0; k < 3; ++k) {
+            const int idx = k * kWave + lane;
+            if (idx < 3 * n) dstj[idx] = stage[kStageVec + idx];
+        }
     }
     if (lane < n) {
         const uint4 u = reinterpret_cast<const uint4*>(stage + 3 * kWave)[lane];
@@ -308,7 +347,7 @@
 template <int DEG, class Src, class Between>
 __device__ __forceinline__ uint32_t geometry_forward_one(
     const FrameDev& f, const Mat16& V, const Mat16& PM, int i, bool valid, const GeoIn& in,
-    const Src& src, float4* stage , Between&& between
+    const Src& src, float4* stage , bool jstaged, Between&& between
 #ifdef SCG_PROBE_TIMELINE
     , uint32_t* g_tp
 #endif
@@ -319,6 +358,15 @@
     uint8_t clamp_bits = 0;
     uint2 rect = make_uint2(0u, 0u);
     float px = 0.f, py = 0.f, con_a = 0.f, con_b = 0.f, con_c = 0.f, tz = 0.f;
+    auto store_jacobian = [&](const float4* jc) {
+        if (jstaged) {
+            float4* js = stage + kStageVec + 3 * lane_id();
+            js[0] = jc[0]; js[1] = jc[1]; js[2] = jc[2];
+        } else if (valid) {
+            float4* dst = f.jac + 3 * (size_t)i;
+            dst[0] = jc[0]; dst[1] = jc[1]; dst[2] = jc[2];
+        }
+    };
 
     Proj p;
     bool ok = valid && project(f, V, PM, in.x, in.y, in.z, p);
@@ -395,6 +443,22 @@
     stage[3 * lane + 1] = sb;
     stage[3 * lane + 2] = sc;
     reinterpret_cast<uint4*>(stage + 3 * kWave)[lane] = make_uint4((uint32_t)radius_i, (uint32_t)clamp_bits, rect.x, rect.y);
+    if constexpr (DEG >= 1) {
+        if (f.jac && ok) {
+            float dx = in.x - f.campos[0], dy = in.y - f.campos[1], dz = in.z - f.campos[2];
+            const float len = sqrtf(dx * dx + dy * dy + dz * dz);
+            dx = dx / len; dy = dy / len; dz = dz / len;
+            float4 jc[3];
+            sh_colour_jacobian<DEG>(sh, dx, dy, dz, jc);
+            store_jacobian(jc);
+        }
+    }
+    if constexpr (DEG >= 1) {
+        if (f.jac && !ok) {
+            const float4 zero[3] = {make_float4(0.f, 0.f, 0.f, 0.f), make_float4(0.f, 0.f, 0.f, 0.f), make_float4(0.f, 0.f, 0.f, 0.f)};
+            store_jacobian(zero);
+        }
+    }
     return my_tiles;
 }
 
@@ -404,23 +468,25 @@
     int32_t* __restrict__ radii, uint8_t* __restrict__ clamped, uint2* __restrict__ rects,
     uint32_t* __restrict__ depth_keys, uint32_t* __restrict__ block_sums) {
     __shared__ uint32_t s_wave_sum[kBlock / kWave];
-    __shared__ float4 s_stage[(kBlock / kWave) * kStageVec];
+    constexpr int kVec = DEG >= 1 ? kStageVecJ : kStageVec;
+    __shared__ float4 s_stage[(kBlock / kWave) * kVec];
     const int i = blockIdx.x * kBlock + threadIdx.x;
     const bool valid = i < f.P;
     const GeoIn in = src.template load<(DEG < 0)>(valid ? i : f.P - 1);
     const Mat16 V = load16(f.view);
     const Mat16 PM = load16(f.proj);
-    float4* stage = s_stage + kStageVec * wave_id();
+    float4* stage = s_stage + kVec * wave_id();
+    const bool with_j = DEG >= 1 && f.jac != nullptr;
 #ifdef SCG_PROBE_TIMELINE
     uint32_t tp_dummy[5] = {0u, 0u, 0u, 0u, 0u};
 #endif
-    const uint32_t my_tiles = geometry_forward_one<DEG>(f, V, PM, i, valid, in, src, stage,
+    const uint32_t my_tiles = geometry_forward_one<DEG>(f, V, PM, i, valid, in, src, stage, with_j,
                                                         [](uint2) {}
 #ifdef SCG_PROBE_TIMELINE
                                                         , tp_dummy
 #endif
                                                         );
-    flush_stage(stage, i - lane_id(), f.P, splats, radii, clamped, rects, depth_keys);
+    flush_stage(stage, i - lane_id(), f.P, splats, radii, clamped, rects, depth_keys, with_j ? f.jac : nullptr);
 
     uint32_t s = my_tiles;
 #pragma unroll
@@ -452,8 +518,9 @@
 __host__ __device__ __forceinline__ size_t geometry_hist_stage_offset(int n_tiles, int max_blocks) {
     return ((size_t)(n_tiles + max_blocks) * sizeof(uint32_t) + 15) & ~(size_t)15;
 }
-__host__ __device__ __forceinline__ size_t geometry_hist_lds_bytes(int n_tiles, int max_blocks) {
-    return geometry_hist_stage_offset(n_tiles, max_blocks) + (size_t)(kBinThreads / kWave) * kStageVec * sizeof(float4);
+__host__ __device__ __forceinline__ size_t geometry_hist_lds_bytes(int n_tiles, int max_blocks, bool stage_j) {
+    return geometry_hist_stage_offset(n_tiles, max_blocks) +
+           (size_t)(kBinThreads / kWave) * (stage_j ? kStageVecJ : kStageVec) * sizeof(float4);
 }
 
 template <int DEG, class Src>
@@ -461,12 +528,16 @@
     const FrameDev& f, const Src& src, float4* __restrict__ splats,
     int32_t* __restrict__ radii, uint8_t* __restrict__ clamped, uint2* __restrict__ rects,
     uint32_t* __restrict__ depth_keys, uint32_t* __restrict__ block_sums,
-    uint32_t* __restrict__ table, uint32_t* __restrict__ class_counts, uint32_t* __restrict__ len_hist, int max_blocks) {
+    uint32_t* __restrict__ table, uint32_t* __restrict__ class_counts, uint32_t* __restrict__ len_hist, int max_blocks,
+    int stage_j ) {
     extern __shared__ __attribute__((aligned(16))) unsigned char smem[];
     uint32_t* hist = reinterpret_cast<uint32_t*>(smem);
     const int n_tiles = f.gx * f.gy;
     uint32_t* s_blk = hist + n_tiles;
-    float4* stage = reinterpret_cast<float4*>(smem + geometry_hist_stage_offset(n_tiles, max_blocks)) + kStageVec * wave_id();
+    const bool with_j = DEG >= 1 && f.jac != nullptr && stage_j != 0;
+    float4* stage = reinterpret_cast<float4*>(smem + geometry_hist_stage_offset(n_tiles, max_blocks)) +
+                    (with_j ? kStageVecJ : kStageVec) * wave_id();
+
     uint32_t blk_a, blk_b;
     block_slice((uint32_t)f.P, gridDim.x, blockIdx.x, blk_a, blk_b);
     const int lane = lane_id();
@@ -498,8 +569,8 @@
         uint32_t grabbed = 0;
         if (lane == 0) grabbed = atomicAdd(next_chunk, 1u);
         const uint32_t my_tiles = geometry_forward_one<DEG>(
-            f, V, PM, i, i < f.P, in, src, stage, [&](uint2 rect) {
-                if (pending >= 0) flush_stage(stage, pending, f.P, splats, radii, clamped, rects, depth_keys);
+            f, V, PM, i, i < f.P, in, src, stage, with_j, [&](uint2 rect) {
+                if (pending >= 0) flush_stage(stage, pending, f.P, splats, radii, clamped, rects, depth_keys, with_j ? f.jac : nullptr);
                 walk_rects(rect, (uint32_t)i, f.gx, [&](uint32_t tile, uint32_t) { atomicAdd(&hist[tile], 1u); });
             }
 #ifdef SCG_PROBE_TIMELINE
@@ -516,7 +587,7 @@
         if (lane == 0 && s) atomicAdd(&s_blk[(chunk >> 2) - blk_a], s);
         chunk = (uint32_t)__builtin_amdgcn_readfirstlane((int)grabbed);
     }
-    if (pending >= 0) flush_stage(stage, pending, f.P, splats, radii, clamped, rects, depth_keys);
+    if (pending >= 0) flush_stage(stage, pending, f.P, splats, radii, clamped, rects, depth_keys, with_j ? f.jac : nullptr);
 #ifdef SCG_PROBE_TIMELINE
     const uint32_t tp_loop_end = (uint32_t)wall_clock64();
 #endif
@@ -540,18 +611,22 @@
     const float* __restrict__ rotations, const float* __restrict__ cov3D_precomp, float4* __restrict__ splats,
     int32_t* __restrict__ radii, uint8_t* __restrict__ clamped, uint2* __restrict__ rects,
     uint32_t* __restrict__ depth_keys, uint32_t* __restrict__ block_sums, int sh_vec16,
-    uint32_t* __restrict__ table, uint32_t* __restrict__ class_counts, uint32_t* __restrict__ len_hist, int max_blocks) {
+    uint32_t* __restrict__ table, uint32_t* __restrict__ class_counts, uint32_t* __restrict__ len_hist, int max_blocks,
+    int stage_j) {
     const TensorSource src{means3D, opacities, shs, colors_precomp, scales, rotations, cov3D_precomp, f.M, sh_vec16};
-    geometry_hist_body<DEG>(f, src, splats, radii, clamped, rects, depth_keys, block_sums, table, class_counts, len_hist, max_blocks);
+    geometry_hist_body<DEG>(f, src, splats, radii, clamped, rects, depth_keys, block_sums, table, class_counts, len_hist, max_blocks,
+                            stage_j);
 }
 
 template <int DEG>
 __global__ __launch_bounds__(kBinThreads) void geometry_hist_model_kernel(
     FrameDev f, ScgModel model, float4* __restrict__ splats, int32_t* __restrict__ radii, uint8_t* __restrict__ clamped,
     uint2* __restrict__ rects, uint32_t* __restrict__ depth_keys, uint32_t* __restrict__ block_sums,
-    uint32_t* __restrict__ table, uint32_t* __restrict__ class_counts, uint32_t* __restrict__ len_hist, int max_blocks) {
+    uint32_t* __restrict__ table, uint32_t* __restrict__ class_counts, uint32_t* __restrict__ len_hist, int max_blocks,
+    int stage_j) {
     const ModelSource src{model};
-    geometry_hist_body<DEG>(f, src, splats, radii, clamped, rects, depth_keys, block_sums, table, class_counts, len_hist, max_blocks);
+    geometry_hist_body<DEG>(f, src, splats, radii, clamped, rects, depth_keys, block_sums, table, class_counts, len_hist, max_blocks,
+                            stage_j);
 }
 
 template <int DEG>
@@ -588,26 +663,28 @@
     }
 }
 
-template <int DEG, bool STREAM = false>
+template <int DEG, bool STREAM = false, bool NO_DIR = false>
 __device__ __forceinline__ void sh_backward(const float* rec, bool vec16, float x, float y, float z,
                                             const float* dRGB, float* dsh_rec, int M,
                                             float& ddx, float& ddy, float& ddz, bool acc,
                                             int sw = -1) {
     auto at = [&](int j) { return sw < 0 ? j : ((((j >> 2) ^ sw) << 2) | (j & 3)); };
     constexpr int K = (DEG + 1) * (DEG + 1);
-    float sh[STREAM ? 3 : (3 * K + 3) / 4 * 4];
-    if (!STREAM) load_sh<K>(rec, vec16, sh);
+    float sh[(STREAM || NO_DIR) ? 3 : (3 * K + 3) / 4 * 4];
+    if (!STREAM && !NO_DIR) load_sh<K>(rec, vec16, sh);
     float basis[K];
     float bx[K], by[K], bz[K];
     sh_basis_grads<DEG>(x, y, z, basis, bx, by, bz);
     ddx = ddy = ddz = 0.f;
 #pragma unroll
     for (int k = 0; k < K; ++k) {
-        float s0, s1, s2;
-        if (STREAM) { s0 = rec[at(3 * k)]; s1 = rec[at(3 * k + 1)]; s2 = rec[at(3 * k + 2)]; }
-        else { s0 = sh[3 * k]; s1 = sh[3 * k + 1]; s2 = sh[3 * k + 2]; }
-        const float g = s0 * dRGB[0] + s1 * dRGB[1] + s2 * dRGB[2];
-        ddx += g * bx[k]; ddy += g * by[k]; ddz += g * bz[k];
+        if (!NO_DIR) {
+            float s0, s1, s2;
+            if (STREAM) { s0 = rec[at(3 * k)]; s1 = rec[at(3 * k + 1)]; s2 = rec[at(3 * k + 2)]; }
+            else { s0 = sh[3 * k]; s1 = sh[3 * k + 1]; s2 = sh[3 * k + 2]; }
+            const float g = s0 * dRGB[0] + s1 * dRGB[1] + s2 * dRGB[2];
+            ddx += g * bx[k]; ddy += g * by[k]; ddz += g * bz[k];
+        }
         if (acc) {
             dsh_rec[at(3 * k + 0)] += basis[k] * dRGB[0];
             dsh_rec[at(3 * k + 1)] += basis[k] * dRGB[1];
@@ -723,7 +800,7 @@
 constexpr int kShVec = 12;
 constexpr int kShSlot = 13;
 
-template <bool STAGED, int BLOCK, bool STAGE_IN = STAGED>
+template <bool STAGED, int BLOCK, bool STAGE_IN = STAGED, bool USE_J = false>
 __global__ __launch_bounds__(BLOCK) void geometry_backward_kernel(
     FrameDev f, const float* __restrict__ means3D, const float* __restrict__ opacities,
     const float* __restrict__ shs, const float* __restrict__ colors_precomp, const float* __restrict__ scales,
@@ -748,7 +825,7 @@
     const int i = owner ? block_first + (int)threadIdx.x : f.P;
     const int n_vec = min(RECS, f.P - block_first) * kShVec;
     if (!STAGED && i >= f.P) return;
-    constexpr bool stage_sh = STAGED && STAGE_IN;
+    constexpr bool stage_sh = STAGED && STAGE_IN && !USE_J;
     float4 stage[stage_sh ? kShVec : 1];
     if (stage_sh) {
         const float4* src = reinterpret_cast<const float4*>(shs) + (size_t)block_first * kShVec;
@@ -763,6 +840,10 @@
     float4 gb = dsplats[kRec * (size_t)ic + 1];
     float4 gc = dsplats[kRec * (size_t)ic + 2];
     uint8_t cb = clamped[ic];
+    float4 j0 = make_float4(0.f, 0.f, 0.f, 0.f), j1 = j0, j2 = j0;
+    if (USE_J && f.D > 0) {
+        j0 = f.jac[3 * (size_t)ic + 0]; j1 = f.jac[3 * (size_t)ic + 1]; j2 = f.jac[3 * (size_t)ic + 2];
+    }
     const Mat16 V = load16(f.view);
     const Mat16 PM = load16(f.proj);
     float cam_x = f.campos[0], cam_y = f.campos[1], cam_z = f.campos[2];
@@ -781,8 +862,9 @@
         asm volatile("" : "+v"(gc.x), "+v"(gc.y), "+v"(gc.z), "+v"(in.x), "+v"(in.y), "+v"(in.z), "+v"(in.opacity));
         asm volatile("" : "+v"(in.a[0]), "+v"(in.a[1]), "+v"(in.a[2]), "+v"(in.a[3]), "+v"(in.a[4]), "+v"(in.a[5]), "+v"(in.a[6]));
         asm volatile("" : "+v"(cam_x), "+v"(cam_y), "+v"(cam_z));
-    }
-    if (STAGED) __syncthreads();
+        if (USE_J) asm volatile("" : "+v"(j0.x), "+v"(j0.y), "+v"(j0.z), "+v"(j1.x), "+v"(j1.y), "+v"(j1.z), "+v"(j2.x), "+v"(j2.y), "+v"(j2.z));
+    }
+    if (STAGED && !USE_J) __syncthreads();
     float* my_slot = reinterpret_cast<float*>(&s_sh[STAGED ? min((int)threadIdx.x, RECS - 1) * kSlot : 0]);
 
     float dm[3] = {0.f, 0.f, 0.f};
@@ -809,6 +891,21 @@
             float gx_ = 0.f, gy_ = 0.f, gz_ = 0.f;
             const float* rec = stage_sh ? my_slot : shs + (size_t)i * f.M * 3;
             float* drec = STAGED ? my_slot : dshs + (size_t)i * f.M * 3;
+            if (USE_J) {
+                switch (f.D) {
+                    case 0: sh_backward<0, false, true>(nullptr, false, dx, dy, dz, dRGB, drec, f.M, gx_, gy_, gz_, !STAGED && accumulate,
+                                                        STAGED ? sw : -1); break;
+                    case 1: sh_backward<1, false, true>(nullptr, false, dx, dy, dz, dRGB, drec, f.M, gx_, gy_, gz_, !STAGED && accumulate,
+                                                        STAGED ? sw : -1); break;
+                    case 2: sh_backward<2, false, true>(nullptr, false, dx, dy, dz, dRGB, drec, f.M, gx_, gy_, gz_, !STAGED && accumulate,
+                                                        STAGED ? sw : -1); break;
+                    default: sh_backward<3, false, true>(nullptr, false, dx, dy, dz, dRGB, drec, f.M, gx_, gy_, gz_, !STAGED && accumulate,
+                                                         STAGED ? sw : -1); break;
+                }
+                gx_ = j0.x * dRGB[0] + j1.x * dRGB[1] + j2.x * dRGB[2];
+                gy_ = j0.y * dRGB[0] + j1.y * dRGB[1] + j2.y * dRGB[2];
+                gz_ = j0.z * dRGB[0] + j1.z * dRGB[1] + j2.z * dRGB[2];
+            } else
             switch (f.D) {
                 case 0: sh_backward<0>(rec, sh_vec16, dx, dy, dz, dRGB, drec, f.M, gx_, gy_, gz_, !STAGED && accumulate,
                                         STAGED ? sw : -1); break;
@@ -934,21 +1031,14 @@
 constexpr int kRestRounds = (kRestVecs + kWave - 1) / kWave;
 constexpr int kDcVecs = kModelRecs * 3 / 4;
 
-template <int DEG, bool STREAM>
-__device__ __forceinline__ void sh_backward_model(const float* sh, float* dc_t, float* rest_t, float x, float y, float z,
-                                                  const float* dRGB, float& ddx, float& ddy, float& ddz) {
+template <int DEG>
+__device__ __forceinline__ void sh_backward_model(float* dc_t, float* rest_t, float x, float y, float z, const float* dRGB) {
     constexpr int K = (DEG + 1) * (DEG + 1);
     float basis[K], bx[K], by[K], bz[K];
     sh_basis_grads<DEG>(x, y, z, basis, bx, by, bz);
-    ddx = ddy = ddz = 0.f;
 #pragma unroll
     for (int k = 0; k < K; ++k) {
         float* slot = (k == 0) ? dc_t : rest_t + 3 * (k - 1);
-        float s0, s1, s2;
-        if (STREAM) { s0 = slot[0]; s1 = slot[1]; s2 = slot[2]; }
-        else { s0 = sh[3 * k]; s1 = sh[3 * k + 1]; s2 = sh[3 * k + 2]; }
-        const float g = s0 * dRGB[0] + s1 * dRGB[1] + s2 * dRGB[2];
-        ddx += g * bx[k]; ddy += g * by[k]; ddz += g * bz[k];
         slot[0] = basis[k] * dRGB[0];
         slot[1] = basis[k] * dRGB[1];
         slot[2] = basis[k] * dRGB[2];
@@ -957,7 +1047,6 @@
         for (int w = 3 * (K - 1); w < kRestFloats; ++w) rest_t[w] = 0.f;
 }
 
-template <bool STAGE_IN>
 __global__ __launch_bounds__(kWave) __attribute__((amdgpu_waves_per_eu(4, 4))) void geometry_backward_model_kernel(
     FrameDev f, ScgModel m, ScgModelGrads g, const int32_t* __restrict__ radii, const uint8_t* __restrict__ clamped,
     const float4* __restrict__ dsplats, float* __restrict__ dmeans2D, int flags, int blocks_ray) {
@@ -982,26 +1071,6 @@
     const int active = 3 * (K - 1);
     const ModelSource src{m};
 
-    const bool full = n == kModelRecs;
-    if constexpr (STAGE_IN) {
-        typedef const __attribute__((address_space(1))) void* gptr_t;
-        typedef __attribute__((address_space(3))) void* lptr_t;
-        if (full) {
-            const float4* src4 = reinterpret_cast<const float4*>(set.features_rest + (size_t)first * kRestFloats);
-#pragma unroll
-            for (int k = 0; k < kRestRounds - 1; ++k)
-                __builtin_amdgcn_global_load_lds((gptr_t)(src4 + k * kWave + t), (lptr_t)(s_rest4 + k * kWave), 16, 0, 0);
-            if ((kRestRounds - 1) * kWave + t < kRestVecs)
-                __builtin_amdgcn_global_load_lds((gptr_t)(src4 + (kRestRounds - 1) * kWave + t),
-                                                 (lptr_t)(s_rest4 + (kRestRounds - 1) * kWave), 16, 0, 0);
-            if (t < kDcVecs)
-                __builtin_amdgcn_global_load_lds((gptr_t)(reinterpret_cast<const float4*>(set.features_dc + (size_t)first * 3) + t),
-                                                 (lptr_t)s_dc4, 16, 0, 0);
-        } else {
-            for (int w = t; w < n_rest; w += kWave) s_rest[w] = set.features_rest[(size_t)first * kRestFloats + w];
-            for (int w = t; w < n_dc; w += kWave) s_dc[w] = set.features_dc[(size_t)first * 3 + w];
-        }
-    }
     int radius = radii[i];
     ModelSource::Raw raw = src.load_raw(i);
     constexpr int kRec = SCG_DSPLAT_FLOATS / 4;
@@ -1009,11 +1078,14 @@
     float4 gb = dsplats[kRec * (size_t)i + 1];
     float4 gc = dsplats[kRec * (size_t)i + 2];
     uint8_t cb = clamped[i];
+    float4 j0 = make_float4(0.f, 0.f, 0.f, 0.f), j1 = j0, j2 = j0;
+    if (f.D > 0) { j0 = f.jac[3 * (size_t)i + 0]; j1 = f.jac[3 * (size_t)i + 1]; j2 = f.jac[3 * (size_t)i + 2]; }
     const Mat16 V = load16(f.view);
     const Mat16 PM = load16(f.proj);
     float cam_x = f.campos[0], cam_y = f.campos[1], cam_z = f.campos[2];
     __builtin_amdgcn_sched_barrier(0);
     {
+        asm volatile("" : "+v"(j0.x), "+v"(j0.y), "+v"(j0.z), "+v"(j1.x), "+v"(j1.y), "+v"(j1.z), "+v"(j2.x), "+v"(j2.y), "+v"(j2.z));
         int rr = radius, cc = cb;
         asm volatile("" : "+v"(rr), "+v"(cc), "+v"(ga.x), "+v"(ga.y), "+v"(ga.z), "+v"(ga.w), "+v"(gb.x), "+v"(gb.y), "+v"(gb.z));
         radius = rr; cb = (uint8_t)cc;
@@ -1021,7 +1093,6 @@
         asm volatile("" : "+v"(raw.o[0]), "+v"(raw.o[1]), "+v"(raw.o[2]), "+v"(raw.d[0]), "+v"(raw.d[1]), "+v"(raw.d[2]));
         asm volatile("" : "+v"(raw.ls[0]), "+v"(raw.ls[1]), "+v"(raw.ls[2]), "+v"(cam_x), "+v"(cam_y), "+v"(cam_z));
     }
-    __syncthreads();
     float den;
     const GeoIn in = ModelSource::activate(raw, &den);
     float* dc_t = s_dc + 3 * min(t, kModelRecs - 1);
@@ -1050,16 +1121,15 @@
         const float len = sqrtf(dx * dx + dy * dy + dz * dz);
         const float ilen = 1.0f / len;
         dx *= ilen; dy *= ilen; dz *= ilen;
-        float gx_ = 0.f, gy_ = 0.f, gz_ = 0.f;
-        if constexpr (STAGE_IN) {
-            sh_backward_model<3, true>(nullptr, dc_t, rest_t, dx, dy, dz, dRGB, gx_, gy_, gz_);
-        } else {
-            switch (f.D) {
-                case 0: { float sh[4]; src.load_sh<1>(i, sh); sh_backward_model<0, false>(sh, dc_t, rest_t, dx, dy, dz, dRGB, gx_, gy_, gz_); break; }
-                case 1: { float sh[12]; src.load_sh<4>(i, sh); sh_backward_model<1, false>(sh, dc_t, rest_t, dx, dy, dz, dRGB, gx_, gy_, gz_); break; }
-                default: { float sh[28]; src.load_sh<9>(i, sh); sh_backward_model<2, false>(sh, dc_t, rest_t, dx, dy, dz, dRGB, gx_, gy_, gz_); break; }
-            }
-        }
+        switch (f.D) {
+            case 0: sh_backward_model<0>(dc_t, rest_t, dx, dy, dz, dRGB); break;
+            case 1: sh_backward_model<1>(dc_t, rest_t, dx, dy, dz, dRGB); break;
+            case 2: sh_backward_model<2>(dc_t, rest_t, dx, dy, dz, dRGB); break;
+            default: sh_backward_model<3>(dc_t, rest_t, dx, dy, dz, dRGB); break;
+        }
+        const float gx_ = j0.x * dRGB[0] + j1.x * dRGB[1] + j2.x * dRGB[2];
+        const float gy_ = j0.y * dRGB[0] + j1.y * dRGB[1] + j2.y * dRGB[2];
+        const float gz_ = j0.z * dRGB[0] + j1.z * dRGB[1] + j2.z * dRGB[2];
         sh_written = true;
         const float dot = dx * gx_ + dy * gy_ + dz * gz_;
         dm[0] += (gx_ - dx * dot) * ilen;
@@ -1209,17 +1279,18 @@
                          const float* colors_precomp, const float* scales, const float* rotations,
                          const float* cov3D_precomp, float* splats, int32_t* radii, uint8_t* clamped, uint32_t* rects,
                          uint32_t* depth_keys, uint32_t* block_sums, int nblocks, uint32_t* table, uint32_t* class_counts,
-                         uint32_t* len_hist, hipStream_t stream) {
+                         uint32_t* len_hist, size_t lds_ceiling, hipStream_t stream) {
     const int vec16 = (shs && aligned16(shs) && ((f.M * 3 * 4) % 16 == 0)) ? 1 : 0;
     const int n_tiles = f.gx * f.gy;
     const int nb256 = (f.P + kBlock - 1) / kBlock;
     const int max_blocks = nb256 / nblocks + 2;
-    const size_t lds = geometry_hist_lds_bytes(n_tiles, max_blocks);
+    const int stage_j = (f.jac && !colors_precomp && f.D >= 1 && geometry_hist_lds_bytes(n_tiles, max_blocks, true) <= lds_ceiling) ? 1 : 0;
+    const size_t lds = geometry_hist_lds_bytes(n_tiles, max_blocks, stage_j != 0);
     by_degree(colors_precomp ? -1 : f.D, [&](auto deg) {
         hipLaunchKernelGGL(geometry_hist_kernel<decltype(deg)::value>, dim3(nblocks), dim3(kBinThreads), lds, stream, f, means3D,
                            opacities, shs, colors_precomp, scales, rotations, cov3D_precomp, reinterpret_cast<float4*>(splats),
                            radii, clamped, reinterpret_cast<uint2*>(rects), depth_keys, block_sums, vec16, table, class_counts,
-                           len_hist, max_blocks);
+                           len_hist, max_blocks, stage_j);
     });
     return check_hip(hipGetLastError(), "geometry_hist_kernel");
 }
@@ -1235,7 +1306,9 @@
     const int block = staged ? kWave : kBlock;
     const int recs = staged ? 60 : kBlock;
     const int blocks = (f.P + recs - 1) / recs;
-    auto kernel = !staged ? geometry_backward_kernel<false, kBlock>
+    const bool use_j = f.jac && shs;
+    auto kernel = !staged ? (use_j ? geometry_backward_kernel<false, kBlock, false, true> : geometry_backward_kernel<false, kBlock>)
+                  : use_j ? geometry_backward_kernel<true, kWave, false, true>
                           : (f.D >= 3 ? geometry_backward_kernel<true, kWave, true> : geometry_backward_kernel<true, kWave, false>);
     hipLaunchKernelGGL(kernel, dim3(blocks), dim3(block), 0, stream, f, means3D, opacities, shs, colors_precomp, scales, rotations,
                        cov3D_precomp, radii, clamped, reinterpret_cast<const float4*>(dsplats), dmeans3D, dmeans2D, dopac,
@@ -1267,15 +1340,16 @@
 
 int launch_geometry_hist_model(const FrameDev& f, const ScgModel& m, float* splats, int32_t* radii, uint8_t* clamped,
                                uint32_t* rects, uint32_t* depth_keys, uint32_t* block_sums, int nblocks, uint32_t* table,
-                               uint32_t* class_counts, uint32_t* len_hist, hipStream_t stream) {
+                               uint32_t* class_counts, uint32_t* len_hist, size_t lds_ceiling, hipStream_t stream) {
     const int n_tiles = f.gx * f.gy;
     const int nb256 = (f.P + kBlock - 1) / kBlock;
     const int max_blocks = nb256 / nblocks + 2;
-    const size_t lds = geometry_hist_lds_bytes(n_tiles, max_blocks);
+    const int stage_j = (f.jac && f.D >= 1 && geometry_hist_lds_bytes(n_tiles, max_blocks, true) <= lds_ceiling) ? 1 : 0;
+    const size_t lds = geometry_hist_lds_bytes(n_tiles, max_blocks, stage_j != 0);
     by_degree(f.D, [&](auto deg) {
         hipLaunchKernelGGL(geometry_hist_model_kernel<decltype(deg)::value>, dim3(nblocks), dim3(kBinThreads), lds, stream, f, m,
                            reinterpret_cast<float4*>(splats), radii, clamped, reinterpret_cast<uint2*>(rects), depth_keys,
-                           block_sums, table, class_counts, len_hist, max_blocks);
+                           block_sums, table, class_counts, len_hist, max_blocks, stage_j);
     });
     return check_hip(hipGetLastError(), "geometry_hist_model_kernel");
 }
@@ -1285,8 +1359,8 @@
     const int blocks_ray = (m.ray.count + kModelRecs - 1) / kModelRecs;
     const int blocks_bg = (m.bg.count + kModelRecs - 1) / kModelRecs;
     if (blocks_ray + blocks_bg == 0) return 0;
-    auto kernel = f.D >= 3 ? geometry_backward_model_kernel<true> : geometry_backward_model_kernel<false>;
-    hipLaunchKernelGGL(kernel, dim3(blocks_ray + blocks_bg), dim3(kWave), 0, stream, f, m, g, radii, clamped,
+    if (!f.jac) return fail(SCG_E_NULL, "geometry_backward_model: the forward's colour Jacobians are missing");
+    hipLaunchKernelGGL(geometry_backward_model_kernel, dim3(blocks_ray + blocks_bg), dim3(kWave), 0, stream, f, m, g, radii, clamped,
                        reinterpret_cast<const float4*>(dsplats), dmeans2D, flags, blocks_ray);
     return check_hip(hipGetLastError(), "geometry_backward_model_kernel");
 }
diff --git a/scgaussian_amd/csrc/scg_common.h b/scgaussian_amd/csrc/scg_common.h
--- a/scgaussian_amd/csrc/scg_common.h
+++ b/scgaussian_amd/csrc/scg_common.h
@@ -33,6 +33,7 @@
     const uint32_t* bcost_in;
     uint32_t* bcost_out;
     uint32_t* nr_out;
+    float4* jac;
 };
 
 inline FrameDev make_frame_dev(const ScgFrame* f) {
@@ -50,6 +51,7 @@
     d.cost_in = f->tile_cost_in; d.cost_out = f->tile_cost_out; d.long_out = f->long_lists_out;
     d.bcost_in = f->bwd_cost_in; d.bcost_out = f->bwd_cost_out;
     d.nr_out = f->num_rendered_out;
+    d.jac = nullptr;
     return d;
 }
 
@@ -71,7 +73,7 @@
                                   uint32_t* rects, uint32_t* depth_keys, uint32_t* block_sums, hipStream_t stream);
 int launch_geometry_hist_model(const FrameDev& f, const ScgModel& m, float* splats, int32_t* radii, uint8_t* clamped,
                                uint32_t* rects, uint32_t* depth_keys, uint32_t* block_sums, int nblocks, uint32_t* table,
-                               uint32_t* class_counts, uint32_t* len_hist, hipStream_t stream);
+                               uint32_t* class_counts, uint32_t* len_hist, size_t lds_ceiling, hipStream_t stream);
 int launch_geometry_hist_binned_model(const FrameDev& f, int64_t R, const ScgModel& m, float* splats, int32_t* radii,
                                       uint8_t* clamped, uint32_t* rects, uint32_t* depth_keys, uint32_t* block_sums,
                                       void* bin_scratch, hipStream_t stream);
@@ -125,7 +127,7 @@
                          const float* colors_precomp, const float* scales, const float* rotations,
                          const float* cov3D_precomp, float* splats, int32_t* radii, uint8_t* clamped, uint32_t* rects,
                          uint32_t* depth_keys, uint32_t* block_sums, int nblocks, uint32_t* table, uint32_t* class_counts,
-                         uint32_t* len_hist, hipStream_t stream);
+                         uint32_t* len_hist, size_t lds_ceiling , hipStream_t stream);
 hipError_t geometry_hist_set_max_lds(int bytes);
 bool tile_binning_defers_sort(int64_t R, int n_tiles);
 int launch_tile_blend_forward(const FrameDev& f, const uint32_t* ranges, uint32_t* point_list, const uint32_t* depth_keys,
```

New measurement: 4310 iters/s. About the same (-0.1%).
